# elizabethfong/SparkSmithWaterman

Measured on AMD Instinct MI355X. Metric: GCUPS, higher is better.
Workload: dtype int32

## Files before the change

include/swmi.h:

```cpp
#ifndef SWMI_H
#define SWMI_H

#include <stddef.h>
#include <stdint.h>

#ifdef __cplusplus
extern "C" {
#endif

#define SWMI_ABI_VERSION 3

typedef enum swmi_status {
    SWMI_OK               =  0,
    SWMI_ERR_INVALID      = -1,
    SWMI_ERR_NO_DEVICE    = -2,
    SWMI_ERR_HIP          = -3,
    SWMI_ERR_NOMEM        = -4,
    SWMI_ERR_UNSUPPORTED  = -5,
    SWMI_ERR_RANGE        = -6
} swmi_status;

#define SWMI_TIE_SERIAL 0
#define SWMI_TIE_STRICT 1

typedef struct swmi_params {
    int32_t match;
    int32_t mismatch;
    int32_t gap;
    int32_t tie_mode;
    char    types[4];
} swmi_params;

typedef struct swmi_ctx    swmi_ctx;
typedef struct swmi_batch  swmi_batch;

int         swmi_abi_version(void);
const char *swmi_last_error(void);
int         swmi_device_count(int *count);
int         swmi_create(int device, swmi_ctx **out);
void        swmi_destroy(swmi_ctx *ctx);
void        swmi_default_params(swmi_params *p);

int         swmi_set_option(swmi_ctx *ctx, const char *name, int64_t value);

int  swmi_batch_upload(swmi_ctx *ctx,
                       const uint8_t *ref_bytes, const uint64_t *ref_off, uint32_t n_refs,
                       const uint8_t *read_bytes, const uint64_t *read_off, uint32_t n_reads,
                       swmi_batch **out);
int  swmi_batch_run(swmi_ctx *ctx, swmi_batch *b, const swmi_params *p);
void swmi_batch_free(swmi_ctx *ctx, swmi_batch *b);
int  swmi_batch_run_async(swmi_ctx *ctx, swmi_batch *b, const swmi_params *p);
int  swmi_batch_wait(swmi_ctx *ctx);

typedef struct swmi_timing {
    float    fill_ms, traceback_ms, d2h_ms, total_ms;
    uint32_t fill_launches, rerun_pairs;
    uint64_t cells;
    uint64_t dir_bytes;
    uint32_t strip_fallbacks;
    uint32_t col_chunks;
    uint32_t resident_pairs;
    uint32_t tfused_pairs;
} swmi_timing;
int  swmi_batch_timing(const swmi_batch *b, swmi_timing *t);
int  swmi_batch_mode(const swmi_batch *b, int *mode);

#define SWMI_PAIR_DEGENERATE 0x1u
uint64_t swmi_batch_n_pairs(const swmi_batch *b);
int      swmi_pair_score(const swmi_batch *b, uint64_t pair, int32_t *score);
int      swmi_pair_n_alignments(const swmi_batch *b, uint64_t pair, uint64_t *n, uint32_t *flags);
int      swmi_batch_pair_results(const swmi_batch *b, int32_t *scores, uint64_t *n_alignments, uint64_t n);
int      swmi_pair_alignment(swmi_batch *b, uint64_t pair, uint64_t k,
                             int32_t *begin, int32_t *end_i, int32_t *end_j,
                             const char **ref_aln, const char **read_aln, uint32_t *len);

int      swmi_batch_materialise_all(swmi_batch *b, uint64_t *n_alignments, uint64_t *n_chars);

int      swmi_ref_total(const swmi_batch *b, uint32_t ref, int32_t *total);
int      swmi_ref_totals(const swmi_batch *b, int32_t *totals, uint32_t n);
int      swmi_ref_n_match_sites(swmi_batch *b, uint32_t ref, uint64_t *n);
int      swmi_ref_match_site(swmi_batch *b, uint32_t ref, uint64_t k, int32_t *begin,
                             const char **ref_aln, const char **read_aln, uint32_t *len);

int      swmi_ref_sites_packed(swmi_batch *b, uint32_t ref_lo, uint32_t ref_hi,
                               int32_t *totals, uint64_t *degenerate, uint64_t *site_first,
                               int32_t *begins, uint32_t *lens, uint64_t *str_off, uint64_t sites_cap,
                               uint8_t *blob, uint64_t blob_cap, uint64_t *n_sites, uint64_t *blob_bytes);

int  swmi_align_batch(swmi_ctx *ctx, const swmi_params *p,
                      const uint8_t *ref_bytes, const uint64_t *ref_off, uint32_t n_refs,
                      const uint8_t *read_bytes, const uint64_t *read_off, uint32_t n_reads,
                      swmi_batch **out);

typedef struct swmi_stream swmi_stream;
typedef struct swmi_stream_stats {
    double   push_ms;
    double   parse_ms;
    double   upload_ms, run_ms;
    double   gpu_sweep_ms, gpu_traceback_ms;
    uint64_t bytes, cells;
    uint32_t chunks, pad;
} swmi_stream_stats;
int      swmi_stream_open(swmi_ctx *ctx, const swmi_params *p, const uint8_t *read_bytes, const uint64_t *read_off,
                          uint32_t n_reads, uint32_t slots, uint64_t chunk_bytes, swmi_stream **out);
int      swmi_stream_push(swmi_stream *s, const uint8_t *ref_bytes, const uint64_t *ref_off, uint32_t n_refs);
int      swmi_stream_push_file(swmi_stream *s, const char *path, const char *delimiter, uint32_t parse_threads);
int      swmi_stream_push_file_shard(swmi_stream *s, const char *path, const char *delimiter, uint32_t parse_threads,
                                     uint32_t shard, uint32_t n_shards);
int      swmi_stream_finish(swmi_stream *s);
uint64_t swmi_stream_n_refs(const swmi_stream *s);
uint32_t swmi_stream_n_chunks(const swmi_stream *s);
int      swmi_stream_chunk(swmi_stream *s, uint32_t k, swmi_batch **batch, uint64_t *first_ref);
int      swmi_stream_totals(const swmi_stream *s, int32_t *totals, uint64_t n);
int      swmi_stream_metadata(const swmi_stream *s, uint64_t ref, char *buf, size_t cap);
int      swmi_stream_ref_pos(const swmi_stream *s, uint64_t ref, uint64_t *pos);
int      swmi_stream_ref_sequence(const swmi_stream *s, uint64_t ref, uint8_t *buf, uint64_t cap, uint64_t *len);
int      swmi_stream_get_stats(const swmi_stream *s, swmi_stream_stats *st);
void     swmi_stream_close(swmi_stream *s);

#ifdef __cplusplus
}
#endif
#endif
```

sparksmithwaterman_amd/_capi.py:

```python
import ctypes as C
import os

_HERE = os.path.dirname(os.path.abspath(__file__))
LIB_PATH = os.environ.get("SWMI_LIB") or os.path.join(_HERE, "lib", "libswmi.so")

TIE_SERIAL = 0
TIE_STRICT = 1
PAIR_DEGENERATE = 0x1


class SwmiError(RuntimeError):
    def __init__(self, code, msg):
        super().__init__("swmi error %d: %s" % (code, msg))
        self.code = code


class Params(C.Structure):
    _fields_ = [("match", C.c_int32), ("mismatch", C.c_int32), ("gap", C.c_int32),
                ("tie_mode", C.c_int32), ("types", C.c_char * 4)]


class Timing(C.Structure):
    _fields_ = [("fill_ms", C.c_float), ("traceback_ms", C.c_float), ("d2h_ms", C.c_float),
                ("total_ms", C.c_float), ("fill_launches", C.c_uint32), ("rerun_pairs", C.c_uint32),
                ("cells", C.c_uint64), ("dir_bytes", C.c_uint64),
                ("strip_fallbacks", C.c_uint32), ("col_chunks", C.c_uint32),
                ("resident_pairs", C.c_uint32), ("tfused_pairs", C.c_uint32)]


class StreamStats(C.Structure):
    _fields_ = [("push_ms", C.c_double), ("parse_ms", C.c_double), ("upload_ms", C.c_double), ("run_ms", C.c_double),
                ("gpu_sweep_ms", C.c_double), ("gpu_traceback_ms", C.c_double), ("bytes", C.c_uint64), ("cells", C.c_uint64),
                ("chunks", C.c_uint32), ("pad", C.c_uint32)]


_P = C.c_void_p
_u8p = C.POINTER(C.c_uint8)
_u64p = C.POINTER(C.c_uint64)
SYMBOLS = [
    ("swmi_abi_version", C.c_int, []),
    ("swmi_last_error", C.c_char_p, []),
    ("swmi_device_count", C.c_int, [C.POINTER(C.c_int)]),
    ("swmi_create", C.c_int, [C.c_int, C.POINTER(_P)]),
    ("swmi_destroy", None, [_P]),
    ("swmi_default_params", None, [C.POINTER(Params)]),
    ("swmi_set_option", C.c_int, [_P, C.c_char_p, C.c_int64]),
    ("swmi_batch_upload", C.c_int, [_P, C.c_char_p, _u64p, C.c_uint32, C.c_char_p, _u64p, C.c_uint32, C.POINTER(_P)]),
    ("swmi_batch_run", C.c_int, [_P, _P, C.POINTER(Params)]),
    ("swmi_batch_run_async", C.c_int, [_P, _P, C.POINTER(Params)]),
    ("swmi_batch_wait", C.c_int, [_P]),
    ("swmi_batch_free", None, [_P, _P]),
    ("swmi_batch_timing", C.c_int, [_P, C.POINTER(Timing)]),
    ("swmi_batch_mode", C.c_int, [_P, C.POINTER(C.c_int)]),
    ("swmi_batch_n_pairs", C.c_uint64, [_P]),
    ("swmi_pair_score", C.c_int, [_P, C.c_uint64, C.POINTER(C.c_int32)]),
    ("swmi_pair_n_alignments", C.c_int, [_P, C.c_uint64, _u64p, C.POINTER(C.c_uint32)]),
    ("swmi_pair_alignment", C.c_int, [_P, C.c_uint64, C.c_uint64, C.POINTER(C.c_int32), C.POINTER(C.c_int32),
                                      C.POINTER(C.c_int32), C.POINTER(C.c_char_p), C.POINTER(C.c_char_p),
                                      C.POINTER(C.c_uint32)]),
    ("swmi_batch_pair_results", C.c_int, [_P, C.POINTER(C.c_int32), _u64p, C.c_uint64]),
    ("swmi_batch_materialise_all", C.c_int, [_P, _u64p, _u64p]),
    ("swmi_ref_total", C.c_int, [_P, C.c_uint32, C.POINTER(C.c_int32)]),
    ("swmi_ref_totals", C.c_int, [_P, C.POINTER(C.c_int32), C.c_uint32]),
    ("swmi_ref_n_match_sites", C.c_int, [_P, C.c_uint32, _u64p]),
    ("swmi_ref_match_site", C.c_int, [_P, C.c_uint32, C.c_uint64, C.POINTER(C.c_int32), C.POINTER(C.c_char_p),
                                      C.POINTER(C.c_char_p), C.POINTER(C.c_uint32)]),
    ("swmi_ref_sites_packed", C.c_int, [_P, C.c_uint32, C.c_uint32, C.POINTER(C.c_int32), _u64p, _u64p, C.POINTER(C.c_int32),
                                        C.POINTER(C.c_uint32), _u64p, C.c_uint64, C.c_void_p, C.c_uint64, _u64p, _u64p]),
    ("swmi_stream_open", C.c_int, [_P, C.POINTER(Params), C.c_char_p, _u64p, C.c_uint32, C.c_uint32, C.c_uint64, C.POINTER(_P)]),
    ("swmi_stream_push", C.c_int, [_P, C.c_char_p, _u64p, C.c_uint32]),
    ("swmi_stream_push_file", C.c_int, [_P, C.c_char_p, C.c_char_p, C.c_uint32]),
    ("swmi_stream_push_file_shard", C.c_int, [_P, C.c_char_p, C.c_char_p, C.c_uint32, C.c_uint32, C.c_uint32]),
    ("swmi_stream_finish", C.c_int, [_P]),
    ("swmi_stream_n_refs", C.c_uint64, [_P]),
    ("swmi_stream_n_chunks", C.c_uint32, [_P]),
    ("swmi_stream_chunk", C.c_int, [_P, C.c_uint32, C.POINTER(_P), _u64p]),
    ("swmi_stream_totals", C.c_int, [_P, C.POINTER(C.c_int32), C.c_uint64]),
    ("swmi_stream_metadata", C.c_int, [_P, C.c_uint64, C.c_char_p, C.c_size_t]),
    ("swmi_stream_ref_pos", C.c_int, [_P, C.c_uint64, _u64p]),
    ("swmi_stream_ref_sequence", C.c_int, [_P, C.c_uint64, C.c_void_p, C.c_uint64, _u64p]),
    ("swmi_stream_get_stats", C.c_int, [_P, C.POINTER(StreamStats)]),
    ("swmi_stream_close", None, [_P]),
    ("swmi_align_batch", C.c_int, [_P, C.POINTER(Params), C.c_char_p, _u64p, C.c_uint32, C.c_char_p, _u64p,
                                   C.c_uint32, C.POINTER(_P)]),
]

_lib = None


def load():
    global _lib
    if _lib is None:
        if not os.path.exists(LIB_PATH):
            raise ImportError(
                "%s is missing: build it with `python -c 'import __graft_entry__ as g; g.build()'` "
                "(hipcc, gfx950).  There is no CPU fallback." % LIB_PATH)
        lib = C.CDLL(LIB_PATH)
        for name, res, args in SYMBOLS:
            f = getattr(lib, name)
            f.restype = res
            f.argtypes = args
        _lib = lib
    return _lib


def check(rc):
    if rc != 0:
        raise SwmiError(rc, load().swmi_last_error().decode("utf-8", "replace"))


def as_bytes(s):
    return bytes(s) if isinstance(s, (bytes, bytearray, memoryview)) else s.encode("latin-1")


def pack(seqs):
    bs = [as_bytes(s) for s in seqs]
    off = (C.c_uint64 * (len(bs) + 1))()
    t = 0
    for k, b in enumerate(bs):
        off[k] = t
        t += len(b)
    off[len(bs)] = t
    return b"".join(bs), off
```

sparksmithwaterman_amd/aligner.py:

```python
import ctypes as C
import weakref

from . import _capi
from ._capi import Params, Timing, StreamStats, check

DEFAULT_SCORES = (5, -3, -4)
DEFAULT_TYPES = ("a", "i", "d", "-")


def make_params(align_scores=None, align_types=None, tie_mode=_capi.TIE_SERIAL):
    sc = DEFAULT_SCORES if align_scores is None else tuple(int(x) for x in align_scores)
    ty = DEFAULT_TYPES if align_types is None else tuple(align_types)
    if len(sc) != 3 or len(ty) != 4:
        raise ValueError("alignScores needs 3 entries and alignTypes 4")
    p = Params()
    p.match, p.mismatch, p.gap = sc
    p.tie_mode = tie_mode
    p.types = b"".join(_capi.as_bytes(t)[:1] for t in ty)
    return p


class Context:

    def __init__(self, device=0):
        self._lib = _capi.load()
        h = C.c_void_p()
        check(self._lib.swmi_create(int(device), C.byref(h)))
        self._h = h
        self.device = int(device)

    def set_option(self, name, value):
        check(self._lib.swmi_set_option(self._h, name.encode(), int(value)))

    def upload(self, refs, reads):
        return Batch(self, refs, reads)

    def stream(self, reads, params=None, slots=0, chunk_bytes=0):
        return Stream(self, reads, params, slots, chunk_bytes)

    def close(self):
        if getattr(self, "_h", None):
            self._lib.swmi_destroy(self._h)
            self._h = None

    def __del__(self):
        try:
            self.close()
        except Exception:
            pass


class Batch:

    _owned = True

    @classmethod
    def _view(cls, lib, handle, n_refs, n_reads, owner):
        b = cls.__new__(cls)
        b._ctx, b._lib, b._h, b.n_refs, b.n_reads, b._owned = None, lib, handle, n_refs, n_reads, False
        b._owner = owner
        return b

    def __init__(self, ctx, refs, reads):
        self._ctx = ctx
        self._lib = ctx._lib
        self.n_refs, self.n_reads = len(refs), len(reads)
        rb, ro = _capi.pack(refs)
        qb, qo = _capi.pack(reads)
        h = C.c_void_p()
        check(self._lib.swmi_batch_upload(ctx._h, rb, ro, self.n_refs, qb, qo, self.n_reads, C.byref(h)))
        self._h = h

    def run(self, params=None):
        p = params if params is not None else make_params()
        check(self._lib.swmi_batch_run(self._ctx._h, self._h, C.byref(p)))
        return self

    def run_async(self, params=None):
        p = params if params is not None else make_params()
        self._async_params = p
        check(self._lib.swmi_batch_run_async(self._ctx._h, self._h, C.byref(p)))
        return self

    def wait(self):
        check(self._lib.swmi_batch_wait(self._ctx._h))
        return self

    def timing(self):
        t = Timing()
        check(self._lib.swmi_batch_timing(self._h, C.byref(t)))
        return t

    def pipeline_mode(self):
        v = C.c_int()
        check(self._lib.swmi_batch_mode(self._h, C.byref(v)))
        return v.value

    def score(self, pair):
        v = C.c_int32()
        check(self._lib.swmi_pair_score(self._h, pair, C.byref(v)))
        return v.value

    def n_alignments(self, pair):
        n, f = C.c_uint64(), C.c_uint32()
        check(self._lib.swmi_pair_n_alignments(self._h, pair, C.byref(n), C.byref(f)))
        return n.value, f.value

    def alignment(self, pair, k, with_cell=False):
        b, ei, ej = C.c_int32(), C.c_int32(), C.c_int32()
        r, q, ln = C.c_char_p(), C.c_char_p(), C.c_uint32()
        check(self._lib.swmi_pair_alignment(self._h, pair, k, C.byref(b), C.byref(ei), C.byref(ej),
                                            C.byref(r), C.byref(q), C.byref(ln)))
        rec = (b.value, (r.value.decode("latin-1"), q.value.decode("latin-1")))
        return rec + ((ei.value, ej.value),) if with_cell else rec

    def alignments(self, pair, with_cell=False):
        n, _ = self.n_alignments(pair)
        return [self.alignment(pair, k, with_cell) for k in range(n)]

    def pair_results(self):
        import numpy as np
        n = self.n_refs * self.n_reads
        sc = np.empty(n, dtype=np.int32)
        na = np.empty(n, dtype=np.uint64)
        check(self._lib.swmi_batch_pair_results(self._h, sc.ctypes.data_as(C.POINTER(C.c_int32)),
                                                na.ctypes.data_as(C.POINTER(C.c_uint64)), n))
        return sc, na

    def scores(self):
        import numpy as np
        n = self.n_refs * self.n_reads
        sc = np.empty(n, dtype=np.int32)
        check(self._lib.swmi_batch_pair_results(self._h, sc.ctypes.data_as(C.POINTER(C.c_int32)), None, n))
        return sc

    def materialise_all(self):
        na, nc = C.c_uint64(), C.c_uint64()
        check(self._lib.swmi_batch_materialise_all(self._h, C.byref(na), C.byref(nc)))
        return na.value, nc.value

    def ref_total(self, ref):
        v = C.c_int32()
        check(self._lib.swmi_ref_total(self._h, ref, C.byref(v)))
        return v.value

    def ref_totals(self):
        import numpy as np
        out = np.empty(self.n_refs, dtype=np.int32)
        check(self._lib.swmi_ref_totals(self._h, out.ctypes.data_as(C.POINTER(C.c_int32)), self.n_refs))
        return out

    def ref_match_sites(self, ref):
        n = C.c_uint64()
        check(self._lib.swmi_ref_n_match_sites(self._h, ref, C.byref(n)))
        out = []
        b, r, q, ln = C.c_int32(), C.c_char_p(), C.c_char_p(), C.c_uint32()
        for k in range(n.value):
            check(self._lib.swmi_ref_match_site(self._h, ref, k, C.byref(b), C.byref(r), C.byref(q), C.byref(ln)))
            out.append((b.value, (r.value.decode("latin-1"), q.value.decode("latin-1"))))
        return out

    def ref_sites_packed(self, ref_lo=0, ref_hi=None):
        import numpy as np
        ref_hi = self.n_refs if ref_hi is None else ref_hi
        n = ref_hi - ref_lo
        ns, nb = C.c_uint64(), C.c_uint64()
        check(self._lib.swmi_ref_sites_packed(self._h, ref_lo, ref_hi, None, None, None, None, None, None, 0, None, 0,
                                              C.byref(ns), C.byref(nb)))
        totals = np.empty(max(n, 1), dtype=np.int32)
        deg = np.empty(max(n, 1), dtype=np.uint64)
        first = np.empty(n + 1, dtype=np.uint64)
        begins = np.empty(max(ns.value, 1), dtype=np.int32)
        lens = np.empty(max(ns.value, 1), dtype=np.uint32)
        off = np.empty(max(ns.value, 1), dtype=np.uint64)
        blob = np.empty(max(nb.value, 1), dtype=np.uint8)
        P = C.POINTER
        check(self._lib.swmi_ref_sites_packed(
            self._h, ref_lo, ref_hi, totals.ctypes.data_as(P(C.c_int32)), deg.ctypes.data_as(P(C.c_uint64)),
            first.ctypes.data_as(P(C.c_uint64)), begins.ctypes.data_as(P(C.c_int32)), lens.ctypes.data_as(P(C.c_uint32)),
            off.ctypes.data_as(P(C.c_uint64)), ns.value, blob.ctypes.data_as(C.c_void_p), nb.value, C.byref(ns), C.byref(nb)))
        raw = blob.tobytes()
        out = []
        for r in range(n):
            sites = []
            for s in range(int(first[r]), int(first[r + 1])):
                o, ln = int(off[s]), int(lens[s])
                sites.append((int(begins[s]), (raw[o:o + ln].decode("latin-1"), raw[o + ln:o + 2 * ln].decode("latin-1"))))
            out.append((int(totals[r]), int(deg[r]), sites))
        return out

    def free(self):
        if getattr(self, "_h", None) and self._owned:
            self._lib.swmi_batch_free(self._ctx._h, self._h)
        self._h = None

    def __del__(self):
        try:
            self.free()
        except Exception:
            pass


class Stream:

    def __init__(self, ctx, reads, params=None, slots=0, chunk_bytes=0):
        self._ctx, self._lib = ctx, ctx._lib
        self.n_reads = len(reads)
        qb, qo = _capi.pack(reads)
        p = params if params is not None else make_params()
        h = C.c_void_p()
        check(self._lib.swmi_stream_open(ctx._h, C.byref(p), qb, qo, self.n_reads, int(slots), int(chunk_bytes), C.byref(h)))
        self._h = h
        self._views = []

    def push(self, refs):
        rb, ro = _capi.pack(refs)
        check(self._lib.swmi_stream_push(self._h, rb, ro, len(refs)))
        return self

    def push_file(self, path, delimiter=">gi", parse_threads=0):
        import os
        check(self._lib.swmi_stream_push_file(self._h, os.fspath(path).encode(), delimiter.encode("latin-1"), int(parse_threads)))
        return self

    def push_file_shard(self, path, shard, n_shards, delimiter=">gi", parse_threads=0):
        import os
        check(self._lib.swmi_stream_push_file_shard(self._h, os.fspath(path).encode(), delimiter.encode("latin-1"),
                                                    int(parse_threads), int(shard), int(n_shards)))
        return self

    def finish(self):
        check(self._lib.swmi_stream_finish(self._h))
        return self

    def n_refs(self):
        return self._lib.swmi_stream_n_refs(self._h)

    def chunks(self):
        out = []
        for k in range(self._lib.swmi_stream_n_chunks(self._h)):
            b, first = C.c_void_p(), C.c_uint64()
            check(self._lib.swmi_stream_chunk(self._h, k, C.byref(b), C.byref(first)))
            n_pairs = self._lib.swmi_batch_n_pairs(b)
            v = Batch._view(self._lib, b, n_pairs // max(self.n_reads, 1), self.n_reads, self)
            self._views.append(weakref.ref(v))
            out.append((first.value, v))
        return out

    def totals(self):
# ... 49 lines not shown
```

sparksmithwaterman_amd/csrc/swmi_api.cpp:

```cpp
#include <hip/hip_runtime.h>

#include <algorithm>
#include <atomic>
#include <chrono>
#include <condition_variable>
#include <unistd.h>
#include <cstdarg>
#include <cstdio>
#include <cstdlib>
#include <cstring>
#include <memory>
#include <mutex>
#include <numeric>
#include <string>
#include <thread>
#include <unordered_map>
#include <deque>
#include <vector>

#include "../../include/swmi.h"
#include "swmi_device.h"
#include "swmi_io_internal.h"

extern "C" hipError_t swmi_launch_fill(const FillArgs *a, hipStream_t st, hipEvent_t ev_start, hipEvent_t ev_stop);
extern "C" hipError_t swmi_launch_traceback(const TraceArgs *a, hipStream_t st, hipEvent_t ev_start, hipEvent_t ev_stop);
extern "C" hipError_t swmi_launch_traceback_split(const TraceArgs *a, uint32_t n_windows, hipStream_t st);
extern "C" hipError_t swmi_launch_resident(const TraceArgs *a, const ResidentArgs *x, hipStream_t st);
extern "C" hipError_t swmi_launch_tfused(const TraceArgs *a, const TFusedArgs *x, hipStream_t st);
extern "C" hipError_t swmi_launch_encode(const uint8_t *raw, const uint64_t *raw_off, SeqDesc *desc, uint32_t *seqw,
                                         const uint8_t *lut, uint32_t n_seq, hipStream_t st);

static thread_local std::string g_err;

static int fail(int code, const char *fmt, ...) {
    char buf[512];
    va_list ap;
    va_start(ap, fmt);
    vsnprintf(buf, sizeof buf, fmt, ap);
    va_end(ap);
    g_err = buf;
    return code;
}

int swmi_io_fail(int code, const std::string &msg) { return fail(code, "%s", msg.c_str()); }

#define HIP_TRY(expr)                                                                         \
    do {                                                                                      \
        hipError_t e_ = (expr);                                                               \
        if (e_ != hipSuccess)                                                                 \
            return fail(e_ == hipErrorOutOfMemory ? SWMI_ERR_NOMEM : SWMI_ERR_HIP,            \
                        "%s failed: %s", #expr, hipGetErrorString(e_));                       \
    } while (0)

struct DevBuf {
    void *p = nullptr;
    size_t cap = 0;
    int reserve(size_t bytes) {
        if (bytes <= cap) return SWMI_OK;
        size_t want = bytes >= (256u << 20) ? bytes + bytes / 2 : bytes;
        if (p) { want = std::max(want, cap + cap / 4); (void)hipFree(p); p = nullptr; cap = 0; }
        hipError_t e = hipMalloc(&p, want);
        if (e != hipSuccess && want > bytes) { want = bytes; e = hipMalloc(&p, want); }
        if (e != hipSuccess) { p = nullptr; return fail(SWMI_ERR_NOMEM, "hipMalloc(%zu) failed: %s", bytes, hipGetErrorString(e)); }
        cap = want;
        return SWMI_OK;
    }
    void release() { if (p) (void)hipFree(p); p = nullptr; cap = 0; }
    template <class T> T *as() const { return (T *)p; }
    DevBuf() = default;
    DevBuf(const DevBuf &) = delete;
    DevBuf &operator=(const DevBuf &) = delete;
    ~DevBuf() { release(); }
};

struct PinnedBuf {
    void *p = nullptr;
    void *dp = nullptr;
    size_t cap = 0;
    int reserve(size_t bytes) {
        if (bytes <= cap) return SWMI_OK;
        if (p) { bytes = std::max(bytes, cap + cap / 4); (void)hipHostFree(p); p = nullptr; dp = nullptr; cap = 0; }
        hipError_t e = hipHostMalloc(&p, bytes, hipHostMallocMapped);
        if (e != hipSuccess) { p = nullptr; return fail(SWMI_ERR_NOMEM, "hipHostMalloc(%zu) failed: %s", bytes, hipGetErrorString(e)); }
        e = hipHostGetDevicePointer(&dp, p, 0);
        if (e != hipSuccess) { (void)hipHostFree(p); p = nullptr; return fail(SWMI_ERR_HIP, "hipHostGetDevicePointer: %s", hipGetErrorString(e)); }
        cap = bytes;
        return SWMI_OK;
    }
    void release() { if (p) (void)hipHostFree(p); p = nullptr; dp = nullptr; cap = 0; }
    PinnedBuf() = default;
    PinnedBuf(const PinnedBuf &) = delete;
    PinnedBuf &operator=(const PinnedBuf &) = delete;
    ~PinnedBuf() { release(); }
};

struct swmi_ctx {
    int device = 0;
    hipStream_t stream = nullptr;
    std::mutex mu;
    uint32_t cell_cap = 64;
    uint64_t max_workspace_bytes = 32ull << 30;
    int profiling = 0;
    uint32_t mode = 1;
    int zero_copy = 1;
    uint64_t arena_words_per_pair = 160;
    uint64_t arena_copy_wpp = 160;
    uint64_t recs_per_pair_x16 = 32;
    hipEvent_t ev[6] = {nullptr, nullptr, nullptr, nullptr, nullptr, nullptr};
    PinnedBuf h_err;
    DevBuf d_hdr_ring;
    uint32_t hdr_next = 0;
    DevBuf d_lut;
    int64_t spin_us = 2000;
    uint32_t dbg_strip_spins = 0;
    uint32_t dbg_reverse_strips = 0;
    uint32_t auto_ties_x100 = 300;
    uint32_t col_chunks = 0;
    int tb_split = -1;
    bool ext_events = false;
    int tfused = -1;
    int resident = -1;
    int scores_only = 0;
    int stream_keep_records = 1;
    int device_strings = 1;
    bool cell_cap_set = false;
    std::thread worker;
    std::mutex job_mu;
    std::condition_variable job_cv;
    std::atomic<int> job_state{0};
    swmi_batch *job_batch = nullptr;
    swmi_params job_params{};
    int job_rc = 0;
    std::string job_err;
};

struct HostAln {
    uint32_t rank;
    int32_t begin, end_i, end_j;
    uint32_t n_ops;
    const uint32_t *rec = nullptr;
    int64_t str_id = -1;
};

struct PairRes {
    int32_t score = 0;
    uint32_t flags = 0;
    uint64_t n_cells = 0;
    uint64_t first = 0;
    uint64_t count = 0;
};

struct SiteRef { uint64_t pair; uint64_t k; int32_t begin; };

struct Work {
    uint32_t pair;
    uint64_t cells;
    uint64_t dir_words;
    uint64_t seam_words;
};

struct swmi_batch {
    uint32_t n_refs = 0, n_reads = 0;
    std::vector<uint8_t> ref_bytes, read_bytes;
    const uint8_t *src_map = nullptr;
    std::vector<swmi_io_recpos> src_recs;
    std::unordered_map<uint32_t, std::vector<uint8_t>> src_cache;
    std::vector<uint64_t> ref_off, read_off;
    std::vector<SeqDesc> ref_desc, read_desc;
    DevBuf d_raw, d_raw_off;
    DevBuf d_seqw, d_refs, d_reads, d_pairs, d_dir, d_seam, d_result, d_cells, d_cells_off, d_cells_cap, d_dbg, d_dbg2;
    DevBuf d_strip_items, d_progress;
    DevBuf d_col_items;
    DevBuf d_win_off, d_queue;
    DevBuf d_tf_items;
    DevBuf d_res_items;
    bool views_built = false;
    bool tb_split_used = false;
    bool acgt_known = false;
    PinnedBuf h_result;
    swmi_params params{};
    bool has_run = false;
    int auto_choice = -1;
    swmi_params auto_params{};
    std::vector<Work> work;
    int work_mode = -1;
    bool work_tfused = false;
    uint32_t eff_mode = 1;
    uint64_t work_cells = 0;
    std::vector<uint8_t> pairs_on_device;
    const void *pairs_dev_ptr = nullptr;
    struct Prep {
        bool valid = false;
        size_t lo = 0, hi = 0;
        const void *work = nullptr;
        swmi_params params{};
        int mode = -1;
        uint64_t dir_words = 0, seam_words = 0;
        uint32_t max_path = 0, max_read = 0;
        size_t n_strip_items = 0, n_col_items = 0, n_strip_chunks = 0;
        uint64_t n_windows = 0, seam_priv_words = 0;
        size_t n_res = 0;
        uint32_t res_lds_words = 0, res_ops_words = 0;
        int resident_opt = -1;
        int tfused_opt = -1;
        size_t n_tf = 0;
        uint32_t tf_max_m = 0, tf_max_n = 0, tf_max_path = 0;
        bool exact = false, scores_only = false;
        uint32_t col_chunks_opt = 0;
        bool reverse_strips = false;
    } prep;
    std::vector<PairRes> pairs;
    struct RawChunk { size_t at, words; size_t tab_at, n_rec; size_t lo; std::vector<uint32_t> wpos; };
    std::vector<uint32_t> raw;
    std::vector<AlnRec> rtab;
    const uint32_t *raw_ext = nullptr;
    const AlnRec *rtab_ext = nullptr;
    uint64_t raw_ext_records = 0, raw_ext_cap = 0;
    std::vector<RawChunk> raw_chunks;
    bool indexed = false;
    bool rec_strings = false;
    bool scores_only = false;
    bool records_dropped = false;
    std::vector<HostAln> alns;
    std::vector<char> str_buf;
    std::vector<uint64_t> str_at;
    std::vector<int8_t> ref_view_ready;
    std::vector<std::vector<SiteRef>> ref_sites;
    std::vector<uint64_t> ref_degenerate;
    swmi_timing timing{};
};

static const uint8_t *code_table();

extern "C" int swmi_abi_version(void) { return SWMI_ABI_VERSION; }

extern "C" const char *swmi_last_error(void) { return g_err.c_str(); }

extern "C" int swmi_device_count(int *count) {
    if (!count) return fail(SWMI_ERR_INVALID, "count is null");
    int n = 0;
    hipError_t e = hipGetDeviceCount(&n);
    if (e != hipSuccess) { *count = 0; return fail(SWMI_ERR_NO_DEVICE, "hipGetDeviceCount: %s", hipGetErrorString(e)); }
    *count = n;
    return SWMI_OK;
}

extern "C" void swmi_default_params(swmi_params *p) {
    if (!p) return;
    p->match = 5; p->mismatch = -3; p->gap = -4;
    p->tie_mode = SWMI_TIE_SERIAL;
    p->types[0] = 'a'; p->types[1] = 'i'; p->types[2] = 'd'; p->types[3] = '-';
}

static void ctx_release(swmi_ctx *c) {
    for (auto &ev : c->ev) if (ev) (void)hipEventDestroy(ev);
    if (c->stream) (void)hipStreamDestroy(c->stream);
    c->h_err.release();
    c->d_lut.release();
    c->d_hdr_ring.release();
    delete c;
}

extern "C" int swmi_create(int device, swmi_ctx **out) {
    if (!out) return fail(SWMI_ERR_INVALID, "out is null");
    *out = nullptr;
    int n = 0;
    hipError_t e = hipGetDeviceCount(&n);
    if (e != hipSuccess || n <= 0)
        return fail(SWMI_ERR_NO_DEVICE, "no HIP device available (%s); this library has no CPU fallback",
                    e != hipSuccess ? hipGetErrorString(e) : "device count 0");
    if (device < 0 || device >= n) return fail(SWMI_ERR_INVALID, "device %d out of range [0,%d)", device, n);
    hipDeviceProp_t prop;
    e = hipGetDeviceProperties(&prop, device);
    if (e != hipSuccess) return fail(SWMI_ERR_NO_DEVICE, "hipGetDeviceProperties: %s", hipGetErrorString(e));
    if (strncmp(prop.gcnArchName, "gfx950", 6) != 0)
        return fail(SWMI_ERR_NO_DEVICE, "device %d is %s; the kernels are built for gfx950 (MI355X) only",
                    device, prop.gcnArchName);
    e = hipSetDevice(device);
    if (e != hipSuccess) return fail(SWMI_ERR_NO_DEVICE, "hipSetDevice: %s", hipGetErrorString(e));
    swmi_ctx *c = new swmi_ctx;
    c->device = device;
    e = hipStreamCreateWithFlags(&c->stream, hipStreamNonBlocking);
    if (e != hipSuccess) { c->stream = nullptr; ctx_release(c); return fail(SWMI_ERR_HIP, "hipStreamCreate: %s", hipGetErrorString(e)); }
    for (auto &ev : c->ev) {
        e = hipEventCreate(&ev);
        if (e != hipSuccess) { ev = nullptr; ctx_release(c); return fail(SWMI_ERR_HIP, "hipEventCreate: %s", hipGetErrorString(e)); }
    }
    { int r = c->h_err.reserve(64); if (r) { ctx_release(c); return r; } }
    { static const char *ee = getenv("SWMI_EXT_EVENTS"); if (ee) c->ext_events = atoi(ee) != 0; }
    *(volatile uint32_t *)c->h_err.p = 0u;
    { int r = c->d_lut.reserve(256); if (r) { ctx_release(c); return r; } }
    e = hipMemcpy(c->d_lut.p, code_table(), 256, hipMemcpyHostToDevice);
    if (e != hipSuccess) { ctx_release(c); return fail(SWMI_ERR_HIP, "code table upload: %s", hipGetErrorString(e)); }
    *out = c;
    return SWMI_OK;
}

extern "C" void swmi_destroy(swmi_ctx *ctx) {
    if (!ctx) return;
    (void)hipSetDevice(ctx->device);
    if (ctx->worker.joinable()) {
        {
            std::unique_lock<std::mutex> lk(ctx->job_mu);
            ctx->job_cv.wait(lk, [&] { return ctx->job_state.load() != 1; });
            ctx->job_state.store(3);
        }
        ctx->job_cv.notify_all();
        ctx->worker.join();
    }
    ctx_release(ctx);
}

extern "C" int swmi_set_option(swmi_ctx *ctx, const char *name, int64_t value) {
    if (!ctx || !name) return fail(SWMI_ERR_INVALID, "null argument");
    std::lock_guard<std::mutex> g(ctx->mu);
    if (!strcmp(name, "cell_cap")) {
        if (value < 1 || value > (1 << 20)) return fail(SWMI_ERR_INVALID, "cell_cap out of range");
        ctx->cell_cap = (uint32_t)value;
        ctx->cell_cap_set = true;
    } else if (!strcmp(name, "max_workspace_bytes")) {
        if (value < (1 << 20)) return fail(SWMI_ERR_INVALID, "max_workspace_bytes too small");
        ctx->max_workspace_bytes = (uint64_t)value;
    } else if (!strcmp(name, "mode")) {
        if (value < -1 || value > 2) return fail(SWMI_ERR_INVALID, "mode must be -1 (automatic), 0, 1 or 2");
        ctx->mode = value < 0 ? 1u : (uint32_t)value;
    } else if (!strcmp(name, "auto_ties_x100")) {
        if (value < 100) return fail(SWMI_ERR_INVALID, "auto_ties_x100 out of range");
        ctx->auto_ties_x100 = (uint32_t)value;
    } else if (!strcmp(name, "spin_us")) {
        if (value < 0) return fail(SWMI_ERR_INVALID, "spin_us out of range");
        ctx->spin_us = value;
    } else if (!strcmp(name, "debug_strip_spins")) {
        ctx->dbg_strip_spins = (uint32_t)value;
    } else if (!strcmp(name, "debug_reverse_strips")) {
        ctx->dbg_reverse_strips = value != 0;
    } else if (!strcmp(name, "tfused")) {
        if (value < -1 || value > 1) return fail(SWMI_ERR_INVALID, "tfused must be -1 (automatic), 0 or 1");
        ctx->tfused = (int)value;
    } else if (!strcmp(name, "resident")) {
        if (value < -1 || value > 1) return fail(SWMI_ERR_INVALID, "resident must be -1 (automatic), 0 or 1");
        ctx->resident = (int)value;
    } else if (!strcmp(name, "scores_only")) {
        ctx->scores_only = value != 0;
    } else if (!strcmp(name, "stream_keep_records")) {
        ctx->stream_keep_records = value != 0;
    } else if (!strcmp(name, "device_strings")) {
        ctx->device_strings = value != 0;
    } else if (!strcmp(name, "tb_split")) {
        if (value < -1 || value > 1) return fail(SWMI_ERR_INVALID, "tb_split must be -1 (automatic), 0 or 1");
        ctx->tb_split = (int)value;
    } else if (!strcmp(name, "col_chunks")) {
        if (value < 0 || value > 4096) return fail(SWMI_ERR_INVALID, "col_chunks out of range");
        ctx->col_chunks = (uint32_t)value;
    } else if (!strcmp(name, "zero_copy")) {
        ctx->zero_copy = value != 0;
    } else if (!strcmp(name, "profiling")) {
        if (value < 0 || value > 2) return fail(SWMI_ERR_INVALID, "profiling must be 0, 1 (every stage) or 2 (the sweep only)");
        ctx->profiling = (int)value;
    } else if (!strcmp(name, "arena_words_per_pair")) {
        if (value < 1) return fail(SWMI_ERR_INVALID, "arena_words_per_pair out of range");
        ctx->arena_words_per_pair = (uint64_t)value;
    } else {
        return fail(SWMI_ERR_INVALID, "unknown option '%s'", name);
    }
    return SWMI_OK;
}

static const uint8_t *code_table() {
    static uint8_t T[256];
    static std::once_flag once;
    std::call_once(once, [] {
        uint8_t perm[256];
        for (int i = 0; i < 256; i++) perm[i] = (uint8_t)i;
        const uint8_t fast[8] = {'A', 'C', 'G', 'T', 'N', 'U', 'R', 'Y'};
        for (int k = 0; k < 8; k++) std::swap(perm[fast[k]], perm[4 * k]);
        for (int i = 0; i < 256; i++) {
            int u = i;
            if ((i >= 'a' && i <= 'z') || (i >= 0xE0 && i <= 0xFE && i != 0xF7)) u = i - 32;
            T[i] = perm[u];
        }
    });
    return T;
}

static uint64_t layout_sequences(const uint64_t *off, uint32_t n, uint64_t word0, std::vector<SeqDesc> &desc) {
    desc.resize(n);
    uint64_t at = word0;
    for (uint32_t s = 0; s < n; s++) {
        const uint64_t len = off[s + 1] - off[s];
        at = (at + 3) & ~(uint64_t)3;
        SeqDesc d{};
        d.len = (uint32_t)len;
        d.boff = (uint32_t)at;
        d.acgt = 0;
        desc[s] = d;
        at += (len + 3) / 4 + SWMI_SEQ_PAD_WORDS;
    }
    return at;
}

static int check_offsets(const uint64_t *off, uint32_t n, const char *what) {
    if (!off) return fail(SWMI_ERR_INVALID, "%s offsets are null", what);
    if (off[0] != 0) return fail(SWMI_ERR_INVALID, "%s offsets must start at 0", what);
    for (uint32_t k = 0; k < n; k++) {
        if (off[k + 1] < off[k]) return fail(SWMI_ERR_INVALID, "%s offsets decrease at %u", what, k);
        if (off[k + 1] - off[k] >= (1ull << 30))
            return fail(SWMI_ERR_UNSUPPORTED, "%s %u is longer than 2^30-1 bases", what, k);
    }
    return SWMI_OK;
}

extern "C" void swmi_batch_free(swmi_ctx *ctx, swmi_batch *b) {
    if (!b) return;
    if (ctx) (void)hipSetDevice(ctx->device);
    b->d_raw.release(); b->d_raw_off.release();
    b->d_seqw.release(); b->d_refs.release(); b->d_reads.release(); b->d_pairs.release();
    b->d_dir.release(); b->d_seam.release(); b->d_result.release(); b->d_cells.release();
    b->d_cells_off.release(); b->d_cells_cap.release(); b->d_dbg.release(); b->d_dbg2.release();
    b->d_strip_items.release(); b->d_progress.release(); b->d_col_items.release(); b->d_win_off.release(); b->d_queue.release(); b->d_res_items.release();
    b->d_tf_items.release();
    b->h_result.release();
    delete b;
}

static int upload_device(swmi_ctx *ctx, swmi_batch *b, hipStream_t st, const uint8_t *ref_src, const uint8_t *read_src) {
    const uint32_t n_refs = b->n_refs, n_reads = b->n_reads;
    const uint64_t ref_total = b->ref_off[n_refs], read_total = b->read_off[n_reads];
    uint64_t words = layout_sequences(b->ref_off.data(), n_refs, 0, b->ref_desc);
    words = layout_sequences(b->read_off.data(), n_reads, words, b->read_desc);
    words = ((words + 3) & ~(uint64_t)3) + SWMI_SEQ_PAD_WORDS;
    if (words >= (1ull << 32)) return fail(SWMI_ERR_UNSUPPORTED, "sequence image exceeds 16 GiB");
    int rc;
    const uint64_t read_base = (ref_total + 15) & ~(uint64_t)15;
    if ((rc = b->d_seqw.reserve(words * 4))) return rc;
    if ((rc = b->d_raw.reserve(read_base + read_total + 16))) return rc;
    if ((rc = b->d_raw_off.reserve(((uint64_t)n_refs + n_reads + 2) * 8))) return rc;
    if ((rc = b->d_refs.reserve(std::max<size_t>(n_refs, 1) * sizeof(SeqDesc)))) return rc;
    if ((rc = b->d_reads.reserve(std::max<size_t>(n_reads, 1) * sizeof(SeqDesc)))) return rc;
    HIP_TRY(hipMemsetAsync(b->d_seqw.p, 0, words * 4, st));
    uint8_t *raw = b->d_raw.as<uint8_t>();
    uint64_t *roff = b->d_raw_off.as<uint64_t>();
    if (ref_total) HIP_TRY(hipMemcpyAsync(raw, ref_src, ref_total, hipMemcpyHostToDevice, st));
    if (read_total) HIP_TRY(hipMemcpyAsync(raw + read_base, read_src, read_total, hipMemcpyHostToDevice, st));
    HIP_TRY(hipMemcpyAsync(roff, b->ref_off.data(), ((size_t)n_refs + 1) * 8, hipMemcpyHostToDevice, st));
    std::vector<uint64_t> read_abs(b->read_off);
    for (auto &o : read_abs) o += read_base;
    HIP_TRY(hipMemcpyAsync(roff + n_refs + 1, read_abs.data(), ((size_t)n_reads + 1) * 8, hipMemcpyHostToDevice, st));
    if (n_refs) HIP_TRY(hipMemcpyAsync(b->d_refs.p, b->ref_desc.data(), n_refs * sizeof(SeqDesc), hipMemcpyHostToDevice, st));
    if (n_reads) HIP_TRY(hipMemcpyAsync(b->d_reads.p, b->read_desc.data(), n_reads * sizeof(SeqDesc), hipMemcpyHostToDevice, st));
    HIP_TRY(swmi_launch_encode(raw, roff, b->d_refs.as<SeqDesc>(), b->d_seqw.as<uint32_t>(), ctx->d_lut.as<uint8_t>(), n_refs, st));
    HIP_TRY(swmi_launch_encode(raw, roff + n_refs + 1, b->d_reads.as<SeqDesc>(), b->d_seqw.as<uint32_t>(),
                               ctx->d_lut.as<uint8_t>(), n_reads, st));
    HIP_TRY(hipStreamSynchronize(st));
    b->work_mode = -1; b->prep.valid = false; b->pairs_dev_ptr = nullptr; b->pairs_on_device.clear();
    b->has_run = false; b->acgt_known = false; b->auto_choice = -1;
    return SWMI_OK;
}

extern "C" int swmi_batch_upload(swmi_ctx *ctx,
                                 const uint8_t *ref_bytes, const uint64_t *ref_off, uint32_t n_refs,
                                 const uint8_t *read_bytes, const uint64_t *read_off, uint32_t n_reads,
                                 swmi_batch **out) {
    if (!ctx || !out) return fail(SWMI_ERR_INVALID, "null argument");
    *out = nullptr;
    int rc;
    if ((rc = check_offsets(ref_off, n_refs, "reference"))) return rc;
    if ((rc = check_offsets(read_off, n_reads, "read"))) return rc;
    if ((n_refs && ref_off[n_refs] && !ref_bytes) || (n_reads && read_off[n_reads] && !read_bytes))
        return fail(SWMI_ERR_INVALID, "sequence bytes are null");
    if ((uint64_t)n_refs * n_reads >= (1ull << 32))
        return fail(SWMI_ERR_UNSUPPORTED, "more than 2^32-1 pairs in one batch");
    std::lock_guard<std::mutex> g(ctx->mu);
    HIP_TRY(hipSetDevice(ctx->device));

    std::unique_ptr<swmi_batch> b(new swmi_batch);
    b->n_refs = n_refs; b->n_reads = n_reads;
    b->ref_off.assign(ref_off, ref_off + n_refs + 1);
    b->read_off.assign(read_off, read_off + n_reads + 1);
    b->ref_bytes.assign(ref_bytes, ref_bytes + ref_off[n_refs]);
    b->read_bytes.assign(read_bytes, read_bytes + read_off[n_reads]);
    if ((rc = upload_device(ctx, b.get(), ctx->stream, ref_bytes, read_bytes))) { swmi_batch_free(ctx, b.release()); return rc; }
    *out = b.release();
    return SWMI_OK;
}

namespace {

struct RunState {
    swmi_ctx *ctx;
    swmi_batch *b;
    FillArgs fa{};
    TraceArgs ta{};
    float fill_ms = 0, tb_ms = 0, d2h_ms = 0;
    uint32_t launches = 0;
    double enqueue_us = 0, wait_us = 0, copyout_us = 0, prep_us = 0, prep_upload_us = 0;
    bool one_wave_sweep = false;
    bool tb_split = false;
    bool defer_copy = false;
    bool keep = true;
};

inline size_t result_out_off() { return 64; }
inline size_t result_tab_off(size_t np) { return (64 + np * sizeof(PairOut) + 255) & ~(size_t)255; }
inline size_t result_arena_off(size_t np, uint64_t tab_cap) { return (result_tab_off(np) + tab_cap * sizeof(AlnRec) + 255) & ~(size_t)255; }
inline uint64_t rec_words(uint32_t n_ops, bool strings) {
    return strings ? 2 * ((uint64_t)n_ops / 4 + 1) : ((uint64_t)n_ops + 15) / 16;
}

}

#define SWMI_RES_CELL_CAP 128u

static uint64_t path_bound(uint64_t n_, uint64_t m_, const swmi_params &p) {
    uint64_t path = n_ + m_;
    if (p.match > 0 && p.gap < 0 && p.mismatch <= p.match) {
        const uint64_t g = (uint64_t)(-(int64_t)p.gap), mt = (uint64_t)p.match;
        path = std::min(path, std::min(m_ + std::min(n_, mt * m_ / g), n_ + std::min(m_, mt * n_ / g)));
    }
    return path;
}

static uint64_t traceback_lds_bytes(uint32_t mode, uint64_t max_path, uint64_t max_read) {
    const uint64_t lds_words = (max_path + 3) / 4 + 1, lds_read_words = (max_read + 3) / 4 + 1;
    const uint64_t win = (uint64_t)SWMI_RMAX * 64;
    const uint64_t tile_words = mode == 0 ? 4ull * 16 * win : (mode == 1 ? 32 + 8ull * SWMI_CK_BLOCKS * win : 4ull * SWMI_CK_BLOCKS * win);
    return 4ull * (tile_words + 4ull * (lds_words + lds_read_words + 96));
}

static int prepare_chunk(RunState &rs, const std::vector<Work> &work, size_t lo, size_t hi, const std::vector<uint64_t> *cells_exact) {
    swmi_ctx *ctx = rs.ctx;
    swmi_batch *b = rs.b;
    const size_t np = hi - lo;
    const uint32_t n_reads = b->n_reads;
    int rc;

    std::vector<PairDesc> pd;
    std::vector<StripItem> strip_items;
    uint64_t seam_priv_words = 0;
    size_t n_strip_chunks = 0;
    std::vector<ColItem> col_items;
    uint64_t dir_words = 0, seam_words = 0;
    uint32_t max_path = 0, max_read = 0;
    size_t n_strip_items = 0, n_col_items = 0;
    uint64_t n_windows = 0;
    std::vector<uint32_t> win_off;
    std::vector<uint32_t> res_items;
    size_t n_res = 0;
    uint32_t res_lds_words = 0, res_ops_words = 0;
    std::vector<uint32_t> tf_items;
    size_t n_tf = 0;
    uint32_t tf_max_m = 0, tf_max_n = 0, tf_max_path = 0;
    const uint32_t res_cell_cap = SWMI_RES_CELL_CAP;
    swmi_batch::Prep &pr = b->prep;
    const auto p0 = std::chrono::steady_clock::now();
    const bool prepared = pr.valid && pr.lo == lo && pr.hi == hi && pr.work == (const void *)work.data() && pr.mode == b->eff_mode &&
                          memcmp(&pr.params, &b->params, sizeof(swmi_params)) == 0 && b->pairs_dev_ptr == b->d_pairs.p &&
                          b->pairs_on_device.size() == np * sizeof(PairDesc) && pr.col_chunks_opt == ctx->col_chunks &&
                          pr.reverse_strips == (ctx->dbg_reverse_strips != 0) && pr.resident_opt == ctx->resident &&
                          pr.tfused_opt == ctx->tfused && pr.exact == (cells_exact != nullptr) && pr.scores_only == (ctx->scores_only != 0);
    if (prepared) {
        dir_words = pr.dir_words; seam_words = pr.seam_words; max_path = pr.max_path; max_read = pr.max_read;
        n_strip_items = pr.n_strip_items; n_col_items = pr.n_col_items; n_windows = pr.n_windows;
        seam_priv_words = pr.seam_priv_words; n_strip_chunks = pr.n_strip_chunks;
        n_res = pr.n_res; res_lds_words = pr.res_lds_words; res_ops_words = pr.res_ops_words;
        n_tf = pr.n_tf; tf_max_m = pr.tf_max_m; tf_max_n = pr.tf_max_n; tf_max_path = pr.tf_max_path;
    } else {
    const swmi_params &P = b->params;
    const bool cols_possible = b->eff_mode == 1 && P.match > 0 && P.gap < 0 && P.mismatch <= 0 &&
                               P.match <= 7 && P.mismatch >= -8 && (np <= 512 || ctx->col_chunks > 1) && ctx->col_chunks != 1;
    const bool res_possible = b->eff_mode == 1 && !cells_exact && !ctx->scores_only && ctx->resident != 0 && (ctx->resident == 1 || np >= 256) &&
                              P.match <= 7 && P.match >= -8 && P.mismatch >= -8 && P.mismatch <= 0 && P.gap <= 0;
    auto res_need_words = [&](uint32_t m_, uint32_t n_, uint32_t &opw) -> uint64_t {
        const uint32_t R_ = swmi_rows_per_lane(m_), lact = (m_ + R_ - 1) / R_;
        const uint64_t nblk = ((uint64_t)n_ + lact - 1 + 15) / 16, n_ck = (nblk + SWMI_CK_BLOCKS - 1) / SWMI_CK_BLOCKS;
        opw = (uint32_t)((path_bound(n_, m_, P) + 15) / 16 + 1);
        return nblk * R_ * 64 + ((n_ck + 1) & ~1ull) + 2ull * res_cell_cap + 64ull * opw + (n_ + 3) / 4 + 1 + (m_ + 3) / 4 + 1 + 8 +
               128;
    };
    bool res_maybe = false;
    if (res_possible)
        for (size_t k = 0; k < np && !res_maybe; k++) {
            const uint32_t m_ = b->read_desc[work[lo + k].pair % n_reads].len, n_ = b->ref_desc[work[lo + k].pair / n_reads].len;
            uint32_t opw;
            res_maybe = m_ <= 64u * SWMI_RMAX && (ctx->resident == 1 || (uint64_t)n_ <= 8ull * m_) &&
                        res_need_words(m_, n_, opw) * 4 <= (ctx->resident == 1 ? 40u : 20u) * 1024u;
        }
    const bool tf_possible = b->eff_mode == 1 && !cells_exact && !ctx->scores_only && ctx->tfused == 1 &&
                             P.match > 0 && P.match <= 7 && P.mismatch >= -8 && P.mismatch <= P.match && P.gap < 0 && P.gap >= -64;
    if ((cols_possible || res_maybe || tf_possible) && !b->acgt_known) {
        if (b->n_refs) HIP_TRY(hipMemcpy(b->ref_desc.data(), b->d_refs.p, b->n_refs * sizeof(SeqDesc), hipMemcpyDeviceToHost));
        if (b->n_reads) HIP_TRY(hipMemcpy(b->read_desc.data(), b->d_reads.p, b->n_reads * sizeof(SeqDesc), hipMemcpyDeviceToHost));
        b->acgt_known = true;
    }
    const uint64_t chunk_budget = ctx->col_chunks > 1 ? ctx->col_chunks : std::max<uint64_t>(1, 1024 / std::max<size_t>(np, 1));
    pd.resize(np);
    if (b->eff_mode == 1) win_off.resize(np + 1);
    uint32_t pb_m = 0xFFFFFFFFu, pb_n = 0xFFFFFFFFu, pb_val = 0;
    for (size_t k = 0; k < np; k++) {
        const Work &w = work[lo + k];
        PairDesc d{};
        d.ref_id = w.pair / n_reads;
        d.read_id = w.pair % n_reads;
        d.out_id = (uint32_t)k;
        const uint32_t m_ = b->read_desc[d.read_id].len, n_ = b->ref_desc[d.ref_id].len;
        if (b->eff_mode == 1) {
            const uint64_t rps = 64ull * swmi_rows_per_lane(m_);
            const uint64_t wb = ((uint64_t)n_ + 63u + 15u) / 16u;
            win_off[k] = (uint32_t)std::min<uint64_t>(n_windows, 0xFFFFFFFFu);
            n_windows += ((m_ + rps - 1) / rps) * ((wb + SWMI_CK_BLOCKS - 1u) / SWMI_CK_BLOCKS);
        }
        uint32_t res_opw = 0;
        const bool res_fit = res_maybe && m_ <= 64u * SWMI_RMAX && b->read_desc[d.read_id].acgt && b->ref_desc[d.ref_id].acgt &&
                             (ctx->resident == 1 || (uint64_t)n_ <= 8ull * m_) &&
                             res_need_words(m_, n_, res_opw) * 4 <= (ctx->resident == 1 ? 40u : 20u) * 1024u;
        const bool tf_fit = !res_fit && tf_possible && m_ <= SWMI_TF_MAX_M && n_ <= 64u * SWMI_TF_BMAX &&
                            b->read_desc[d.read_id].acgt && b->ref_desc[d.ref_id].acgt && w.dir_words >= swmi_tf_ck_words(m_);
        if (tf_fit) {
            d.pad = SWMI_PAD_RESIDENT;
            tf_items.push_back((uint32_t)k);
            tf_max_m = std::max(tf_max_m, m_); tf_max_n = std::max(tf_max_n, n_);
            tf_max_path = std::max<uint32_t>(tf_max_path, (uint32_t)path_bound(n_, m_, P));
        } else if (res_fit) {
            d.pad = SWMI_PAD_RESIDENT;
            res_items.push_back((uint32_t)k);
            uint32_t opw;
            res_lds_words = std::max<uint32_t>(res_lds_words, (uint32_t)res_need_words(m_, n_, opw));
            res_ops_words = std::max(res_ops_words, opw);
        } else if (b->eff_mode == 1 && m_ > 64u * SWMI_RMAX && strip_items.size() < (1u << 30)) {
            const uint32_t strips = (m_ + 64u * SWMI_RMAX - 1u) / (64u * SWMI_RMAX);
            d.pad = (uint32_t)strip_items.size();
            auto push_strips = [&](StripItem it) {
                it.pair = (uint32_t)k;
                it.prog = (uint32_t)strip_items.size();
                it.pad = 0;
                if (ctx->dbg_reverse_strips) for (uint32_t st = strips; st-- > 0;) { it.strip = st; strip_items.push_back(it); }
                else                         for (uint32_t st = 0; st < strips; st++) { it.strip = st; strip_items.push_back(it); }
            };
            uint64_t chunks = 1;
            const uint64_t wblocks = ((uint64_t)n_ + 63u + 15u) / 16u;
            const uint32_t n_ck = (uint32_t)((wblocks + SWMI_CK_BLOCKS - 1u) / SWMI_CK_BLOCKS);
            const uint32_t step_w = 16u * SWMI_CK_BLOCKS;
            const uint64_t span = (uint64_t)m_ + (uint64_t)(P.match > 0 ? P.match : 0) * m_ / (uint64_t)(P.gap < 0 ? -(int64_t)P.gap : 1) + 1;
            if (cols_possible) {
                const uint64_t budget = ctx->col_chunks > 1 ? ctx->col_chunks : chunk_budget / strips;
                chunks = std::min<uint64_t>(budget, n_ / std::max<uint64_t>((span + 64) / 4, 256));
                chunks = std::min<uint64_t>(chunks, n_ck);
                if (chunks < 2) chunks = 1;
            }
            if (chunks == 1) {
                StripItem it{};
                it.col0 = 0; it.g_lo = 0; it.g_hi = 0xFFFFFFFFu; it.priv_stride = 0; it.priv_off = 0;
                push_strips(it);
            } else {
                const uint32_t wpc = (uint32_t)((n_ck + chunks - 1) / chunks);
                for (uint32_t g_lo = 0; g_lo < n_ck; g_lo += wpc) {
                    StripItem it{};
                    it.g_lo = g_lo;
                    it.g_hi = std::min(g_lo + wpc, n_ck);
                    if (it.g_hi < n_ck && (uint64_t)it.g_hi * step_w > n_) it.g_hi = n_ck;
                    const int64_t c0 = (int64_t)g_lo * step_w - 64 - (int64_t)span - 1;
                    it.col0 = g_lo == 0 || c0 <= 0 ? 0u : (uint32_t)(c0 / step_w * step_w);
                    const uint64_t ext0 = (uint64_t)it.g_hi * step_w - it.col0 + 64ull * (strips - 1u);
                    const uint64_t n0 = it.g_hi < n_ck ? std::min<uint64_t>(n_ - it.col0, ext0) : n_ - it.col0;
                    it.priv_stride = (uint32_t)((n0 + 1 + 15) & ~15ull);
                    it.priv_off = seam_priv_words;
                    seam_priv_words += (uint64_t)(strips - 1u) * it.priv_stride;
                    if (it.g_hi == n_ck) it.g_hi = 0xFFFFFFFFu;
                    push_strips(it);
                    n_strip_chunks++;
                    if (it.g_hi == 0xFFFFFFFFu) break;
                }
            }
        } else if (cols_possible && chunk_budget > 1 && m_ <= 64u * SWMI_RMAX && b->read_desc[d.read_id].acgt && b->ref_desc[d.ref_id].acgt) {
            const uint64_t span = (uint64_t)m_ + (uint64_t)P.match * m_ / (uint64_t)(-(int64_t)P.gap) + 1;
            const uint64_t wblocks = ((uint64_t)n_ + 63u + 15u) / 16u;
            const uint32_t n_ck = (uint32_t)((wblocks + SWMI_CK_BLOCKS - 1u) / SWMI_CK_BLOCKS);
            const uint32_t step_w = 16u * SWMI_CK_BLOCKS;
            uint64_t chunks = std::min<uint64_t>(chunk_budget, n_ / std::max<uint64_t>(span + 64, 256));
            chunks = std::min<uint64_t>(chunks, n_ck);
            static const bool dbg_one = getenv("SWMI_DEBUG_ONE_CHUNK") != nullptr;
            if (dbg_one) chunks = 1;
            if (chunks >= 2 || dbg_one) {
                const uint32_t wpc = (uint32_t)((n_ck + chunks - 1) / chunks);
                const size_t first = col_items.size();
                for (uint32_t g_lo = 0; g_lo < n_ck; g_lo += wpc) {
                    ColItem ci;
                    ci.pair = (uint32_t)k;
                    ci.g_lo = g_lo;
                    ci.g_hi = std::min(g_lo + wpc, n_ck);
                    if (ci.g_hi < n_ck && (uint64_t)ci.g_hi * step_w > n_) ci.g_hi = n_ck;
                    const int64_t c0 = (int64_t)g_lo * step_w - 64 - (int64_t)span - 1;
                    ci.col0 = g_lo == 0 || c0 <= 0 ? 0u : (uint32_t)(c0 / step_w * step_w);
                    col_items.push_back(ci);
                    if (ci.g_hi == n_ck) break;
                }
                d.pad = SWMI_PAD_COLS | (uint32_t)(col_items.size() - first);
            }
        }
        pd[k] = d;
        if (m_ != pb_m || n_ != pb_n) { pb_m = m_; pb_n = n_; pb_val = (uint32_t)path_bound(n_, m_, b->params); }
        max_path = std::max<uint32_t>(max_path, pb_val);
        max_read = std::max(max_read, m_);
    }
    n_strip_items = strip_items.size();
    n_col_items = col_items.size();
    n_res = res_items.size();
    n_tf = tf_items.size();
    res_lds_words = 0;
    for (uint32_t k : res_items) {
        uint32_t opw;
        const uint32_t m_ = b->read_desc[pd[k].read_id].len, n_ = b->ref_desc[pd[k].ref_id].len;
        const uint64_t own = res_need_words(m_, n_, opw);
        res_lds_words = std::max<uint32_t>(res_lds_words, (uint32_t)(own + 64ull * (res_ops_words - opw)));
    }
    if (16ull * res_lds_words > 160ull * 1024) {
        for (uint32_t k : res_items) pd[k].pad = 0;
        res_items.clear();
        n_res = 0; res_lds_words = 0; res_ops_words = 0;
    }
    {
        std::vector<uint8_t> is_res(np, 0);
        for (uint32_t k : res_items) is_res[k] = 1;
        for (size_t k = 0; k < np; k++) {
            pd[k].dir_off = dir_words;
            pd[k].seam_off = seam_words;
            if (!is_res[k]) { dir_words += work[lo + k].dir_words; seam_words += work[lo + k].seam_words; }
        }
    }
    if (b->eff_mode == 1) win_off[np] = (uint32_t)std::min<uint64_t>(n_windows, 0xFFFFFFFFu);
    for (StripItem &it : strip_items)
        if (it.priv_stride) it.priv_off += seam_words;
    }
    const auto p1 = std::chrono::steady_clock::now();
    if (!prepared && b->eff_mode == 1) {
        if ((rc = b->d_win_off.reserve((np + 1) * sizeof(uint32_t)))) return rc;
        HIP_TRY(hipMemcpyAsync(b->d_win_off.p, win_off.data(), (np + 1) * sizeof(uint32_t), hipMemcpyHostToDevice, ctx->stream));
        HIP_TRY(hipStreamSynchronize(ctx->stream));
    }
    if ((rc = b->d_pairs.reserve(np * sizeof(PairDesc)))) return rc;
    if (!prepared && !strip_items.empty()) {
        if ((rc = b->d_strip_items.reserve(strip_items.size() * sizeof(StripItem)))) return rc;
        if ((rc = b->d_progress.reserve(strip_items.size() * sizeof(uint32_t)))) return rc;
        HIP_TRY(hipMemcpyAsync(b->d_strip_items.p, strip_items.data(), strip_items.size() * sizeof(StripItem), hipMemcpyHostToDevice, ctx->stream));
        HIP_TRY(hipStreamSynchronize(ctx->stream));
    }
    if (!prepared && !res_items.empty()) {
        if ((rc = b->d_res_items.reserve(res_items.size() * sizeof(uint32_t)))) return rc;
        HIP_TRY(hipMemcpyAsync(b->d_res_items.p, res_items.data(), res_items.size() * sizeof(uint32_t), hipMemcpyHostToDevice, ctx->stream));
        HIP_TRY(hipStreamSynchronize(ctx->stream));
    }
    if (!prepared && !tf_items.empty()) {
        if ((rc = b->d_tf_items.reserve(tf_items.size() * sizeof(uint32_t)))) return rc;
        HIP_TRY(hipMemcpyAsync(b->d_tf_items.p, tf_items.data(), tf_items.size() * sizeof(uint32_t), hipMemcpyHostToDevice, ctx->stream));
        HIP_TRY(hipStreamSynchronize(ctx->stream));
    }
    if (!prepared && !col_items.empty()) {
        if ((rc = b->d_col_items.reserve(col_items.size() * sizeof(ColItem)))) return rc;
        HIP_TRY(hipMemcpyAsync(b->d_col_items.p, col_items.data(), col_items.size() * sizeof(ColItem), hipMemcpyHostToDevice, ctx->stream));
        HIP_TRY(hipStreamSynchronize(ctx->stream));
    }
    if ((rc = b->d_dir.reserve(std::max<uint64_t>(dir_words, 1) * 4))) return rc;
    if ((rc = b->d_seam.reserve(std::max<uint64_t>(seam_words + seam_priv_words, 1) * 4))) return rc;
    if (!prepared && (b->pairs_dev_ptr != b->d_pairs.p || b->pairs_on_device.size() != np * sizeof(PairDesc) ||
        memcmp(b->pairs_on_device.data(), pd.data(), np * sizeof(PairDesc)) != 0)) {
        HIP_TRY(hipMemcpyAsync(b->d_pairs.p, pd.data(), np * sizeof(PairDesc), hipMemcpyHostToDevice, ctx->stream));
        HIP_TRY(hipStreamSynchronize(ctx->stream));
        b->pairs_on_device.assign((const uint8_t *)pd.data(), (const uint8_t *)pd.data() + np * sizeof(PairDesc));
        b->pairs_dev_ptr = b->d_pairs.p;
    }
    if (!prepared) {
        pr.valid = b->pairs_dev_ptr == b->d_pairs.p;
        pr.lo = lo; pr.hi = hi; pr.work = (const void *)work.data(); pr.params = b->params; pr.mode = b->eff_mode;
        pr.dir_words = dir_words; pr.seam_words = seam_words; pr.max_path = max_path; pr.max_read = max_read;
        pr.n_strip_items = n_strip_items; pr.n_col_items = n_col_items; pr.n_windows = n_windows;
        pr.seam_priv_words = seam_priv_words; pr.n_strip_chunks = n_strip_chunks;
        pr.n_res = n_res; pr.res_lds_words = res_lds_words; pr.res_ops_words = res_ops_words;
        pr.resident_opt = ctx->resident; pr.exact = cells_exact != nullptr;
        pr.tfused_opt = ctx->tfused; pr.n_tf = n_tf; pr.tf_max_m = tf_max_m; pr.tf_max_n = tf_max_n; pr.tf_max_path = tf_max_path;
        pr.col_chunks_opt = ctx->col_chunks; pr.reverse_strips = ctx->dbg_reverse_strips != 0;
        pr.scores_only = ctx->scores_only != 0;
    }
    rs.prep_us += std::chrono::duration<double, std::micro>(p1 - p0).count();
    rs.prep_upload_us += std::chrono::duration<double, std::micro>(std::chrono::steady_clock::now() - p1).count();
    return SWMI_OK;
}

static int dump_traceback_diagnostics(swmi_batch *b, const TraceArgs &ta, size_t np, size_t n_tf) {
    if (!ta.dbg) return SWMI_OK;
    std::vector<unsigned long long> d(np * 4);
    HIP_TRY(hipMemcpy(d.data(), ta.dbg, np * 32, hipMemcpyDeviceToHost));
    if (n_tf) {
        double t0 = 0, t1 = 0, t2 = 0, t3 = 0, t4 = 0, t5 = 0; unsigned long long mx = 0;
        for (size_t k = 0; k < np; k++) {
            t0 += d[4*k]; t1 += d[4*k+1] & 0xFFFFFFFFull; t2 += d[4*k+1] >> 32; t3 += d[4*k+2] >> 16; t4 += d[4*k+3] >> 32; t5 += d[4*k+3] & 0xFFFFFFFFull;
            mx = std::max(mx, d[4*k]);
        }
        fprintf(stderr, "[swmi tfused dbg] ticks per sweeper wavefront: lifetime mean=%.0f max=%llu = prologue %.0f + sweep %.0f + first block task %.0f (%.2f block tasks per wavefront) + waiting for tasks %.0f + rest (more tasks, walk items) %.0f\n",
                t0 / np, mx, t2 / np, t1 / np, t3 / np, t5 / np, t4 / np, (t0 - t1 - t2 - t3 - t4) / np);
        {
            std::vector<size_t> idx(np);
            for (size_t k = 0; k < np; k++) idx[k] = k;
            std::sort(idx.begin(), idx.end(), [&](size_t x, size_t y) { return d[4 * x] < d[4 * y]; });
            auto at = [&](double q) { return d[4 * idx[std::min<size_t>(np - 1, (size_t)(q * np))]]; };
            fprintf(stderr, "[swmi tfused dbg]   lifetime p10=%llu p50=%llu p90=%llu p99=%llu max=%llu\n", at(0.10), at(0.50), at(0.90), at(0.99), d[4 * idx[np - 1]]);
            for (size_t t = 0; t < std::min<size_t>(np, 6); t++) {
                const size_t k = idx[np - 1 - t];
                fprintf(stderr, "[swmi tfused dbg]   slow wavefront (pair %zu): lifetime %llu, sweep %llu, first block task %llu, block tasks taken %llu, waiting %llu, alignments of its pair %llu\n",
                        k, d[4 * k], d[4 * k + 1] & 0xFFFFFFFFull, d[4 * k + 2] >> 16, d[4 * k + 3] & 0xFFFFFFFFull, d[4 * k + 3] >> 32,
                        (unsigned long long)((const PairOut *)((const uint8_t *)b->h_result.p + result_out_off()))[k].n_cells);
            }
        }
    }
    double a0 = 0, a1 = 0, a2 = 0, a3 = 0; unsigned long long mx = 0;
    double a4 = 0;
    for (size_t k = 0; k < np; k++) { a0 += d[4*k]; a1 += d[4*k+1] & 0xFFFFFFFFull; a2 += d[4*k+2] & 0xFFFF; a4 += d[4*k+2] >> 16; a3 += d[4*k+3] & 0xFFFFFFFFull; mx = std::max(mx, d[4*k]); }
    fprintf(stderr, "[swmi tb dbg] wave ticks mean=%.0f max=%llu; walk ticks mean=%.0f; staging ticks mean=%.0f; steps mean=%.1f; iterations mean=%.2f\n",
            a0 / np, mx, a1 / np, a4 / np, a2 / np, a3 / np);
    const PairOut *po_dbg = (const PairOut *)((const uint8_t *)b->h_result.p + result_out_off());
    double cs[4] = {0, 0, 0, 0}, cw[4] = {0, 0, 0, 0}; unsigned long long cm[4] = {0, 0, 0, 0}; size_t cn[4] = {0, 0, 0, 0};
    for (size_t k = 0; k < np; k++) {
        const size_t c = std::min<uint64_t>(po_dbg[k].n_cells, 4) - (po_dbg[k].n_cells ? 1 : 0);
        cs[c] += d[4 * k]; cw[c] += d[4 * k + 1] & 0xFFFFFFFFull; cm[c] = std::max(cm[c], d[4 * k]); cn[c]++;
    }
    {
        std::vector<size_t> idx(np);
        for (size_t k = 0; k < np; k++) idx[k] = k;
        const size_t top = std::min<size_t>(np, 6);
        std::partial_sort(idx.begin(), idx.begin() + top, idx.end(), [&](size_t x, size_t y) { return d[4 * x] > d[4 * y]; });
        for (size_t t = 0; t < top; t++)
            fprintf(stderr, "[swmi tb dbg]   slow pair %zu: ticks=%llu walk=%llu staging=%llu in %llu stagings, steps=%llu iterations=%llu alignments=%llu\n", idx[t],
                    d[4 * idx[t]], d[4 * idx[t] + 1] & 0xFFFFFFFFull, d[4 * idx[t] + 2] >> 16, d[4 * idx[t] + 3] >> 32, d[4 * idx[t] + 2] & 0xFFFF,
                    d[4 * idx[t] + 3] & 0xFFFFFFFFull, (unsigned long long)po_dbg[idx[t]].n_cells);
        for (size_t t = 0; t < top; t++)
            fprintf(stderr, "[swmi tb dbg]     ... of the staging time of pair %zu, %llu ticks waiting for helpers\n", idx[t], d[4 * idx[t] + 1] >> 32);
    }
    for (int c = 0; c < 4; c++)
        if (cn[c]) fprintf(stderr, "[swmi tb dbg]   %d%s alignment(s): %zu pairs, wave ticks mean=%.0f max=%llu, walk(slot 0) mean=%.0f\n",
                           c + 1, c == 3 ? "+" : "", cn[c], cs[c] / cn[c], cm[c], cw[c] / cn[c]);
    return SWMI_OK;
}

static int dump_fill_diagnostics(swmi_batch *b, const FillArgs &fa, size_t np) {
    if (!fa.dbg) return SWMI_OK;
    std::vector<unsigned long long> d(np * 2);
    HIP_TRY(hipMemcpy(d.data(), fa.dbg, np * 16, hipMemcpyDeviceToHost));
#ifdef SWMI_STRIP_DIAG
    for (size_t k = 0; k < np && k < 8; k++)
        fprintf(stderr, "[swmi strip dbg] pair %zu: strip 0 lifetime %llu ticks, %llu waiting before publications; strip 1 lifetime %llu, "
                "%llu polls, %llu ticks in polls, %llu waiting for seam groups\n", k, d[2 * k] >> 32, d[2 * k] & 0xFFFFFFFFull,
                d[2 * k + 1] >> 40, (d[2 * k + 1] >> 32) & 0xFF, (d[2 * k + 1] >> 16) & 0xFFFF, d[2 * k + 1] & 0xFFFF);
#endif
    unsigned long long ev = 0, cyc = 0, evmax = 0, cmax = 0, cmin = ~0ull;
    for (size_t k = 0; k < np; k++) {
        ev += d[2 * k]; cyc += d[2 * k + 1];
        evmax = std::max(evmax, d[2 * k]); cmax = std::max(cmax, d[2 * k + 1]); cmin = std::min(cmin, d[2 * k + 1]);
    }
    fprintf(stderr, "[swmi fill dbg] pairs=%zu slow-path entries mean=%.1f max=%llu; wave ticks mean=%.0f min=%llu max=%llu\n",
            np, (double)ev / np, evmax, (double)cyc / np, cmin, cmax);
    if (b->eff_mode == 1) {
        std::unordered_map<unsigned long long, int> per_simd, per_cu;
        for (size_t k = 0; k < np; k++) {
            const unsigned long long hw = d[2 * k] & 0xFFFFFFFFull, xcc = (d[2 * k] >> 32) & 0xF;
            const unsigned long long simd = (hw >> 4) & 3, cu = (hw >> 8) & 15, sh = (hw >> 12) & 1, se = (hw >> 13) & 7;
            const unsigned long long cukey = (xcc << 16) | (se << 8) | (sh << 4) | cu;
            per_cu[cukey]++; per_simd[(cukey << 4) | simd]++;
        }
        int h_simd[9] = {0}, h_cu[17] = {0};
        for (auto &kv : per_simd) h_simd[std::min(kv.second, 8)]++;
        for (auto &kv : per_cu) h_cu[std::min(kv.second, 16)]++;
        fprintf(stderr, "[swmi fill dbg] placement: %zu CUs, %zu SIMDs used; SIMDs by waves held: 1:%d 2:%d 3:%d 4+:%d; CUs by waves held: 1-4:%d 5-8:%d 9+:%d\n",
                per_cu.size(), per_simd.size(), h_simd[1], h_simd[2], h_simd[3], h_simd[4] + h_simd[5] + h_simd[6] + h_simd[7] + h_simd[8],
                h_cu[1] + h_cu[2] + h_cu[3] + h_cu[4], h_cu[5] + h_cu[6] + h_cu[7] + h_cu[8], h_cu[9] + h_cu[10] + h_cu[11] + h_cu[12] + h_cu[13] + h_cu[14] + h_cu[15] + h_cu[16]);
    }
    return SWMI_OK;
}

static int keep_chunk_records(RunState &rs, const AlnRec *tab, uint64_t n_rec, const uint32_t *arena, uint64_t arena_cap, size_t lo) {
    swmi_batch *b = rs.b;
    if (rs.defer_copy && b->raw_chunks.empty()) {
        b->raw_ext = arena; b->rtab_ext = tab; b->raw_ext_records = n_rec; b->raw_ext_cap = arena_cap;
        b->raw_chunks.push_back(swmi_batch::RawChunk{0, 0, 0, (size_t)n_rec, lo, {}});
        return SWMI_OK;
    }
    uint64_t used = 0;
    for (uint64_t k = 0; k < n_rec; k++) {
        const uint64_t end = (((uint64_t)tab[k].off_hi << 32) | tab[k].off_lo) + rec_words(tab[k].n_ops, b->rec_strings);
        used = std::max(used, end);
    }
    if (used > arena_cap) return fail(SWMI_ERR_HIP, "record payloads overrun the arena");
    b->raw_chunks.push_back(swmi_batch::RawChunk{b->raw.size(), (size_t)used, b->rtab.size(), (size_t)n_rec, lo, {}});
    b->raw.insert(b->raw.end(), arena, arena + used);
    b->rtab.insert(b->rtab.end(), tab, tab + n_rec);
    return SWMI_OK;
}

static int run_chunk(RunState &rs, const std::vector<Work> &work, size_t lo, size_t hi,
                     const std::vector<uint64_t> *cells_exact, std::vector<PairOut> &outs) {
    swmi_ctx *ctx = rs.ctx;
    swmi_batch *b = rs.b;
    const size_t np = hi - lo;
    int rc;
    if ((rc = prepare_chunk(rs, work, lo, hi, cells_exact))) return rc;
    const swmi_batch::Prep &pr = b->prep;
    const uint64_t seam_words = pr.seam_words, n_windows = pr.n_windows;
    const uint32_t max_path = pr.max_path, max_read = pr.max_read;
    const size_t n_strip_items = pr.n_strip_items, n_col_items = pr.n_col_items, n_res = pr.n_res, n_tf = pr.n_tf;
    const uint32_t res_lds_words = pr.res_lds_words, res_ops_words = pr.res_ops_words, res_cell_cap = SWMI_RES_CELL_CAP;
    const uint32_t tf_max_m = pr.tf_max_m, tf_max_n = pr.tf_max_n, tf_max_path = pr.tf_max_path;
    if (seam_words) HIP_TRY(hipMemsetAsync(b->d_seam.p, 0, seam_words * 4, ctx->stream));

    uint32_t cell_cap = ctx->cell_cap;
    std::vector<uint64_t> coff;
    std::vector<uint32_t> ccap;
    uint64_t cells_total = 0;
    if (cells_exact) {
        coff.resize(np); ccap.resize(np);
        for (size_t k = 0; k < np; k++) {
            coff[k] = cells_total;
            ccap[k] = (uint32_t)std::min<uint64_t>((*cells_exact)[lo + k], 0xFFFFFFFFu);
            cells_total += ccap[k];
        }
        if ((rc = b->d_cells_off.reserve(np * 8))) return rc;
        if ((rc = b->d_cells_cap.reserve(np * 4))) return rc;
        HIP_TRY(hipMemcpyAsync(b->d_cells_off.p, coff.data(), np * 8, hipMemcpyHostToDevice, ctx->stream));
        HIP_TRY(hipMemcpyAsync(b->d_cells_cap.p, ccap.data(), np * 4, hipMemcpyHostToDevice, ctx->stream));
    } else {
        if (!ctx->cell_cap_set) cell_cap = (uint32_t)std::min<uint64_t>(65536, std::max<uint64_t>(cell_cap, (4ull << 20) / np));
        cells_total = (uint64_t)np * cell_cap;
    }
    if ((rc = b->d_cells.reserve(std::max<uint64_t>(cells_total, 1) * sizeof(uint2)))) return rc;

    const uint32_t lds_words = (max_path + 3) / 4 + 1;
    const uint32_t lds_read_words = (max_read + 3) / 4 + 1;
    {
        const uint64_t need = traceback_lds_bytes(b->eff_mode, max_path, max_read);
        if (need > 160ull * 1024)
            return fail(SWMI_ERR_UNSUPPORTED, "a pair of %u bases in total needs %llu bytes of LDS for the traceback (limit 163840)",
                        max_path, (unsigned long long)need);
    }

    const auto c0 = std::chrono::steady_clock::now();
    uint64_t arena_cap = std::max<uint64_t>(np * ctx->arena_words_per_pair, 1024);
    uint64_t tab_cap = std::max<uint64_t>(np * ctx->recs_per_pair_x16 / 16 + 64, 256);
    std::vector<uint8_t> saved_outs;
    for (int attempt = 0;; attempt++) {
        if (attempt > 4) return fail(SWMI_ERR_HIP, "the record arena overflowed %d times in a row; results discarded", attempt);
        const size_t t_off = result_tab_off(np), a_off = result_arena_off(np, tab_cap);
        if ((rc = b->d_result.reserve(a_off + arena_cap * 4))) return rc;
        uint8_t *res = b->d_result.as<uint8_t>();
        if (attempt > 0) {
            HIP_TRY(hipMemsetAsync(res, 0, 64, ctx->stream));
            HIP_TRY(hipMemcpyAsync(res + result_out_off(), saved_outs.data(), saved_outs.size(),
                                   hipMemcpyHostToDevice, ctx->stream));
        }

        FillArgs &fa = rs.fa;
        fa.seqw = b->d_seqw.as<uint32_t>();
        fa.refs = b->d_refs.as<SeqDesc>();
        fa.reads = b->d_reads.as<SeqDesc>();
        fa.pairs = b->d_pairs.as<PairDesc>();
        fa.dir = b->d_dir.as<uint32_t>();
        fa.seam = b->d_seam.as<int32_t>();
        fa.out = (PairOut *)(res + result_out_off());
        fa.cells = b->d_cells.as<uint2>();
        fa.cells_off = cells_exact ? b->d_cells_off.as<uint64_t>() : nullptr;
        fa.cells_cap = cells_exact ? b->d_cells_cap.as<uint32_t>() : nullptr;
        fa.hdr = (ArenaHdr *)res;
        fa.dbg = nullptr;
        fa.dbg_pad = 0;
        static const bool dbg_fill = getenv("SWMI_DEBUG_FILL") != nullptr;
        if (dbg_fill) {
            if ((rc = b->d_dbg.reserve(np * 16))) return rc;
            fa.dbg = b->d_dbg.as<unsigned long long>();
            fa.dbg_thr0 = getenv("SWMI_DEBUG_THR0") ? (uint32_t)atoi(getenv("SWMI_DEBUG_THR0")) : 1u;
            fa.dbg_pad = getenv("SWMI_DEBUG_SKIP") ? 1u : 0u;
        }
        fa.n_pairs = (uint32_t)np;
        fa.cell_cap = cell_cap;
        fa.match = b->params.match; fa.mismatch = b->params.mismatch; fa.gap = b->params.gap;
        fa.strict = b->params.tie_mode == SWMI_TIE_STRICT;
        fa.mode = b->eff_mode;
        const bool pipe = n_strip_items && !rs.one_wave_sweep;
        fa.skip_multi = pipe ? 1u : 0u;
        fa.strip_items = pipe ? b->d_strip_items.as<StripItem>() : nullptr;
        fa.progress = pipe ? b->d_progress.as<uint32_t>() : nullptr;
        fa.n_strip_items = pipe ? (uint32_t)n_strip_items : 0u;
        fa.err_host = (uint32_t *)ctx->h_err.dp;
        fa.pad3 = 0;
        if (attempt == 0) b->timing.col_chunks += (uint32_t)n_col_items + (pipe ? (uint32_t)pr.n_strip_chunks : 0u);
        fa.col_items = n_col_items ? b->d_col_items.as<ColItem>() : nullptr;
        fa.n_col_items = (uint32_t)n_col_items;
        fa.strip_spins = ctx->dbg_strip_spins;
        const bool split_q = rs.tb_split && !cells_exact && b->eff_mode == 1 && n_windows < 0xFFFFFFFFull;
        const uint64_t q_cap = std::min<uint64_t>(std::max<uint64_t>(cells_total, 1), 1ull << 24);
        if (split_q && (rc = b->d_queue.reserve(256 + q_cap * sizeof(uint4)))) return rc;
        fa.q_reset = split_q ? b->d_queue.as<uint32_t>() : nullptr;

        TraceArgs &ta = rs.ta;
        ta.seqw = fa.seqw; ta.refs = fa.refs; ta.reads = fa.reads; ta.pairs = fa.pairs;
        ta.dir = fa.dir; ta.out = fa.out; ta.cells = fa.cells;
        ta.cells_off = fa.cells_off; ta.cells_cap = fa.cells_cap;
        ta.hdr = (ArenaHdr *)res;
        ta.arena = (uint32_t *)(res + a_off);
        ta.arena_cap_words = arena_cap;
        ta.rec_tab = (AlnRec *)(res + t_off);
        ta.rec_tab_cap = (uint32_t)std::min<uint64_t>(tab_cap, 0xFFFFFFFFu);
        ta.n_pairs = fa.n_pairs; ta.cell_cap = fa.cell_cap;
        ta.match = fa.match; ta.mismatch = fa.mismatch; ta.gap = fa.gap; ta.strict = fa.strict;
        ta.lds_words = lds_words;
        ta.seam = fa.seam;
        ta.mode = b->eff_mode;
        ta.pad2 = 0;
        ta.lds_read_words = lds_read_words;
        ta.out_host = nullptr;
        ta.ovf_host = (uint32_t *)ctx->h_err.dp + 4;
        ((volatile uint32_t *)ctx->h_err.p)[4] = 0u; ((volatile uint32_t *)ctx->h_err.p)[5] = 0u;
        ta.win_off = nullptr; ta.q_count = nullptr; ta.q_items = nullptr; ta.q_cap = 0; ta.pad4 = 0;
        const bool strings = ctx->device_strings != 0 && b->d_raw.p != nullptr;
        ta.raw = strings ? b->d_raw.as<uint8_t>() : nullptr;
        ta.raw_off = strings ? b->d_raw_off.as<uint64_t>() : nullptr;
        ta.raw_reads_at = b->n_refs + 1u;
        b->rec_strings = strings;
        ResidentArgs xa;
        xa.res_items = n_res ? b->d_res_items.as<uint32_t>() : nullptr;
        xa.n_res = (uint32_t)n_res; xa.res_lds_words = res_lds_words; xa.res_cell_cap = res_cell_cap; xa.res_ops_words = res_ops_words;
        TFusedArgs xt{};
        xt.items = n_tf ? b->d_tf_items.as<uint32_t>() : nullptr;
        xt.n_items = (uint32_t)n_tf;
        xt.cell_cap = 16;
        xt.tile_words = ((tf_max_m + 63u + 15u) / 16u) * 64u * SWMI_TF_BR;
        xt.ref_words = (tf_max_n + 3u) / 4u + 1u;
        xt.read_words = (tf_max_m + 3u) / 4u + 1u;
        xt.stage_words = (tf_max_path + 3u) / 4u + 1u + 128u;
        static const bool tf_marks = getenv("SWMI_DEBUG_MARKS") != nullptr;
        xt.debug_marks = tf_marks ? 1u : 0u;
        xt.lds_words = (xt.tile_words + 2u * xt.cell_cap + xt.stage_words + xt.ref_words + xt.read_words + 3u) & ~3u;
        {
            static const int tf_helpers = getenv("SWMI_TF_HELPERS") ? atoi(getenv("SWMI_TF_HELPERS")) : 2;
            const uint64_t region = 4ull * xt.lds_words, budget = 156ull * 1024;
            const uint64_t left = budget > 4 * region ? budget - 4 * region : 0;
            xt.n_helpers = (uint32_t)std::min<uint64_t>((uint64_t)std::max(0, std::min(tf_helpers, (int)SWMI_TF_HELPERS)), region ? left / region : 0);
        }
        const bool zc = ctx->zero_copy != 0;
        if (zc) {
            if ((rc = b->h_result.reserve(a_off + arena_cap * 4))) return rc;
            uint8_t *hd = (uint8_t *)b->h_result.dp;
            *(volatile uint32_t *)b->h_result.p = 0u;
            ((volatile uint32_t *)b->h_result.p)[1] = 0u;
            ta.ovf_host = (uint32_t *)hd;
            ta.out_host = (PairOut *)(hd + result_out_off());
            ta.arena = (uint32_t *)(hd + a_off);
            ta.rec_tab = (AlnRec *)(hd + t_off);
        }
        ta.dbg = nullptr;
        if (dbg_fill) {
            if ((rc = b->d_dbg2.reserve(np * 32))) return rc;
            HIP_TRY(hipMemsetAsync(b->d_dbg2.p, 0, np * 32, ctx->stream));
            ta.dbg = b->d_dbg2.as<unsigned long long>();
        }

        const bool whole_only = zc && n_tf + n_res == np;
        if (whole_only) {
            const uint32_t slots = 1024;
            if (!ctx->d_hdr_ring.p || ctx->hdr_next >= slots) {
                if ((rc = ctx->d_hdr_ring.reserve((size_t)slots * 64))) return rc;
                HIP_TRY(hipMemsetAsync(ctx->d_hdr_ring.p, 0, (size_t)slots * 64, ctx->stream));
                ctx->hdr_next = 0;
            }
            ta.hdr = (ArenaHdr *)(ctx->d_hdr_ring.as<uint8_t>() + (size_t)ctx->hdr_next++ * 64);
        }
        const bool split_now = rs.tb_split && !cells_exact && b->eff_mode == 1 && n_windows < 0xFFFFFFFFull;
        const bool ext_timing = ctx->profiling == 1 && attempt == 0 && !whole_only && !n_res && !n_tf && !split_now && b->eff_mode == 1 &&
                                !fa.n_strip_items && !fa.n_col_items && ctx->ext_events;
        if (ctx->profiling && !ext_timing) HIP_TRY(hipEventRecord(ctx->ev[0], ctx->stream));
        if (attempt == 0 && !whole_only) {
            if (fa.n_strip_items) HIP_TRY(hipMemsetAsync(fa.progress, 0, (size_t)fa.n_strip_items * sizeof(uint32_t), ctx->stream));
            HIP_TRY(swmi_launch_fill(&fa, ctx->stream, ext_timing ? ctx->ev[0] : nullptr, ext_timing ? ctx->ev[1] : nullptr));
            rs.launches++;
        }
        if (n_tf) HIP_TRY(swmi_launch_tfused(&ta, &xt, ctx->stream));
        if (whole_only && n_tf) rs.launches++;
        if (ctx->profiling && !ext_timing) HIP_TRY(hipEventRecord(ctx->ev[1], ctx->stream));
        if (n_res) HIP_TRY(swmi_launch_resident(&ta, &xa, ctx->stream));
        if (attempt == 0) b->timing.resident_pairs += (uint32_t)n_res;
        if (attempt == 0) b->timing.tfused_pairs += (uint32_t)n_tf;
        const bool split = rs.tb_split && !cells_exact && b->eff_mode == 1 && n_windows < 0xFFFFFFFFull;
        const bool sweep_only = ctx->scores_only != 0 && !cells_exact;
        if (sweep_only) {
            if ((rc = b->h_result.reserve(a_off + arena_cap * 4))) return rc;
            HIP_TRY(hipMemcpyAsync((uint8_t *)b->h_result.p + result_out_off(), res + result_out_off(), np * sizeof(PairOut),
                                   hipMemcpyDeviceToHost, ctx->stream));
        } else if (split) {
            ta.win_off = b->d_win_off.as<uint32_t>();
            ta.q_count = b->d_queue.as<uint32_t>();
            ta.q_items = (uint4 *)(b->d_queue.as<uint8_t>() + 256);
            ta.q_cap = (uint32_t)q_cap;
            if (attempt > 0 || whole_only) HIP_TRY(hipMemsetAsync(ta.q_count, 0, 4, ctx->stream));
            HIP_TRY(swmi_launch_traceback_split(&ta, (uint32_t)n_windows, ctx->stream));
        } else if (n_res + n_tf < np) {
            HIP_TRY(swmi_launch_traceback(&ta, ctx->stream, ext_timing ? ctx->ev[2] : nullptr, ext_timing ? ctx->ev[3] : nullptr));
        }
        const bool time_all = ctx->profiling == 1;
        if (time_all && !ext_timing) HIP_TRY(hipEventRecord(ctx->ev[3], ctx->stream));

        const uint64_t copy_words = std::min<uint64_t>(arena_cap, std::max<uint64_t>(256, np * ctx->arena_copy_wpp));
        const uint64_t copy_recs = std::min<uint64_t>(tab_cap, np * ctx->recs_per_pair_x16 / 16 + 64);
        if (!zc && !sweep_only) {
            if ((rc = b->h_result.reserve(a_off + arena_cap * 4))) return rc;
            HIP_TRY(hipMemcpyAsync(b->h_result.p, res, t_off + copy_recs * sizeof(AlnRec), hipMemcpyDeviceToHost, ctx->stream));
            HIP_TRY(hipMemcpyAsync((uint8_t *)b->h_result.p + a_off, res + a_off, copy_words * 4, hipMemcpyDeviceToHost, ctx->stream));
            if (time_all) HIP_TRY(hipEventRecord(ctx->ev[4], ctx->stream));
        }
        static const char *watchdog = getenv("SWMI_DEBUG_WATCHDOG");
        if (watchdog) {
            const auto w0 = std::chrono::steady_clock::now();
            while (hipStreamQuery(ctx->stream) == hipErrorNotReady)
                if (std::chrono::duration<double>(std::chrono::steady_clock::now() - w0).count() > atof(watchdog)) {
                    const volatile uint32_t *hm = (const volatile uint32_t *)b->h_result.p;
                    fprintf(stderr, "[swmi watchdog] launch still running after %s s; marks:", watchdog);
                    for (int k = 0; k < 12; k++) fprintf(stderr, " %08x", hm ? hm[k] : 0u);
                    fprintf(stderr, "\n");
                    fflush(stderr);
                    _exit(3);
                }
        }
        const auto c1 = std::chrono::steady_clock::now();
        {
            hipError_t q = hipErrorNotReady;
            while (ctx->spin_us > 0 && (q = hipStreamQuery(ctx->stream)) == hipErrorNotReady &&
                   std::chrono::duration<double, std::micro>(std::chrono::steady_clock::now() - c1).count() < (double)ctx->spin_us)
                __builtin_ia32_pause();
            if (q != hipSuccess && q != hipErrorNotReady) return fail(SWMI_ERR_HIP, "hipStreamQuery: %s", hipGetErrorString(q));
            if (q != hipSuccess) HIP_TRY(hipStreamSynchronize(ctx->stream));
        }
        const auto c2 = std::chrono::steady_clock::now();
        volatile uint32_t *giveup = zc ? (volatile uint32_t *)b->h_result.p + 1 : (volatile uint32_t *)ctx->h_err.p + 5;
        if (*giveup != 0u) {
            const uint32_t code = *giveup;
            *giveup = 0u;
            return fail(SWMI_ERR_HIP, "sw_tfused_kernel: internal wait abandoned (code %08x); results discarded", code);
        }
        if (*(volatile uint32_t *)ctx->h_err.p != 0u) {
            *(volatile uint32_t *)ctx->h_err.p = 0u;
            if (rs.one_wave_sweep)
                return fail(SWMI_ERR_HIP, "the sweep raised its error flag without the strip pipeline; results discarded");
            rs.one_wave_sweep = true;
            b->timing.strip_fallbacks++;
            return run_chunk(rs, work, lo, hi, cells_exact, outs);
        }
        rs.enqueue_us += std::chrono::duration<double, std::micro>(c1 - c0).count();
        rs.wait_us += std::chrono::duration<double, std::micro>(c2 - c1).count();
        if (ctx->profiling) {
            float ms = 0;
            if (attempt == 0 || whole_only) { HIP_TRY(hipEventElapsedTime(&ms, ctx->ev[0], ctx->ev[1])); rs.fill_ms += ms; }
            if (time_all) { HIP_TRY(hipEventElapsedTime(&ms, ctx->ev[ext_timing ? 2 : 1], ctx->ev[3])); rs.tb_ms += ms; }
            if (time_all && !zc) { HIP_TRY(hipEventElapsedTime(&ms, ctx->ev[3], ctx->ev[4])); rs.d2h_ms += ms; }
        }
        if ((rc = dump_traceback_diagnostics(b, ta, np, n_tf))) return rc;
        if (attempt == 0 && (rc = dump_fill_diagnostics(b, fa, np))) return rc;
        const uint8_t *h = (const uint8_t *)b->h_result.p;
        if (sweep_only) {
            outs.assign((const PairOut *)(h + result_out_off()), (const PairOut *)(h + result_out_off()) + np);
            for (size_t k = 0; k < np; k++) {
                PairOut &o = outs[k];
                if (o.score <= 0 && !(o.flags & SWMI_F_DEGENERATE)) {
                    const uint32_t pair = work[lo + k].pair;
                    o.score = 0; o.flags = SWMI_F_DEGENERATE;
                    o.n_cells = (uint64_t)b->read_desc[pair % b->n_reads].len * b->ref_desc[pair / b->n_reads].len;
                }
                o.flags &= SWMI_F_DEGENERATE;
            }
            return SWMI_OK;
        }
        ArenaHdr hdr_copy{};
        const ArenaHdr *hdr = (const ArenaHdr *)h;
        bool overflow;
        if (zc) {
            overflow = *(const volatile uint32_t *)h != 0u;
            if (overflow) {
                HIP_TRY(hipMemcpy(&hdr_copy, ta.hdr, sizeof hdr_copy, hipMemcpyDeviceToHost));
                hdr = &hdr_copy;
            }
        }
        const uint64_t hdr_words = zc && !overflow ? 0 : hdr->reserved & SWMI_HDR_WORD_MASK;
        const uint64_t hdr_recs = zc && !overflow ? 0 : hdr->reserved >> SWMI_HDR_WORD_BITS;
        if (!zc) overflow = hdr_words > arena_cap || hdr_recs > tab_cap;
        if (overflow) {
            if (zc) {
                saved_outs.resize(np * sizeof(PairOut));
                HIP_TRY(hipMemcpy(saved_outs.data(), res + result_out_off(), saved_outs.size(), hipMemcpyDeviceToHost));
            } else {
                saved_outs.assign(h + result_out_off(), h + result_out_off() + np * sizeof(PairOut));
            }
            for (size_t k = 0; k < np; k++) {
                PairOut &so = ((PairOut *)saved_outs.data())[k];
                so.flags &= ~SWMI_F_ARENA_OVF;
                if (split && !(so.flags & SWMI_F_DEGENERATE)) { so.n_cells = 0; so.flags &= ~SWMI_F_CELL_OVF; }
            }
            arena_cap = std::max<uint64_t>(arena_cap, hdr_words + 1024);
            tab_cap = std::max<uint64_t>(tab_cap, hdr_recs + 64);
            if (arena_cap >= SWMI_HDR_WORD_MASK || tab_cap >= (1ull << (64u - SWMI_HDR_WORD_BITS)) - 1ull)
                return fail(SWMI_ERR_UNSUPPORTED, "one launch would hold %llu alignment records in %llu arena dwords: lower max_workspace_bytes so that the batch runs in smaller launches",
                            (unsigned long long)tab_cap, (unsigned long long)arena_cap);
            ctx->arena_words_per_pair = std::max<uint64_t>(ctx->arena_words_per_pair, arena_cap / np + 1);
            ctx->recs_per_pair_x16 = std::max<uint64_t>(ctx->recs_per_pair_x16, tab_cap * 16 / np + 1);
            continue;
        }
        outs.assign((const PairOut *)(h + result_out_off()), (const PairOut *)(h + result_out_off()) + np);
        for (auto &o : outs) o.flags &= ~SWMI_F_ARENA_OVF;
        uint64_t n_rec = 0;
        if (zc) {
            for (auto &o : outs)
                if (!(o.flags & (SWMI_F_DEGENERATE | SWMI_F_CELL_OVF))) n_rec += o.n_cells;
        } else {
            n_rec = hdr_recs;
        }
        if (n_rec > tab_cap) return fail(SWMI_ERR_HIP, "more records than the table holds");
        const AlnRec *tab = (const AlnRec *)(h + t_off);
        const uint32_t *aw = (const uint32_t *)(h + a_off);
        if (!zc) {
            if (n_rec > copy_recs)
                HIP_TRY(hipMemcpy((uint8_t *)b->h_result.p + t_off + copy_recs * sizeof(AlnRec), res + t_off + copy_recs * sizeof(AlnRec),
                                  (n_rec - copy_recs) * sizeof(AlnRec), hipMemcpyDeviceToHost));
            if (hdr_words > copy_words)
                HIP_TRY(hipMemcpy((uint8_t *)b->h_result.p + a_off + copy_words * 4, res + a_off + copy_words * 4,
                                  (hdr_words - copy_words) * 4, hipMemcpyDeviceToHost));
            ctx->arena_copy_wpp = hdr_words * 5 / (4 * np) + 2;
            ctx->recs_per_pair_x16 = std::max<uint64_t>(ctx->recs_per_pair_x16, n_rec * 20 / np + 1);
        }
        if (rs.keep) {
            if ((rc = keep_chunk_records(rs, tab, n_rec, aw, arena_cap, lo))) return rc;
            rs.copyout_us += std::chrono::duration<double, std::micro>(std::chrono::steady_clock::now() - c2).count();
        }
        return SWMI_OK;
    }
}

static int settle_raw(swmi_batch *b) {
    if (!b->raw_ext) return SWMI_OK;
    const uint32_t *aw = b->raw_ext;
    const AlnRec *tab = b->rtab_ext;
    b->raw_ext = nullptr; b->rtab_ext = nullptr;
    uint64_t used = 0;
    for (uint64_t k = 0; k < b->raw_ext_records; k++)
        used = std::max(used, (((uint64_t)tab[k].off_hi << 32) | tab[k].off_lo) + rec_words(tab[k].n_ops, b->rec_strings));
    if (used > b->raw_ext_cap) return fail(SWMI_ERR_HIP, "record payloads overrun the arena");
    b->raw.assign(aw, aw + used);
    b->rtab.assign(tab, tab + b->raw_ext_records);
    if (b->raw_chunks.size() == 1) { b->raw_chunks[0].at = 0; b->raw_chunks[0].words = (size_t)used; b->raw_chunks[0].tab_at = 0; }
    return SWMI_OK;
}

static int ensure_indexed(swmi_batch *b) {
    if (b->indexed) return SWMI_OK;
    if (b->scores_only)
        return fail(SWMI_ERR_INVALID, "the batch was run with scores_only = 1: scores and totals only, no alignments");
    if (b->records_dropped)
        return fail(SWMI_ERR_INVALID, "this chunk's alignment records were not kept (option stream_keep_records = 0): scores, counts and totals only");
    const std::vector<Work> &work = b->work;
    struct Src { const AlnRec *tab; uint64_t n_rec; const uint32_t *arena; uint64_t words; const swmi_batch::RawChunk *c; };
    std::vector<Src> srcs;
    for (auto &c : b->raw_chunks) {
        if (b->raw_ext) srcs.push_back(Src{b->rtab_ext, b->raw_ext_records, b->raw_ext, b->raw_ext_cap, &c});
        else            srcs.push_back(Src{b->rtab.data() + c.tab_at, c.n_rec, b->raw.data() + c.at, c.words, &c});
    }
    auto wpos_of = [](const Src &sr, uint32_t out_id) -> uint64_t {
        return sr.c->wpos.empty() ? sr.c->lo + out_id : (out_id < sr.c->wpos.size() ? sr.c->wpos[out_id] : ~0ull);
    };
    for (auto &w : work) b->pairs[w.pair].count = 0;
    uint64_t total = 0;
    for (auto &sr : srcs) {
        for (uint64_t k = 0; k < sr.n_rec; k++) {
            const uint64_t wp = wpos_of(sr, sr.tab[k].out_id);
            if (wp >= work.size()) return fail(SWMI_ERR_HIP, "record of an unknown pair");
            b->pairs[work[wp].pair].count++;
        }
        total += sr.n_rec;
    }
    uint64_t run = 0;
    for (auto &w : work) { PairRes &pr = b->pairs[w.pair]; pr.first = run; run += pr.count; }
    if (run != total) return fail(SWMI_ERR_HIP, "record count mismatch");
    b->alns.assign(run, HostAln{});
    std::vector<uint32_t> cursor;
    const bool strict = b->params.tie_mode == SWMI_TIE_STRICT;
    for (auto &sr : srcs) {
        for (uint64_t k = 0; k < sr.n_rec; k++) {
            const AlnRec &e = sr.tab[k];
            const uint64_t wp = wpos_of(sr, e.out_id);
            PairRes &pr = b->pairs[work[wp].pair];
            const uint64_t off = ((uint64_t)e.off_hi << 32) | e.off_lo;
            if (off + rec_words(e.n_ops, b->rec_strings) > sr.words) return fail(SWMI_ERR_HIP, "record payload overruns the arena");
            HostAln a;
            a.rank = e.rank; a.begin = e.begin; a.end_i = e.end_i; a.end_j = e.end_j; a.n_ops = e.n_ops;
            a.rec = sr.arena + off;
            if (e.rank == SWMI_RANK_BY_CELL) {
                if (cursor.empty()) cursor.assign(work.size(), 0u);
                uint32_t &c = cursor[wp];
                if (c >= pr.count) return fail(SWMI_ERR_HIP, "more records than counted for a pair");
                b->alns[pr.first + c++] = a;
            } else {
                if (e.rank >= pr.count) return fail(SWMI_ERR_HIP, "record rank %u out of range", e.rank);
                b->alns[pr.first + e.rank] = a;
            }
        }
    }
    for (size_t wi = 0; wi < work.size(); wi++) {
        PairRes &pr = b->pairs[work[wi].pair];
        if (!(pr.flags & SWMI_PAIR_DEGENERATE) && pr.count != pr.n_cells)
            return fail(SWMI_ERR_HIP, "pair %u: %llu records for %llu max cells", work[wi].pair,
                        (unsigned long long)pr.count, (unsigned long long)pr.n_cells);
        if (!cursor.empty() && cursor[wi] > 1) {
            auto key = [strict](const HostAln &x) {
                return strict ? (((uint64_t)((uint32_t)x.end_i + (uint32_t)x.end_j)) << 32) | (uint32_t)x.end_j
                              : ((uint64_t)(uint32_t)x.end_i << 32) | (uint32_t)x.end_j;
            };
            std::sort(b->alns.begin() + pr.first, b->alns.begin() + pr.first + pr.count,
                      [&](const HostAln &x, const HostAln &y) { return key(x) < key(y); });
        }
        if (!cursor.empty() && cursor[wi] != 0)
            for (uint64_t k = 0; k < pr.count; k++) b->alns[pr.first + k].rank = (uint32_t)k;
        if (strict && pr.count > 1)
            std::stable_sort(b->alns.begin() + pr.first, b->alns.begin() + pr.first + pr.count,
                             [](const HostAln &x, const HostAln &y) { return x.begin < y.begin; });
    }
    if (!b->rec_strings) {
        b->str_at.resize(run);
        uint64_t chars = 0;
        for (uint64_t k = 0; k < run; k++) { b->alns[k].str_id = -1; b->str_at[k] = chars; chars += 2ull * (b->alns[k].n_ops + 1); }
        b->str_buf.resize(chars);
    }
    b->indexed = true;
    return SWMI_OK;
}

extern "C" int swmi_batch_run(swmi_ctx *ctx, swmi_batch *b, const swmi_params *p) {
    if (!ctx || !b || !p) return fail(SWMI_ERR_INVALID, "null argument");
    if (p->tie_mode != SWMI_TIE_SERIAL && p->tie_mode != SWMI_TIE_STRICT)
        return fail(SWMI_ERR_INVALID, "unknown tie_mode %d", p->tie_mode);
    if (p->types[0] == p->types[1] || p->types[0] == p->types[2] || p->types[1] == p->types[2])
        return fail(SWMI_ERR_UNSUPPORTED, "alignTypes a/i/d must be pairwise distinct");
    std::lock_guard<std::mutex> g(ctx->mu);
    static const bool host_dbg = getenv("SWMI_DEBUG_HOST") != nullptr;
    auto now = [] { return std::chrono::steady_clock::now(); };
    auto us = [](std::chrono::steady_clock::time_point a, std::chrono::steady_clock::time_point c) {
        return std::chrono::duration<double, std::micro>(c - a).count();
    };
    const auto h0 = now();
    {
        int cur = -1;
        if (hipGetDevice(&cur) != hipSuccess || cur != ctx->device) HIP_TRY(hipSetDevice(ctx->device));
    }
    b->params = *p;
    b->has_run = false;
    b->scores_only = ctx->scores_only != 0;

    const uint32_t n_refs = b->n_refs, n_reads = b->n_reads;
    const uint64_t n_pairs = (uint64_t)n_refs * n_reads;
    b->pairs.assign(n_pairs, PairRes{});
    b->alns.clear(); b->str_at.clear();
    b->raw.clear(); b->rtab.clear(); b->raw_chunks.clear(); b->indexed = false;
    b->raw_ext = nullptr; b->rtab_ext = nullptr;
    if (b->views_built || b->ref_view_ready.size() != n_refs) {
        b->ref_view_ready.assign(n_refs, 0);
        b->ref_sites.assign(n_refs, {});
        b->ref_degenerate.assign(n_refs, 0);
        b->views_built = false;
    }
    b->timing = swmi_timing{};

    b->eff_mode = (ctx->mode == 1 && (p->mismatch > 0 || p->gap > 0)) ? 2u : ctx->mode;
    if (ctx->tb_split < 0 && !ctx->scores_only && b->eff_mode == 1 && n_pairs >= 64 && n_pairs <= 256 &&
        (b->auto_choice < 0 || memcmp(&b->auto_params, p, sizeof(swmi_params)) != 0)) {
        std::vector<Work> sample;
        const uint64_t want = 48, stride = std::max<uint64_t>(1, n_pairs / want);
        for (uint64_t pi = stride / 2; pi < n_pairs && sample.size() < want; pi += stride) {
            const uint32_t m = b->read_desc[pi % n_reads].len, n = b->ref_desc[pi / n_reads].len;
            if (m == 0 || n == 0) continue;
            Work w;
            w.pair = (uint32_t)pi; w.cells = (uint64_t)m * n;
            w.dir_words = swmi_dir_words(m, n, 1); w.seam_words = swmi_seam_words(m, n);
            sample.push_back(w);
        }
        int choice = 1;
        if (!sample.empty()) {
            RunState rs0;
            rs0.ctx = ctx; rs0.b = b;
            rs0.tb_split = true;
            rs0.keep = false;
            std::vector<PairOut> o0;
            int rc = run_chunk(rs0, sample, 0, sample.size(), nullptr, o0);
            if (rc) return rc;
            uint64_t cells = 0, live = 0;
            for (auto &o : o0)
                if (!(o.flags & SWMI_F_DEGENERATE)) { cells += o.n_cells; live++; }
            if (live && cells * 100 >= (uint64_t)ctx->auto_ties_x100 * live) choice = 0;
            b->prep.valid = false;
            b->timing = swmi_timing{};
        }
        b->auto_choice = choice;
        b->auto_params = *p;
    }
    if (b->eff_mode == 0) {
        uint32_t max_n = 0, max_m = 0;
        for (const auto &d : b->ref_desc) max_n = std::max(max_n, d.len);
        for (const auto &d : b->read_desc) max_m = std::max(max_m, d.len);
        if (traceback_lds_bytes(0, path_bound(max_n, max_m, *p), max_m) > 160ull * 1024)
            b->eff_mode = (p->mismatch > 0 || p->gap > 0) ? 2u : 1u;
    }
    if (b->work_mode != (int)b->eff_mode || b->work_tfused != (ctx->tfused == 1)) {
        b->work_tfused = ctx->tfused == 1;
        b->work.clear();
        b->work.reserve(n_pairs);
        b->work_cells = 0;
        std::vector<uint32_t> ro(n_refs), qo(n_reads);
        std::iota(ro.begin(), ro.end(), 0u);
        std::iota(qo.begin(), qo.end(), 0u);
        std::stable_sort(ro.begin(), ro.end(), [&](uint32_t a, uint32_t c) { return b->ref_desc[a].len > b->ref_desc[c].len; });
        std::stable_sort(qo.begin(), qo.end(), [&](uint32_t a, uint32_t c) { return b->read_desc[a].len > b->read_desc[c].len; });
        const bool refs_uniform = n_refs && b->ref_desc[ro.front()].len == b->ref_desc[ro.back()].len;
        auto add = [&](uint32_t r, uint32_t q, uint32_t n, uint32_t m, uint64_t dw, uint64_t sw) {
            Work w;
            w.pair = r * n_reads + q;
            w.cells = (uint64_t)m * n;
            w.dir_words = dw; w.seam_words = sw;
            b->work_cells += w.cells;
            b->work.push_back(w);
        };
        const bool tf = ctx->tfused == 1;
        if (refs_uniform) {
            for (uint32_t q : qo) {
                const uint32_t m = b->read_desc[q].len;
                if (m == 0) continue;
                const uint32_t n = n_refs ? b->ref_desc[ro[0]].len : 0;
                if (n == 0) break;
                const uint64_t dw = swmi_dir_words(m, n, b->eff_mode, tf), sw = swmi_seam_words(m, n);
                for (uint32_t r : ro) add(r, q, n, m, dw, sw);
            }
        } else {
            uint32_t last_m = 0xFFFFFFFFu;
            uint64_t dw = 0, sw = 0;
            for (uint32_t r : ro) {
                const uint32_t n = b->ref_desc[r].len;
                if (n == 0) continue;
                last_m = 0xFFFFFFFFu;
                for (uint32_t q : qo) {
                    const uint32_t m = b->read_desc[q].len;
                    if (m == 0) continue;
                    if (m != last_m) { dw = swmi_dir_words(m, n, b->eff_mode, tf); sw = swmi_seam_words(m, n); last_m = m; }
                    add(r, q, n, m, dw, sw);
                }
            }
        }
        b->work_mode = (int)b->eff_mode;
    }
    const std::vector<Work> &work = b->work;
    const uint64_t total_cells = b->work_cells;
    const auto h1 = now();
    RunState rs;
    rs.ctx = ctx; rs.b = b;
    rs.tb_split = b->eff_mode == 1 &&
                  (ctx->tb_split == 1 || (ctx->tb_split < 0 && (work.size() < 64 || (work.size() <= 256 && b->auto_choice == 0 &&
                                                                                      memcmp(&b->auto_params, p, sizeof(swmi_params)) == 0))));
    b->tb_split_used = rs.tb_split;

    std::vector<PairOut> outs;
    std::vector<uint32_t> arena;
    std::vector<size_t> ovf;
    uint64_t dir_bytes = 0;

    size_t lo = 0;
    while (lo < work.size()) {
        uint64_t words = 0;
        size_t hi = lo;
        while (hi < work.size() && (hi == lo || (words + work[hi].dir_words) * 4 <= ctx->max_workspace_bytes)) {
            words += work[hi].dir_words;
            hi++;
        }
        dir_bytes += words * 4;
        rs.defer_copy = lo == 0 && hi == work.size();
        int rc = run_chunk(rs, work, lo, hi, nullptr, outs);
        rs.defer_copy = false;
        if (rc) return rc;
        for (size_t k = 0; k < hi - lo; k++) {
            PairRes &pr = b->pairs[work[lo + k].pair];
            pr.score = outs[k].score;
            pr.flags = (outs[k].flags & SWMI_F_DEGENERATE) ? SWMI_PAIR_DEGENERATE : 0u;
            pr.n_cells = outs[k].n_cells;
            if (outs[k].flags & SWMI_F_CELL_OVF) ovf.push_back(lo + k);
        }
        lo = hi;
    }

    const auto h2 = now();
    if (!ovf.empty()) {
        { int rc0 = settle_raw(b); if (rc0) return rc0; }
        std::vector<Work> w2;
        std::vector<uint64_t> exact;
        for (size_t pos : ovf) { w2.push_back(work[pos]); exact.push_back(b->pairs[work[pos].pair].n_cells); }
        size_t lo2 = 0;
        while (lo2 < w2.size()) {
            uint64_t words = 0;
            size_t hi2 = lo2;
            while (hi2 < w2.size() && (hi2 == lo2 || (words + w2[hi2].dir_words) * 4 <= ctx->max_workspace_bytes)) {
                words += w2[hi2].dir_words;
                hi2++;
            }
            int rc = run_chunk(rs, w2, lo2, hi2, &exact, outs);
            if (rc) return rc;
            swmi_batch::RawChunk &rc2 = b->raw_chunks.back();
            rc2.wpos.resize(hi2 - lo2);
            for (size_t k = 0; k < hi2 - lo2; k++) rc2.wpos[k] = (uint32_t)ovf[lo2 + k];
            for (size_t k = 0; k < hi2 - lo2; k++) b->pairs[w2[lo2 + k].pair].n_cells = outs[k].n_cells;
            for (size_t k = 0; k < hi2 - lo2; k++)
                if (outs[k].flags & SWMI_F_CELL_OVF)
                    return fail(SWMI_ERR_HIP, "cell list overflowed again on the exact-size re-run");
            lo2 = hi2;
        }
        b->timing.rerun_pairs = (uint32_t)ovf.size();
    }

    b->timing.fill_ms = rs.fill_ms; b->timing.traceback_ms = rs.tb_ms; b->timing.d2h_ms = rs.d2h_ms;
    b->timing.total_ms = rs.fill_ms + rs.tb_ms + rs.d2h_ms;
    b->timing.fill_launches = rs.launches;
    b->timing.cells = total_cells;
    b->timing.dir_bytes = dir_bytes;
    b->has_run = true;
    if (host_dbg)
        fprintf(stderr, "[swmi host] setup %.1f us, chunks (launch+wait+parse) %.1f us [prepare %.1f, its uploads %.1f, enqueue %.1f, wait %.1f, copy-out %.1f], grouping %.1f us\n",
                us(h0, h1), us(h1, h2), rs.prep_us, rs.prep_upload_us, rs.enqueue_us, rs.wait_us, rs.copyout_us, us(h2, now()));
    return SWMI_OK;
}

static void swmi_worker_loop(swmi_ctx *ctx) {
    for (;;) {
        int st = 0;
        for (int spin = 0; spin < 4000 && (st = ctx->job_state.load(std::memory_order_acquire)) != 1 && st != 3; ++spin)
            __builtin_ia32_pause();
        if (st != 1 && st != 3) {
            std::unique_lock<std::mutex> lk(ctx->job_mu);
            ctx->job_cv.wait(lk, [&] { const int v = ctx->job_state.load(); return v == 1 || v == 3; });
            st = ctx->job_state.load();
        }
        if (st == 3) return;
        const int rc = swmi_batch_run(ctx, ctx->job_batch, &ctx->job_params);
        ctx->job_rc = rc;
        ctx->job_err = rc ? swmi_last_error() : "";
        { std::lock_guard<std::mutex> lk(ctx->job_mu); ctx->job_state.store(2, std::memory_order_release); }
        ctx->job_cv.notify_all();
    }
}

extern "C" int swmi_batch_run_async(swmi_ctx *ctx, swmi_batch *b, const swmi_params *p) {
    if (!ctx || !b || !p) return fail(SWMI_ERR_INVALID, "null argument");
    if (ctx->job_state.load(std::memory_order_acquire) != 0)
        return fail(SWMI_ERR_INVALID, "a run is already in flight on this context: call swmi_batch_wait first");
    if (!ctx->worker.joinable()) ctx->worker = std::thread(swmi_worker_loop, ctx);
    ctx->job_batch = b;
    ctx->job_params = *p;
    { std::lock_guard<std::mutex> lk(ctx->job_mu); ctx->job_state.store(1, std::memory_order_release); }
    ctx->job_cv.notify_all();
    return SWMI_OK;
}

extern "C" int swmi_batch_wait(swmi_ctx *ctx) {
    if (!ctx) return fail(SWMI_ERR_INVALID, "null argument");
    int st = ctx->job_state.load(std::memory_order_acquire);
    if (st == 0) return fail(SWMI_ERR_INVALID, "no run in flight on this context");
    for (int spin = 0; spin < 20000 && st != 2; ++spin) {
        __builtin_ia32_pause();
        st = ctx->job_state.load(std::memory_order_acquire);
    }
    if (st != 2) {
        std::unique_lock<std::mutex> lk(ctx->job_mu);
        ctx->job_cv.wait(lk, [&] { return ctx->job_state.load() == 2; });
    }
    const int rc = ctx->job_rc;
    const std::string err = ctx->job_err;
    ctx->job_state.store(0, std::memory_order_release);
    if (rc) return fail(rc, "%s", err.c_str());
    return SWMI_OK;
}

extern "C" int swmi_batch_mode(const swmi_batch *b, int *mode) {
    if (!b || !mode) return fail(SWMI_ERR_INVALID, "null argument");
    if (!b->has_run) return fail(SWMI_ERR_INVALID, "batch has no results (run it first)");
    *mode = (int)b->eff_mode;
    return SWMI_OK;
}

extern "C" int swmi_batch_timing(const swmi_batch *b, swmi_timing *t) {
    if (!b || !t) return fail(SWMI_ERR_INVALID, "null argument");
    *t = b->timing;
    return SWMI_OK;
}

extern "C" int swmi_align_batch(swmi_ctx *ctx, const swmi_params *p,
                                const uint8_t *ref_bytes, const uint64_t *ref_off, uint32_t n_refs,
                                const uint8_t *read_bytes, const uint64_t *read_off, uint32_t n_reads,
                                swmi_batch **out) {
    int rc = swmi_batch_upload(ctx, ref_bytes, ref_off, n_refs, read_bytes, read_off, n_reads, out);
    if (rc) return rc;
    rc = swmi_batch_run(ctx, *out, p);
    if (rc) { swmi_batch_free(ctx, *out); *out = nullptr; }
    return rc;
}

extern "C" uint64_t swmi_batch_n_pairs(const swmi_batch *b) { return b ? (uint64_t)b->n_refs * b->n_reads : 0; }

static int check_pair(const swmi_batch *b, uint64_t pair) {
    if (!b) return fail(SWMI_ERR_INVALID, "batch is null");
    if (!b->has_run) return fail(SWMI_ERR_INVALID, "batch has no results (run it first)");
    if (pair >= (uint64_t)b->n_refs * b->n_reads) return fail(SWMI_ERR_RANGE, "pair %llu out of range", (unsigned long long)pair);
    return SWMI_OK;
}

extern "C" int swmi_pair_score(const swmi_batch *b, uint64_t pair, int32_t *score) {
    int rc = check_pair(b, pair);
    if (rc) return rc;
    if (score) *score = b->pairs[pair].score;
    return SWMI_OK;
}

extern "C" int swmi_pair_n_alignments(const swmi_batch *b, uint64_t pair, uint64_t *n, uint32_t *flags) {
    int rc = check_pair(b, pair);
    if (rc) return rc;
    if (b->scores_only && !(b->pairs[pair].flags & SWMI_PAIR_DEGENERATE))
        return fail(SWMI_ERR_INVALID, "the batch was run with scores_only = 1: the number of alignments was not computed");
    if (n) *n = b->pairs[pair].n_cells;
    if (flags) *flags = b->pairs[pair].flags;
    return SWMI_OK;
}

extern "C" int swmi_batch_pair_results(const swmi_batch *b, int32_t *scores, uint64_t *n_alignments, uint64_t n) {
    if (!b) return fail(SWMI_ERR_INVALID, "batch is null");
    if (!b->has_run) return fail(SWMI_ERR_INVALID, "batch has no results (run it first)");
    if (n != (uint64_t)b->n_refs * b->n_reads) return fail(SWMI_ERR_RANGE, "the batch has %llu pairs, not %llu",
                                                           (unsigned long long)b->n_refs * b->n_reads, (unsigned long long)n);
    if (b->scores_only && n_alignments)
        return fail(SWMI_ERR_INVALID, "the batch was run with scores_only = 1: pass n_alignments = NULL");
    for (uint64_t k = 0; k < n; k++) {
        if (scores) scores[k] = b->pairs[k].score;
        if (n_alignments) n_alignments[k] = b->pairs[k].n_cells;
    }
    return SWMI_OK;
}

static void materialise(swmi_batch *b, uint64_t pair, HostAln &a, uint64_t slot) {
    const uint32_t r = (uint32_t)(pair / b->n_reads), q = (uint32_t)(pair % b->n_reads);
    const uint8_t *ref;
    if (b->src_map) {
        auto it = b->src_cache.find(r);
        if (it == b->src_cache.end()) {
            it = b->src_cache.emplace(r, std::vector<uint8_t>()).first;
            swmi_io_read_record(b->src_map, b->src_recs[r], it->second);
        }
        ref = it->second.data();
    } else {
        ref = b->ref_bytes.data() + b->ref_off[r];
    }
    const uint8_t *read = b->read_bytes.data() + b->read_off[q];
    char *sr = b->str_buf.data() + b->str_at[slot], *sq = sr + a.n_ops + 1;
    sr[a.n_ops] = 0; sq[a.n_ops] = 0;
    int64_t i = a.end_i, j = a.end_j;
    const uint32_t *ops = a.rec;
    struct Lut { uint8_t nref, nread, roff[4], qoff[4], rgap[4], qgap[4]; };
    static const Lut *lut = [] {
        static Lut t[256];
        for (int v = 0; v < 256; v++) {
            Lut &L = t[v];
            L.nref = L.nread = 0;
            for (int k = 0; k < 4; k++) {
                const uint32_t op = (v >> (2 * k)) & 3u;
                const bool use_ref = op != SWMI_DIR_I, use_read = op != SWMI_DIR_D;
                L.roff[k] = L.nref; L.qoff[k] = L.nread;
                L.rgap[k] = use_ref ? 0 : 0xFF; L.qgap[k] = use_read ? 0 : 0xFF;
                L.nref += use_ref; L.nread += use_read;
            }
        }
        return t;
    }();
    uint32_t t = 0;
    while (t + 4 <= a.n_ops && i >= 4 && j >= 4) {
        const Lut &L = lut[(ops[t >> 4] >> (2 * (t & 15))) & 0xFFu];
        const uint32_t pos = a.n_ops - 1 - t;
        for (int k = 0; k < 4; k++) {
            const uint8_t rc = ref[j - 1 - L.roff[k]], qc = read[i - 1 - L.qoff[k]];
            sr[pos - k] = (char)((rc & ~L.rgap[k]) | ('_' & L.rgap[k]));
            sq[pos - k] = (char)((qc & ~L.qgap[k]) | ('_' & L.qgap[k]));
        }
        j -= L.nref; i -= L.nread;
        t += 4;
    }
    for (; t < a.n_ops; t++) {
        const uint32_t op = (ops[t >> 4] >> (2 * (t & 15))) & 3u;
        const uint32_t pos = a.n_ops - 1 - t;
        const bool use_ref = op != SWMI_DIR_I, use_read = op != SWMI_DIR_D;
        sr[pos] = use_ref ? (char)ref[j - 1] : '_';
        sq[pos] = use_read ? (char)read[i - 1] : '_';
        j -= use_ref; i -= use_read;
    }
    a.str_id = (int64_t)b->str_at[slot];
}

static const char EMPTY_STR[1] = {0};

extern "C" int swmi_pair_alignment(swmi_batch *b, uint64_t pair, uint64_t k,
                                   int32_t *begin, int32_t *end_i, int32_t *end_j,
                                   const char **ref_aln, const char **read_aln, uint32_t *len) {
    int rc = check_pair(b, pair);
    if (rc) return rc;
    if ((rc = ensure_indexed(b))) return rc;
    PairRes &pr = b->pairs[pair];
    if (k >= pr.n_cells) return fail(SWMI_ERR_RANGE, "alignment %llu out of range", (unsigned long long)k);
    if (pr.flags & SWMI_PAIR_DEGENERATE) {
        const uint32_t n = b->ref_desc[pair / b->n_reads].len;
        if (begin) *begin = 0;
        if (end_i) *end_i = (int32_t)(k / n) + 1;
        if (end_j) *end_j = (int32_t)(k % n) + 1;
        if (ref_aln) *ref_aln = EMPTY_STR;
        if (read_aln) *read_aln = EMPTY_STR;
        if (len) *len = 0;
        return SWMI_OK;
    }
    HostAln &a = b->alns[pr.first + k];
    if (begin) *begin = a.begin;
    if (end_i) *end_i = a.end_i;
    if (end_j) *end_j = a.end_j;
    if (len) *len = a.n_ops;
    if (b->rec_strings) {
        const uint32_t *sr = a.rec;
        if (ref_aln) *ref_aln = (const char *)sr;
        if (read_aln) *read_aln = (const char *)(sr + a.n_ops / 4u + 1u);
        return SWMI_OK;
    }
    if (a.str_id < 0) materialise(b, pair, a, pr.first + k);
    if (ref_aln) *ref_aln = b->str_buf.data() + a.str_id;
    if (read_aln) *read_aln = b->str_buf.data() + a.str_id + a.n_ops + 1;
    return SWMI_OK;
}

extern "C" int swmi_batch_materialise_all(swmi_batch *b, uint64_t *n_alignments, uint64_t *n_chars) {
    if (!b) return fail(SWMI_ERR_INVALID, "batch is null");
// ... 575 lines not shown
```

sparksmithwaterman_amd/csrc/swmi_kernels.hip:

```cpp
#include <hip/hip_runtime.h>
#include <hip/hip_ext.h>
#include <stdint.h>
#include <stdlib.h>
#include "swmi_device.h"
#include "swmi_emit.h"

#define WAVE 64
#ifndef SWMI_HELPER_SLEEP
#define SWMI_HELPER_SLEEP 8
#endif
#define BALLOT(pred) __builtin_amdgcn_ballot_w64(pred)
#define WAVE_SYNC() do { __builtin_amdgcn_fence(__ATOMIC_ACQ_REL, "wavefront"); __builtin_amdgcn_wave_barrier(); } while (0)

__device__ __forceinline__ int wave_shr1(int old, int src) {
    return __builtin_amdgcn_update_dpp(old, src, 0x138 , 0xf, 0xf, false);
}
__device__ __forceinline__ int wave_shr1_zero(int src) {
    return __builtin_amdgcn_update_dpp(0, src, 0x138 , 0xf, 0xf, true);
}

__device__ __forceinline__ int wave_max_i32(int v) {
#ifndef SWMI_NO_ASM
    asm volatile("s_nop 1\n\t"
                 "v_max_i32_dpp %0, %0, %0 row_shr:1 row_mask:0xf bank_mask:0xf\n\ts_nop 1\n\t"
// ... 623 lines not shown
    const SeqDesc qd = A.reads[pd.read_id];
    const uint32_t n_full = rd.len, m = qd.len;
    const StripGeom G = strip_geom<R>(m, n_full, 1u);
    const uint32_t col0 = COLS ? ci.col0 : 0u;
    const uint32_t g_lo = COLS ? ci.g_lo : 0u, g_hi = COLS ? ci.g_hi : G.n_ck;
    const bool last = g_hi >= G.n_ck;
    const uint32_t n = (last ? n_full : 16u * SWMI_CK_BLOCKS * g_hi) - col0;
    const uint32_t *__restrict__ refw = A.seqw + rd.boff + (col0 >> 2);
    const uint32_t *__restrict__ readw = A.seqw + qd.boff;
    const uint32_t lact = m >= G.rps ? WAVE : (m + R - 1) / R;
    const uint32_t lane_eff = lane < lact ? lane : 0x40000000u;
    const uint32_t T = n + lact - 1;
    const uint32_t nblk = last ? (T + 15u) / 16u : n / 16u;
    const uint32_t gm = (uint32_t)(-(int64_t)A.gap);
    const int one = 1;
    int pair_max = 0;

    const unsigned long long dbg_t0 = A.dbg ? __builtin_amdgcn_s_memtime() : 0ull;
    SweepState<R> S;
    build_profiles<R>(S.q, readw, lane * R, m, A.match, A.mismatch);
#pragma unroll
    for (int k = 0; k < R; ++k) {
        S.h[k] = 0; S.g[k] = 0; S.hp[k] = 0;
    }
    S.lmax = -1;
    const uint4 *__restrict__ refq = reinterpret_cast<const uint4 *>(refw);
    uint4 wnext = refq[0];
    S.rby = 0;
    S.rbx = wave_shr1((int)(1u << (wnext.x & 31u)), 0);

    uint32_t *__restrict__ wsp = A.dir + pd.dir_off + lane;
    auto close_window = [&](uint32_t g) {
        const int wm = wave_max_i32(lane < lact ? S.lmax : -1);
        if (lane == 0) A.dir[pd.dir_off + G.wmax_off + g] = (uint32_t)wm;
        pair_max = pair_max > wm ? pair_max : wm;
        S.lmax = -1;
    };
    for (uint32_t tb = 0; tb < nblk; ++tb) {
        const uint4 w = wnext;
        wnext = refq[tb + 1];
        const uint32_t tbg = tb + (col0 >> 4);
        if ((tbg % SWMI_CK_BLOCKS) == 0u) {
            const uint32_t g = tbg / SWMI_CK_BLOCKS;
            if (tb > 0u) {
                if (g > g_lo) close_window(g - 1u); else S.lmax = -1;
            }
            if (g >= g_lo) {
                uint32_t *__restrict__ ck = wsp + (uint64_t)g * (R + 2) * WAVE;
#pragma unroll
                for (int k = 0; k < R; ++k) ck[k * WAVE] = (uint32_t)S.h[k];
                ck[R * WAVE] = (uint32_t)wave_shr1_zero(S.g[R - 1]);
                ck[(R + 1) * WAVE] = (uint32_t)S.rby;
            }
        }
        const uint32_t t0 = 16u * tb;
#ifndef SWMI_NO_ASM
        if (t0 + 15u < n) {
            SweepStep4Asm<R>::run(S.h, S.g, S.hp, S.q, S.rbx, S.rby, w.x, w.y, one, gm, S.lmax);
            SweepStep4Asm<R>::run(S.h, S.g, S.hp, S.q, S.rbx, S.rby, w.y, w.z, one, gm, S.lmax);
            SweepStep4Asm<R>::run(S.h, S.g, S.hp, S.q, S.rbx, S.rby, w.z, w.w, one, gm, S.lmax);
            SweepStep4Asm<R>::run(S.h, S.g, S.hp, S.q, S.rbx, S.rby, w.w, wnext.x, one, gm, S.lmax);
        } else
#endif
        {
            sweep_tail_block<R>(S, w, wnext.x, t0, lane_eff, n, one, gm);
        }
    }
    {
        const uint32_t gl = (nblk - 1u + (col0 >> 4)) / SWMI_CK_BLOCKS;
        if (gl >= g_lo) close_window(gl);
    }
    if (lane != 0) return;
    if (A.dbg) {
        A.dbg[2 * pd.out_id] = (unsigned long long)__builtin_amdgcn_s_getreg((4 ) | (0 << 6) | (31 << 11)) |
                               ((unsigned long long)__builtin_amdgcn_s_getreg((20 ) | (0 << 6) | (31 << 11)) << 32);
        A.dbg[2 * pd.out_id + 1] = __builtin_amdgcn_s_memtime() - dbg_t0;
    }
    PairOut *o = &A.out[pd.out_id];
    if (COLS) {
        if (pair_max > 0) atomicMax(&o->score, pair_max);
        return;
    }
    PairOut v;
    if (pair_max <= 0) { v.score = 0; v.flags = SWMI_F_DEGENERATE; v.n_cells = (uint64_t)m * n_full; }
    else               { v.score = pair_max; v.flags = 0u; v.n_cells = 0; }
    *o = v;
}

template <bool COLS>
__device__ __forceinline__ void sweep_fast_dispatch(const FillArgs &A, const PairDesc pd, uint32_t lane, uint32_t m, const ColItem ci) {
    const uint32_t R = swmi_rows_per_lane(m);
    if (R == 1)      sweep_fast<1, COLS>(A, pd, lane, ci);
    else if (R == 2) sweep_fast<2, COLS>(A, pd, lane, ci);
    else if (R == 3) sweep_fast<3, COLS>(A, pd, lane, ci);
    else             sweep_fast<4, COLS>(A, pd, lane, ci);
}

template <bool ACGT, bool STRICT, int MODE>
__device__ __forceinline__ void fill_dispatch(const FillArgs &A, const PairDesc pd, uint32_t lane, uint32_t m) {
    const uint32_t R = swmi_rows_per_lane(m);
    if (R == 1)      fill_pair<1, ACGT, STRICT, false, MODE>(A, pd, lane);
    else if (R == 2) fill_pair<2, ACGT, STRICT, false, MODE>(A, pd, lane);
    else if (R == 3) fill_pair<3, ACGT, STRICT, false, MODE>(A, pd, lane);
    else if (m <= WAVE * SWMI_RMAX) fill_pair<SWMI_RMAX, ACGT, STRICT, false, MODE>(A, pd, lane);
    else             fill_pair<SWMI_RMAX, ACGT, STRICT, true, MODE>(A, pd, lane);
}

#define FILL_WAVES 4
template <int MODE>
__device__ __forceinline__ void fill_entry(const FillArgs &A) {
    const uint32_t pair = blockIdx.x * FILL_WAVES + (threadIdx.x >> 6);
    if (pair >= A.n_pairs) return;
    const uint32_t lane = threadIdx.x & 63u;
    if (pair == 0 && lane == 0 && A.hdr) { A.hdr->reserved = 0; A.hdr->pad = 0; }
    if (pair == 0 && lane == 0 && A.q_reset) *A.q_reset = 0u;
    const PairDesc pd = A.pairs[pair];
    if (MODE == SWMI_MODE_WINMAX && (pd.pad & SWMI_PAD_RESIDENT)) return;
    const SeqDesc rd = A.refs[pd.ref_id];
    const SeqDesc qd = A.reads[pd.read_id];
    if (MODE == SWMI_MODE_WINMAX && A.skip_multi && qd.len > WAVE * SWMI_RMAX) {
        if (lane == 0) { PairOut z; z.score = 0; z.flags = 0u; z.n_cells = 0; A.out[pd.out_id] = z; }
        return;
    }
    const bool acgt = rd.acgt && qd.acgt &&
                      SWMI_SCORES_FIT(A);
    if (MODE == SWMI_MODE_WINMAX && qd.len <= WAVE * SWMI_RMAX && (pd.pad & SWMI_PAD_COLS)) {
        if (lane == 0) { PairOut z; z.score = 0; z.flags = 0u; z.n_cells = 0; A.out[pd.out_id] = z; }
        return;
    }
    if (MODE == SWMI_MODE_WINMAX && acgt && qd.len <= WAVE * SWMI_RMAX && A.gap <= 0) {
        sweep_fast_dispatch<false>(A, pd, lane, qd.len, ColItem{0u, 0u, 0u, 0u});
        return;
    }
    if (MODE == SWMI_MODE_SCORE || MODE == SWMI_MODE_WINMAX) {
        if (acgt) fill_dispatch<true, false, MODE>(A, pd, lane, qd.len);
        else      fill_dispatch<false, false, MODE>(A, pd, lane, qd.len);
    } else if (acgt) {
        if (A.strict) fill_dispatch<true, true, MODE>(A, pd, lane, qd.len);
        else          fill_dispatch<true, false, MODE>(A, pd, lane, qd.len);
    } else {
        if (A.strict) fill_dispatch<false, true, MODE>(A, pd, lane, qd.len);
        else          fill_dispatch<false, false, MODE>(A, pd, lane, qd.len);
    }
}

extern "C" __global__ void __launch_bounds__(WAVE * FILL_WAVES)
sw_fill_kernel(const FillArgs A) { fill_entry<SWMI_MODE_FIELD>(A); }

extern "C" __global__ void __launch_bounds__(WAVE * FILL_WAVES)
sw_fill_score_kernel(const FillArgs A) { fill_entry<SWMI_MODE_SCORE>(A); }

extern "C" __global__ void __launch_bounds__(WAVE * FILL_WAVES) __attribute__((amdgpu_waves_per_eu(4, 4)))
sw_sweep_winmax_kernel(const FillArgs A) { fill_entry<SWMI_MODE_WINMAX>(A); }

extern "C" __global__ void __launch_bounds__(WAVE * FILL_WAVES)
sw_sweep_winmax_strips_kernel(const FillArgs A) {
    const uint32_t item = blockIdx.x * FILL_WAVES + (threadIdx.x >> 6);
    if (item >= A.n_strip_items) return;
    const uint32_t lane = threadIdx.x & 63u;
    const StripItem *it = A.strip_items + item;
    const PairDesc pd = A.pairs[it->pair];
    const SeqDesc rd = A.refs[pd.ref_id];
    const SeqDesc qd = A.reads[pd.read_id];
    const bool acgt = rd.acgt && qd.acgt &&
                      SWMI_SCORES_FIT(A);
    const uint32_t strip = __builtin_amdgcn_readfirstlane(it->strip);
    if (acgt) fill_pair<SWMI_RMAX, true, false, true, SWMI_MODE_WINMAX, true>(A, pd, lane, strip, it);
    else      fill_pair<SWMI_RMAX, false, false, true, SWMI_MODE_WINMAX, true>(A, pd, lane, strip, it);
}

extern "C" __global__ void __launch_bounds__(WAVE * FILL_WAVES)
sw_sweep_winmax_cols_kernel(const FillArgs A) {
    const uint32_t item = blockIdx.x * FILL_WAVES + (threadIdx.x >> 6);
    if (item >= A.n_col_items) return;
    const uint32_t lane = threadIdx.x & 63u;
    const ColItem ci = A.col_items[item];
    const PairDesc pd = A.pairs[ci.pair];
    sweep_fast_dispatch<true>(A, pd, lane, A.reads[pd.read_id].len, ci);
}

#define SWMI_TB_BLOCKS 16u
#define SWMI_TB_REFWIN_WORDS 96u
#define SWMI_TB_SLOTS 4u
#if SWMI_CK_BLOCKS > 2
#define SWMI_TB_WAVES 4u
#else
#define SWMI_TB_WAVES 8u
#endif

template <int R, bool STRICT>
__device__ __forceinline__ void replay_window_fast(const TraceArgs &A, const PairDesc pd, const uint32_t n, const uint32_t m,
                                                   const uint32_t *__restrict__ refw, const uint32_t *__restrict__ readw,
                                                   const uint32_t wlo, const uint32_t lane, uint32_t *__restrict__ lds_tile) {
    const uint32_t gm = (uint32_t)(-(int64_t)A.gap);
    const int one = 1;
    int h[R], g[R], hp[R], q[R];
    uint32_t acc[R];
    const uint32_t *__restrict__ ck = A.dir + pd.dir_off + (uint64_t)(wlo / SWMI_CK_BLOCKS) * (R + 2) * WAVE + lane;
    build_profiles<R>(q, readw, lane * R, m, A.match, A.mismatch);
#pragma unroll
    for (int k = 0; k < R; ++k) {
        h[k] = (int)ld_l2(ck + k * WAVE);
        hp[k] = (uint32_t)h[k] > gm ? (int)((uint32_t)h[k] - gm) : 0;
        g[k] = 0;
        acc[k] = 0;
    }
    const int nprev = (int)ld_l2(ck + R * WAVE);
    g[R - 1] = __builtin_amdgcn_update_dpp(0, nprev, 0x130 , 0xf, 0xf, true);
    const int rb_ck = (int)ld_l2(ck + (R + 1) * WAVE);
    const uint32_t lact = m >= WAVE * R ? WAVE : (m + R - 1) / R;
    const uint32_t T = n + lact - 1, nblk = (T + 15u) / 16u;
    const uint4 *__restrict__ refq = reinterpret_cast<const uint4 *>(refw);
    uint4 wv[SWMI_CK_BLOCKS + 1];
#pragma unroll
    for (uint32_t b = 0; b <= SWMI_CK_BLOCKS; ++b) wv[b] = refq[wlo + b];
    int rbx = wave_shr1((int)(1u << (wv[0].x & 31u)), rb_ck), rby = rb_ck;
#pragma unroll
    for (uint32_t b = 0; b < SWMI_CK_BLOCKS; ++b) {
        if (wlo + b >= nblk) break;
        const uint4 w = wv[b];
        DirStep4Asm<R, STRICT>::run(h, g, hp, acc, q, rbx, rby, w.x, w.y, one, gm);
        DirStep4Asm<R, STRICT>::run(h, g, hp, acc, q, rbx, rby, w.y, w.z, one, gm);
        DirStep4Asm<R, STRICT>::run(h, g, hp, acc, q, rbx, rby, w.z, w.w, one, gm);
        DirStep4Asm<R, STRICT>::run(h, g, hp, acc, q, rbx, rby, w.w, wv[b + 1].x, one, gm);
#pragma unroll
        for (int k = 0; k < R; ++k) lds_tile[(b * R + k) * WAVE + lane] = acc[k];
    }
}

template <int R, bool ACGT, bool STRICT, bool MULTI, bool DETECT>
__device__ __forceinline__ uint32_t replay_window(const TraceArgs &A, const PairDesc pd, const uint32_t n, const uint32_t m,
                                                  const uint32_t *__restrict__ refw, const uint32_t *__restrict__ readw,
                                                  const StripGeom G, const uint32_t s, const uint32_t wlo,
                                                  const uint32_t lane, uint32_t *__restrict__ lds_tile,
                                                  const int maxv, const uint32_t cnt_in, uint2 *__restrict__ cells, const uint32_t ccap) {
#ifndef SWMI_NO_ASM
    if constexpr (ACGT && !MULTI && !DETECT) {
        if (A.gap <= 0 && s == 0u) {
            replay_window_fast<R, STRICT>(A, pd, n, m, refw, readw, wlo, lane, lds_tile);
            return cnt_in;
        }
    }
#endif
    constexpr int BM = DETECT ? SWMI_MODE_DETECT : SWMI_MODE_REPLAY;
    FillState<R> S;
    S.thr = DETECT ? maxv : 0x7FFFFFFF; S.cnt = cnt_in; S.ev_prev = 0; S.events = 0; S.dbg_skip = false; S.lmax = -1;
    const uint32_t row0 = s * G.rps + lane * R;
    const uint32_t rows_left = m - s * G.rps;
    const uint32_t lact = rows_left >= G.rps ? WAVE : (rows_left + R - 1) / R;
    const uint32_t T = n + lact - 1;
    const uint32_t lane_eff = lane < lact ? lane : 0x40000000u;
    setup_rows<R, ACGT>(S, readw, row0, m, A.match, A.mismatch);
    const uint32_t *__restrict__ ck = A.dir + pd.dir_off + s * G.strip_words +
                                      (uint64_t)(wlo / SWMI_CK_BLOCKS) * (R + 2) * WAVE + lane;
#pragma unroll
    for (int k = 0; k < R; ++k) S.h[k] = (int)ld_l2(ck + k * WAVE);
    S.nprev = (int)ld_l2(ck + R * WAVE);
    S.rb = (int)ld_l2(ck + (R + 1) * WAVE);
    const int32_t *seam_in = nullptr;
    if (MULTI) seam_in = A.seam + pd.seam_off + (uint64_t)(s > 0 ? s - 1 : 0) * (n + 1);
    const bool reads_seam = MULTI && (s > 0);
    const uint32_t nblk = (T + 15u) / 16u;
    const uint4 *__restrict__ refq = reinterpret_cast<const uint4 *>(refw);
    uint4 wv[SWMI_CK_BLOCKS];
#pragma unroll
    for (uint32_t b = 0; b < SWMI_CK_BLOCKS; ++b) wv[b] = refq[wlo + b];
#pragma unroll
    for (uint32_t b = 0; b < SWMI_CK_BLOCKS; ++b) {
        const uint32_t tb = wlo + b;
        if (tb >= nblk) break;
        const uint4 w = wv[b];
        const uint32_t t0 = 16u * tb;
        int seamv = 0;
        if (reads_seam) {
            const uint32_t col = t0 + 1u + (lane & 15u);
            seamv = col <= n ? (int)ld_l2((const uint32_t *)seam_in + col) : 0;
        }
        const bool steady = (t0 + 1u >= lact) && (t0 + 15u < n);
        if (steady)
            fill_block16<R, ACGT, STRICT, MULTI, false, BM>(S, w, t0, lane, lane_eff, n, m, row0, A.gap, A.match, A.mismatch,
                                                            seamv, reads_seam, false, nullptr, cells, ccap);
        else
            fill_block16<R, ACGT, STRICT, MULTI, true, BM>(S, w, t0, lane, lane_eff, n, m, row0, A.gap, A.match, A.mismatch,
                                                           seamv, reads_seam, false, nullptr, cells, ccap);
        const int miss = (int)(t0 + 15u) - ((int)(lane + n) - 1);
#pragma unroll
        for (int k = 0; k < R; ++k) {
            uint32_t v = S.acc[k];
            if (miss > 0 && miss < 16) v <<= 2 * miss;
            lds_tile[(b * R + k) * WAVE + lane] = v;
        }
    }
    return S.cnt;
}

template <int R, bool MULTI, bool DETECT>
__device__ __forceinline__ uint32_t replay_dispatch(const TraceArgs &A, const PairDesc pd, uint32_t n, uint32_t m, bool acgt,
                                                    const uint32_t *__restrict__ refw, const uint32_t *__restrict__ readw,
                                                    const StripGeom G, uint32_t s, uint32_t wlo, uint32_t lane, uint32_t *lds_tile,
                                                    int maxv, uint32_t cnt_in, uint2 *__restrict__ cells, uint32_t ccap) {
    if (acgt) {
        if (A.strict) return replay_window<R, true, true, MULTI, DETECT>(A, pd, n, m, refw, readw, G, s, wlo, lane, lds_tile, maxv, cnt_in, cells, ccap);
        else          return replay_window<R, true, false, MULTI, DETECT>(A, pd, n, m, refw, readw, G, s, wlo, lane, lds_tile, maxv, cnt_in, cells, ccap);
    } else {
        if (A.strict) return replay_window<R, false, true, MULTI, DETECT>(A, pd, n, m, refw, readw, G, s, wlo, lane, lds_tile, maxv, cnt_in, cells, ccap);
        else          return replay_window<R, false, false, MULTI, DETECT>(A, pd, n, m, refw, readw, G, s, wlo, lane, lds_tile, maxv, cnt_in, cells, ccap);
// ... 445 lines not shown
        last = seq;
        __builtin_amdgcn_fence(__ATOMIC_ACQUIRE, "workgroup");
        const uint32_t flags = shared[4u + 4u * team], wlo = shared[5u + 4u * team], nq = shared[6u + 4u * team];
        const uint32_t s = flags >> 2;
        const uint32_t win = (flags & 2u) ? q - 1u : q;
        if (q < ts && win < nq) {
            uint32_t *__restrict__ base = ((flags & 1u) ? tiles + n_waves_all * (SWMI_CK_BLOCKS * SWMI_RMAX * WAVE) : tiles) +
                                          team * ts * (SWMI_CK_BLOCKS * SWMI_RMAX * WAVE);
            (void)replay_any<R, false, false>(A, pd, n, m, acgt, refw, readw, G, s, wlo + win * SWMI_CK_BLOCKS, lane,
                                       base + win * SWMI_CK_BLOCKS * R * WAVE, 0, 0u, nullptr, 0u);
            __builtin_amdgcn_fence(__ATOMIC_RELEASE, "workgroup");
            if (lane == 0) atomicAdd(const_cast<uint32_t *>(&shared[20u + team]), 1u);
        }
    }
}

template <int TMODE>
__device__ __forceinline__ void traceback_entry(const TraceArgs &A, uint32_t *lds_all) {
    const uint32_t wave = threadIdx.x >> 6;
    const uint32_t pair = blockIdx.x * FILL_WAVES + wave;
    if (pair >= A.n_pairs) return;
    const uint32_t lane = threadIdx.x & 63u;
    const uint32_t slot = blockIdx.y;
    uint32_t *tb_lds = lds_all + wave * (A.lds_words + A.lds_read_words + SWMI_TB_REFWIN_WORDS +
                                         (TMODE == 0 ? SWMI_TB_BLOCKS : SWMI_CK_BLOCKS) * SWMI_RMAX * WAVE);
    uint32_t *tile = tb_lds + A.lds_words + A.lds_read_words + SWMI_TB_REFWIN_WORDS;
    const PairDesc pd = A.pairs[pair];
    const PairOut po = A.out[pd.out_id];
    if (A.out_host && slot == 0 && lane == 0) A.out_host[pd.out_id] = po;
    if (po.flags & (SWMI_F_DEGENERATE | SWMI_F_CELL_OVF)) return;
    if (po.n_cells <= slot) return;
    const uint32_t R = swmi_rows_per_lane(A.reads[pd.read_id].len);
    if (R == 1)      traceback_pair<1, TMODE, false>(A, pd, po, lane, slot, SWMI_TB_SLOTS, tb_lds, tile, nullptr, 1u);
    else if (R == 2) traceback_pair<2, TMODE, false>(A, pd, po, lane, slot, SWMI_TB_SLOTS, tb_lds, tile, nullptr, 1u);
    else if (R == 3) traceback_pair<3, TMODE, false>(A, pd, po, lane, slot, SWMI_TB_SLOTS, tb_lds, tile, nullptr, 1u);
    else             traceback_pair<4, TMODE, false>(A, pd, po, lane, slot, SWMI_TB_SLOTS, tb_lds, tile, nullptr, 1u);
}

template <int R>
__device__ __forceinline__ uint32_t winmax_detect(const TraceArgs &A, const PairDesc pd, PairOut &po, const uint32_t lane,
                                                  const uint32_t wave, const uint32_t n_waves, const uint32_t ccap,
                                                  uint32_t *__restrict__ tiles, uint32_t *__restrict__ walker_lds,
                                                  const uint32_t per_walker, volatile uint32_t *__restrict__ shared) {
    const SeqDesc rd = A.refs[pd.ref_id];
    const SeqDesc qd = A.reads[pd.read_id];
    const uint32_t n = rd.len, m = qd.len;
    const uint32_t *__restrict__ refw = A.seqw + rd.boff;
    const uint32_t *__restrict__ readw = A.seqw + qd.boff;
    const bool acgt = rd.acgt && qd.acgt && SWMI_SCORES_FIT(A);
    const StripGeom G = strip_geom<R>(m, n, 1u);
    constexpr uint32_t WIN_WORDS = SWMI_CK_BLOCKS * SWMI_RMAX * WAVE;
    uint32_t ncand = 0, gc[SWMI_TB_SLOTS] = {0u, 0u, 0u, 0u};
    if (G.n_strips == 1u) {
        const uint32_t *__restrict__ wm = A.dir + pd.dir_off + G.wmax_off;
        for (uint32_t g0 = 0; g0 < G.n_ck; g0 += WAVE) {
            const uint32_t g = g0 + lane;
            const int wv = g < G.n_ck ? (int)wm[g] : -1;
            uint64_t cand = BALLOT(wv == po.score);
            while (cand) {
                const uint32_t gg = g0 + (uint32_t)__builtin_ctzll(cand);
                cand &= cand - 1ull;
                if (ncand == 0u) gc[0] = gg; else if (ncand == 1u) gc[1] = gg; else if (ncand == 2u) gc[2] = gg; else if (ncand == 3u) gc[3] = gg;
                ++ncand;
            }
        }
    }
    auto stage_ref = [&](uint32_t *__restrict__ dst, uint32_t wlo, uint32_t nwin) {
        const int clo = (int)(16u * wlo) - 63;
        const uint32_t cw0 = clo > 0 ? (uint32_t)clo >> 2 : 0u;
        const uint32_t cw1 = (16u * (wlo + nwin * SWMI_CK_BLOCKS) - 1u) >> 2;
        for (uint32_t x = cw0 + lane; x <= cw1 && x < (n + 3u) / 4u; x += WAVE) dst[x - cw0] = refw[x];
    };
    auto publish = [&](uint32_t cnt, uint32_t staged) {
        if (lane == 0) {
            po.n_cells = cnt;
            if (cnt > ccap) po.flags |= SWMI_F_CELL_OVF;
            A.out[pd.out_id] = po;
            if (A.out_host) A.out_host[pd.out_id] = po;
            shared[0] = cnt;
            shared[3] = staged;
        }
        if (lane < SWMI_TB_SLOTS) { shared[7u + 4u * lane] = 0u; shared[20u + lane] = 0u; }
        asm volatile("s_waitcnt vmcnt(0)" ::: "memory");
    };
    const uint64_t cbase = A.cells_off ? A.cells_off[pd.out_id] : (uint64_t)pd.out_id * A.cell_cap;
    uint2 *__restrict__ cells = const_cast<uint2 *>(A.cells) + cbase;

    const uint32_t seg = ccap / SWMI_TB_SLOTS;
    if (ncand >= 2u && ncand <= SWMI_TB_SLOTS && ncand <= n_waves && seg >= 1u) {
        const uint32_t nw = ncand, ts = n_waves / nw;
        if (wave < nw) {
            const uint32_t g = wave == 0u ? gc[0] : wave == 1u ? gc[1] : wave == 2u ? gc[2] : gc[3];
            const uint32_t nq0 = g + 1u < ts ? g + 1u : ts;
            const uint32_t wlo0 = (g + 1u - nq0) * SWMI_CK_BLOCKS;
            uint32_t *my = walker_lds + wave * per_walker;
            for (uint32_t w = lane; w < (m + 3u) / 4u; w += WAVE) my[A.lds_words + w] = readw[w];
            stage_ref(my + A.lds_words + A.lds_read_words, wlo0, nq0);
            const uint32_t c = replay_any<R, true, false>(A, pd, n, m, acgt, refw, readw, G, 0u, g * SWMI_CK_BLOCKS, lane,
                                                   tiles + wave * ts * WIN_WORDS + (nq0 - 1u) * SWMI_CK_BLOCKS * R * WAVE,
                                                   po.score, 0u, cells + wave * seg, seg);
            if (lane == 0) { shared[24u + wave] = c; shared[28u + wave] = wlo0; }
            asm volatile("s_waitcnt vmcnt(0)" ::: "memory");
        } else {
            const uint32_t team = (wave - nw) % nw, q = 1u + (wave - nw) / nw;
            const uint32_t g = team == 0u ? gc[0] : team == 1u ? gc[1] : team == 2u ? gc[2] : gc[3];
            const uint32_t nq0 = g + 1u < ts ? g + 1u : ts;
            if (q < nq0)
                (void)replay_any<R, false, false>(A, pd, n, m, acgt, refw, readw, G, 0u, (g - q) * SWMI_CK_BLOCKS, lane,
                                           tiles + team * ts * WIN_WORDS + (nq0 - 1u - q) * SWMI_CK_BLOCKS * R * WAVE,
                                           0, 0u, nullptr, 0u);
        }
        __syncthreads();
        bool one_each = true;
        for (uint32_t w = 0; w < nw; ++w) one_each = one_each && shared[24u + w] == 1u;
        if (one_each) {
            if (wave == 0) {
                uint2 c = make_uint2(0, 0);
                if (lane < nw) { c.x = ld_l2(&cells[lane * seg].x); c.y = ld_l2(&cells[lane * seg].y); }
                if (lane < nw) cells[lane] = c;
                publish(nw, 1u);
            }
            __syncthreads();
            return wave < nw ? shared[28u + wave] : 0xFFFFFFFFu;
        }
        __syncthreads();
    }

    const bool pre = ncand == 1u;
    const uint32_t nq0 = gc[0] + 1u < n_waves ? gc[0] + 1u : n_waves;
    const uint32_t wlo0 = (gc[0] + 1u - nq0) * SWMI_CK_BLOCKS;
    if (wave == 0) {
        if (n_waves == 1u) {
            for (uint32_t w = lane; w < (m + 3u) / 4u; w += WAVE) walker_lds[A.lds_words + w] = readw[w];
            if (pre) stage_ref(walker_lds + A.lds_words + A.lds_read_words, wlo0, nq0);
        }
        const uint32_t cnt = detect_cells<R, false>(A, pd, po, lane, pre ? tiles + (nq0 - 1u) * SWMI_CK_BLOCKS * R * WAVE : tiles);
        publish(cnt, (pre && cnt == 1u) ? 1u : 0u);
    } else {
        if (wave < SWMI_TB_SLOTS)
            for (uint32_t w = lane; w < (m + 3u) / 4u; w += WAVE) walker_lds[wave * per_walker + A.lds_words + w] = readw[w];
        if (wave == n_waves - 1u)
            for (uint32_t w = lane; w < (m + 3u) / 4u; w += WAVE) walker_lds[A.lds_words + w] = readw[w];
        if (pre) {
            if (wave < nq0)
                (void)replay_any<R, false, false>(A, pd, n, m, acgt, refw, readw, G, 0u, wlo0 + (wave - 1u) * SWMI_CK_BLOCKS, lane,
                                           tiles + (wave - 1u) * SWMI_CK_BLOCKS * R * WAVE, 0, 0u, nullptr, 0u);
            if (wave == n_waves - 1u) stage_ref(walker_lds + A.lds_words + A.lds_read_words, wlo0, nq0);
        }
    }
    __syncthreads();
    return (pre && wave == 0) ? wlo0 : 0xFFFFFFFFu;
}

extern "C" __global__ void __launch_bounds__(WAVE * SWMI_TB_WAVES) __attribute__((amdgpu_waves_per_eu(4, 4)))
sw_traceback_winmax_kernel(const TraceArgs A) {
    extern __shared__ uint32_t wm_lds[];
    const uint32_t pair = blockIdx.x;
    if (pair >= A.n_pairs) return;
    const uint32_t wave = threadIdx.x >> 6, lane = threadIdx.x & 63u;
    const PairDesc pd = A.pairs[pair];
    PairOut po = A.out[pd.out_id];
    if (finish_pair(A, pd, po) && wave == 0 && lane == 0) A.out[pd.out_id] = po;
    if (po.flags & (SWMI_F_DEGENERATE | SWMI_F_DONE)) {
        if (A.out_host && wave == 0 && lane == 0) A.out_host[pd.out_id] = po;
        return;
    }
    const uint32_t n_waves = blockDim.x >> 6;
    const uint32_t per_walker = A.lds_words + A.lds_read_words + SWMI_TB_REFWIN_WORDS;
    constexpr uint32_t WIN_WORDS = SWMI_CK_BLOCKS * SWMI_RMAX * WAVE;
    uint32_t *shared = wm_lds;
    uint32_t *tiles = wm_lds + 32;
    const uint32_t R = swmi_rows_per_lane(A.reads[pd.read_id].len);
    const uint32_t ccap = A.cells_cap ? A.cells_cap[pd.out_id] : A.cell_cap;
    const uint32_t tile_sets = A.pad2 ? 2u : 1u;
    uint32_t *tiles2 = A.pad2 ? tiles + n_waves * WIN_WORDS : nullptr;
    uint32_t *walker_lds0 = tiles + tile_sets * n_waves * WIN_WORDS;
    if (!swmi_common_pair(A, A.refs[pd.ref_id], A.reads[pd.read_id])) {
        if (wave == 0) {
            uint32_t c;
            if (R == 1)      c = detect_cells<1>(A, pd, po, lane, tiles);
            else if (R == 2) c = detect_cells<2>(A, pd, po, lane, tiles);
            else if (R == 3) c = detect_cells<3>(A, pd, po, lane, tiles);
            else             c = detect_cells<4>(A, pd, po, lane, tiles);
            if (lane == 0) {
                po.n_cells = c;
                if (c > ccap) po.flags |= SWMI_F_CELL_OVF;
                A.out[pd.out_id] = po;
                if (A.out_host) A.out_host[pd.out_id] = po;
                shared[0] = c;
            }
            asm volatile("s_waitcnt vmcnt(0)" ::: "memory");
        }
        __syncthreads();
        const uint32_t c = shared[0];
        uint32_t nwr = c < SWMI_TB_SLOTS ? c : SWMI_TB_SLOTS;
        if (nwr > n_waves) nwr = n_waves;
        if (c > ccap || wave >= nwr) return;
        po.n_cells = c;
        uint32_t *lds = walker_lds0 + wave * per_walker;
        uint32_t *tile = tiles + wave * WIN_WORDS;
        if (R == 1)      traceback_pair<1, 1, false>(A, pd, po, lane, wave, nwr, lds, tile, nullptr, 1u);
        else if (R == 2) traceback_pair<2, 1, false>(A, pd, po, lane, wave, nwr, lds, tile, nullptr, 1u);
        else if (R == 3) traceback_pair<3, 1, false>(A, pd, po, lane, wave, nwr, lds, tile, nullptr, 1u);
        else             traceback_pair<4, 1, false>(A, pd, po, lane, wave, nwr, lds, tile, nullptr, 1u);
        return;
    }
    uint32_t pre_wlo;
    if (R == 1)      pre_wlo = winmax_detect<1>(A, pd, po, lane, wave, n_waves, ccap, tiles, walker_lds0, per_walker, shared);
    else if (R == 2) pre_wlo = winmax_detect<2>(A, pd, po, lane, wave, n_waves, ccap, tiles, walker_lds0, per_walker, shared);
    else if (R == 3) pre_wlo = winmax_detect<3>(A, pd, po, lane, wave, n_waves, ccap, tiles, walker_lds0, per_walker, shared);
    else             pre_wlo = winmax_detect<4>(A, pd, po, lane, wave, n_waves, ccap, tiles, walker_lds0, per_walker, shared);
    const uint32_t cnt = shared[0];
    if (shared[3] != 1u) pre_wlo = 0xFFFFFFFFu;
    if (cnt > ccap || cnt == 0u) return;
    po.n_cells = cnt;
    uint32_t nw = cnt < SWMI_TB_SLOTS ? cnt : SWMI_TB_SLOTS;
    if (nw > n_waves) nw = n_waves;
    const uint32_t ts = n_waves / nw;
    if (ts == 1u) {
        if (wave >= nw) return;
        uint32_t *lds = walker_lds0 + wave * per_walker;
        uint32_t *tile = tiles + wave * WIN_WORDS;
        if (R == 1)      traceback_pair<1, 1, false, false>(A, pd, po, lane, wave, nw, lds, tile, nullptr, 1u, pre_wlo, true);
        else if (R == 2) traceback_pair<2, 1, false, false>(A, pd, po, lane, wave, nw, lds, tile, nullptr, 1u, pre_wlo, true);
        else if (R == 3) traceback_pair<3, 1, false, false>(A, pd, po, lane, wave, nw, lds, tile, nullptr, 1u, pre_wlo, true);
        else             traceback_pair<4, 1, false, false>(A, pd, po, lane, wave, nw, lds, tile, nullptr, 1u, pre_wlo, true);
        return;
    }
    if (wave < nw) {
        uint32_t *lds = walker_lds0 + wave * per_walker;
        uint32_t *tile = tiles + wave * ts * WIN_WORDS;
        uint32_t *tile2 = tiles2 ? tiles2 + wave * ts * WIN_WORDS : nullptr;
        if (R == 1)      traceback_pair<1, 1, true, false>(A, pd, po, lane, wave, nw, lds, tile, shared, ts, pre_wlo, true, nullptr, tile2);
        else if (R == 2) traceback_pair<2, 1, true, false>(A, pd, po, lane, wave, nw, lds, tile, shared, ts, pre_wlo, true, nullptr, tile2);
        else if (R == 3) traceback_pair<3, 1, true, false>(A, pd, po, lane, wave, nw, lds, tile, shared, ts, pre_wlo, true, nullptr, tile2);
        else             traceback_pair<4, 1, true, false>(A, pd, po, lane, wave, nw, lds, tile, shared, ts, pre_wlo, true, nullptr, tile2);
    } else {
        if (R == 1)      coop_helper<1>(A, pd, lane, wave, nw, ts, n_waves, tiles, shared);
        else if (R == 2) coop_helper<2>(A, pd, lane, wave, nw, ts, n_waves, tiles, shared);
        else if (R == 3) coop_helper<3>(A, pd, lane, wave, nw, ts, n_waves, tiles, shared);
        else             coop_helper<4>(A, pd, lane, wave, nw, ts, n_waves, tiles, shared);
    }
}

extern "C" __global__ void __launch_bounds__(WAVE * FILL_WAVES)
sw_traceback_kernel(const TraceArgs A) {
    extern __shared__ uint32_t tb_lds[];
    traceback_entry<0>(A, tb_lds);
}

extern "C" __global__ void __launch_bounds__(WAVE * FILL_WAVES)
sw_traceback_replay_kernel(const TraceArgs A) {
    extern __shared__ uint32_t tb_lds[];
    traceback_entry<1>(A, tb_lds);
}

#define SWMI_SPLIT_WAVES 4u

extern "C" __global__ void __launch_bounds__(WAVE * SWMI_SPLIT_WAVES)
sw_detect_windows_kernel(const TraceArgs A) {
    extern __shared__ uint32_t dw_lds[];
    const uint32_t wave = threadIdx.x >> 6, lane = threadIdx.x & 63u;
    const uint32_t item = blockIdx.x * SWMI_SPLIT_WAVES + wave;
    const uint32_t n_items = A.win_off[A.n_pairs];
    if (item >= n_items) return;
    uint32_t lo = 0, hi = A.n_pairs;
    while (hi - lo > 1u) {
        const uint32_t mid = (lo + hi) >> 1;
        if (A.win_off[mid] <= item) lo = mid; else hi = mid;
    }
    const uint32_t pair = lo, wloc = item - A.win_off[pair];
    const PairDesc pd = A.pairs[pair];
    PairOut po = A.out[pd.out_id];
    if (finish_pair(A, pd, po) && wloc == 0u && lane == 0) A.out[pd.out_id] = po;
    if (po.flags & (SWMI_F_DEGENERATE | SWMI_F_DONE)) return;
    const SeqDesc rd = A.refs[pd.ref_id];
    const SeqDesc qd = A.reads[pd.read_id];
    const uint32_t n = rd.len, m = qd.len;
    const uint32_t R = swmi_rows_per_lane(m);
    const uint64_t wblocks = ((uint64_t)n + 63u + 15u) / 16u;
    const uint32_t n_ck = (uint32_t)((wblocks + SWMI_CK_BLOCKS - 1u) / SWMI_CK_BLOCKS);
    const uint32_t strip = wloc / n_ck, g = wloc - strip * n_ck;
    const uint64_t wmax_off = (uint64_t)n_ck * (R + 2) * WAVE;
    const uint64_t strip_words = wmax_off + (uint64_t)((n_ck + 63u) & ~63u);
    if ((int)A.dir[pd.dir_off + strip * strip_words + wmax_off + g] != po.score) return;

    constexpr uint32_t WIN_WORDS = SWMI_CK_BLOCKS * SWMI_RMAX * WAVE;
    uint32_t *tile = dw_lds + wave * (WIN_WORDS + 2u * SWMI_DETECT_LCAP);
    uint2 *found = reinterpret_cast<uint2 *>(tile + WIN_WORDS);
    const uint32_t *__restrict__ refw = A.seqw + rd.boff;
    const uint32_t *__restrict__ readw = A.seqw + qd.boff;
    const bool acgt = rd.acgt && qd.acgt && SWMI_SCORES_FIT(A);
    uint32_t cnt;
    if (R == 1)      { const StripGeom G = strip_geom<1>(m, n, 1u); cnt = replay_any<1, true>(A, pd, n, m, acgt, refw, readw, G, strip, g * SWMI_CK_BLOCKS, lane, tile, po.score, 0u, found, SWMI_DETECT_LCAP); }
    else if (R == 2) { const StripGeom G = strip_geom<2>(m, n, 1u); cnt = replay_any<2, true>(A, pd, n, m, acgt, refw, readw, G, strip, g * SWMI_CK_BLOCKS, lane, tile, po.score, 0u, found, SWMI_DETECT_LCAP); }
    else if (R == 3) { const StripGeom G = strip_geom<3>(m, n, 1u); cnt = replay_any<3, true>(A, pd, n, m, acgt, refw, readw, G, strip, g * SWMI_CK_BLOCKS, lane, tile, po.score, 0u, found, SWMI_DETECT_LCAP); }
    else             { const StripGeom G = strip_geom<4>(m, n, 1u); cnt = replay_any<4, true>(A, pd, n, m, acgt, refw, readw, G, strip, g * SWMI_CK_BLOCKS, lane, tile, po.score, 0u, found, SWMI_DETECT_LCAP); }
    if (cnt == 0u) return;
    WAVE_SYNC();
    const uint64_t cbase = A.cells_off ? A.cells_off[pd.out_id] : (uint64_t)pd.out_id * A.cell_cap;
    const uint32_t ccap = A.cells_cap ? A.cells_cap[pd.out_id] : A.cell_cap;
    unsigned long long base = 0;
    uint32_t qbase = 0;
    const uint32_t have = cnt < SWMI_DETECT_LCAP ? cnt : SWMI_DETECT_LCAP;
    if (lane == 0) {
        base = atomicAdd((unsigned long long *)&A.out[pd.out_id].n_cells, (unsigned long long)cnt);
        const bool fits = cnt <= SWMI_DETECT_LCAP && base + cnt <= (unsigned long long)ccap;
        if (fits) {
            qbase = atomicAdd(A.q_count, have);
            if (qbase + have > A.q_cap) qbase = 0xFFFFFFFFu;
        } else {
            qbase = 0xFFFFFFFFu;
        }
        if (qbase == 0xFFFFFFFFu) atomicOr(&A.out[pd.out_id].flags, SWMI_F_CELL_OVF);
    }
    base = ((unsigned long long)(uint32_t)__builtin_amdgcn_readfirstlane((int)(base >> 32)) << 32) |
           (uint32_t)__builtin_amdgcn_readfirstlane((int)(uint32_t)base);
    qbase = (uint32_t)__builtin_amdgcn_readfirstlane((int)qbase);
    if (qbase == 0xFFFFFFFFu) return;
    uint2 *__restrict__ cells = const_cast<uint2 *>(A.cells) + cbase;
    for (uint32_t c = lane; c < have; c += WAVE) {
        const uint2 cell = found[c];
        cells[base + c] = cell;
        A.q_items[qbase + c] = make_uint4(pair, cell.x, cell.y, 0u);
    }
}

extern "C" __global__ void __launch_bounds__(WAVE * SWMI_SPLIT_WAVES)
sw_walk_items_kernel(const TraceArgs A) {
    extern __shared__ uint32_t wi_lds[];
    const uint32_t wave = threadIdx.x >> 6, lane = threadIdx.x & 63u;
    const uint32_t gw = blockIdx.x * SWMI_SPLIT_WAVES + wave, n_waves = gridDim.x * SWMI_SPLIT_WAVES;
    if (A.out_host)
        for (uint32_t p = gw * WAVE + lane; p < A.n_pairs; p += n_waves * WAVE) A.out_host[p] = A.out[p];
    uint32_t n_items = *A.q_count;
    if (n_items > A.q_cap) n_items = A.q_cap;
    constexpr uint32_t WIN_WORDS = SWMI_CK_BLOCKS * SWMI_RMAX * WAVE;
    const uint32_t per_wave = A.lds_words + A.lds_read_words + SWMI_TB_REFWIN_WORDS + WIN_WORDS;
    uint32_t *lds = wi_lds + wave * per_wave;
    uint32_t *tile = lds + A.lds_words + A.lds_read_words + SWMI_TB_REFWIN_WORDS;
    for (uint32_t it = gw; it < n_items; it += n_waves) {
        const uint4 item = A.q_items[it];
        const PairDesc pd = A.pairs[item.x];
        PairOut po = A.out[pd.out_id];
        if (po.flags & (SWMI_F_DEGENERATE | SWMI_F_CELL_OVF)) continue;
        const uint32_t R = swmi_rows_per_lane(A.reads[pd.read_id].len);
        if (R == 1)      traceback_pair<1, 1, false>(A, pd, po, lane, 0u, 1u, lds, tile, nullptr, 1u, 0xFFFFFFFFu, false, &item);
        else if (R == 2) traceback_pair<2, 1, false>(A, pd, po, lane, 0u, 1u, lds, tile, nullptr, 1u, 0xFFFFFFFFu, false, &item);
        else if (R == 3) traceback_pair<3, 1, false>(A, pd, po, lane, 0u, 1u, lds, tile, nullptr, 1u, 0xFFFFFFFFu, false, &item);
        else             traceback_pair<4, 1, false>(A, pd, po, lane, 0u, 1u, lds, tile, nullptr, 1u, 0xFFFFFFFFu, false, &item);
        WAVE_SYNC();
    }
}

__device__ __forceinline__ uint32_t wave_scan_add_u32(uint32_t v) {
#define SWMI_DPP_ADD(ctrl, rmask, bmask)                                                     \
    { const uint32_t o_ = (uint32_t)__builtin_amdgcn_update_dpp(0, (int)v, ctrl, rmask, bmask, true); v += o_; }
    SWMI_DPP_ADD(0x111, 0xf, 0xf)
    SWMI_DPP_ADD(0x112, 0xf, 0xf)
    SWMI_DPP_ADD(0x114, 0xf, 0xf)
    SWMI_DPP_ADD(0x118, 0xf, 0xf)
    SWMI_DPP_ADD(0x142, 0xa, 0xf)
    SWMI_DPP_ADD(0x143, 0xc, 0xf)
#undef SWMI_DPP_ADD
    return v;
}

template <int R, bool STRICT>
__device__ __forceinline__ void resident_pair(const TraceArgs &A, const ResidentArgs &X, const PairDesc pd, const uint32_t lane, uint32_t *__restrict__ lds) {
    const SeqDesc rd = A.refs[pd.ref_id];
    const SeqDesc qd = A.reads[pd.read_id];
    const uint32_t n = rd.len, m = qd.len;
    const uint32_t *__restrict__ refw = A.seqw + rd.boff;
    const uint32_t *__restrict__ readw = A.seqw + qd.boff;
    const uint32_t lact = (m + R - 1) / R;
    const uint32_t lane_eff = lane < lact ? lane : 0x40000000u;
    const uint32_t T = n + lact - 1, nblk = (T + 15u) / 16u, n_ck = (nblk + SWMI_CK_BLOCKS - 1u) / SWMI_CK_BLOCKS;
    uint32_t *field = lds;
    uint32_t *wmaxs = field + nblk * R * WAVE;
    uint2 *cells = reinterpret_cast<uint2 *>(wmaxs + ((n_ck + 1u) & ~1u));
    uint32_t *opsb = reinterpret_cast<uint32_t *>(cells + X.res_cell_cap);
    uint32_t *refc = opsb + WAVE * X.res_ops_words;
    uint32_t *readc = refc + (n + 3u) / 4u + 1u;
    uint32_t *scratch = readc + (m + 3u) / 4u + 1u;
    for (uint32_t w = lane; w < (n + 3u) / 4u; w += WAVE) refc[w] = refw[w];
    for (uint32_t w = lane; w < (m + 3u) / 4u; w += WAVE) readc[w] = readw[w];
    const uint4 *__restrict__ refq = reinterpret_cast<const uint4 *>(refw);

    int pair_max = 0;
    {
        const uint32_t gm = (uint32_t)(-(int64_t)A.gap);
        const int one = 1;
        SweepState<R> S;
        build_profiles<R>(S.q, readw, lane * R, m, A.match, A.mismatch);
#pragma unroll
        for (int k = 0; k < R; ++k) { S.h[k] = 0; S.g[k] = 0; S.hp[k] = 0; }
// ... 33 lines not shown
        if (lane == 0) { A.out[pd.out_id] = po; if (A.out_host) A.out_host[pd.out_id] = po; }
        return;
    }
    WAVE_SYNC();

    uint32_t ncell;
    {
        FillState<R> S;
        S.thr = pair_max; S.cnt = 0; S.ev_prev = 0; S.events = 0; S.dbg_skip = false; S.lmax = -1;
        setup_rows<R, true>(S, readw, lane * R, m, A.match, A.mismatch);
        uint4 wnext = refq[0];
        for (uint32_t tb = 0; tb < nblk; ++tb) {
            const uint4 w = wnext;
            wnext = refq[tb + 1];
            const uint32_t t0 = 16u * tb;
            const bool steady = (t0 + 1u >= lact) && (t0 + 15u < n);
            const bool hot = (int)wmaxs[tb / SWMI_CK_BLOCKS] == pair_max;
            if (hot) {
                if (steady) fill_block16<R, true, STRICT, false, false, SWMI_MODE_DETECT>(S, w, t0, lane, lane_eff, n, m, lane * R, A.gap, A.match, A.mismatch,
                                                                                          0, false, false, nullptr, cells, X.res_cell_cap);
                else        fill_block16<R, true, STRICT, false, true, SWMI_MODE_DETECT>(S, w, t0, lane, lane_eff, n, m, lane * R, A.gap, A.match, A.mismatch,
                                                                                         0, false, false, nullptr, cells, X.res_cell_cap);
            } else {
                if (steady) fill_block16<R, true, STRICT, false, false, SWMI_MODE_REPLAY>(S, w, t0, lane, lane_eff, n, m, lane * R, A.gap, A.match, A.mismatch,
                                                                                          0, false, false, nullptr, nullptr, 0u);
                else        fill_block16<R, true, STRICT, false, true, SWMI_MODE_REPLAY>(S, w, t0, lane, lane_eff, n, m, lane * R, A.gap, A.match, A.mismatch,
                                                                                         0, false, false, nullptr, nullptr, 0u);
            }
            const int miss = (int)(t0 + 15u) - ((int)(lane + n) - 1);
#pragma unroll
            for (int k = 0; k < R; ++k) {
                uint32_t v = S.acc[k];
                if (miss > 0 && miss < 16) v <<= 2 * miss;
                field[(tb * R + k) * WAVE + lane] = v;
            }
        }
        ncell = S.cnt;
    }
    po.score = pair_max; po.flags = SWMI_F_DONE | (ncell > X.res_cell_cap ? SWMI_F_CELL_OVF : 0u); po.n_cells = ncell;
    if (lane == 0) { A.out[pd.out_id] = po; if (A.out_host) A.out_host[pd.out_id] = po; }
    if (ncell > X.res_cell_cap || ncell == 0u) return;
    WAVE_SYNC();

    const uint8_t *ref_b = reinterpret_cast<const uint8_t *>(refc);
    const uint8_t *read_b = reinterpret_cast<const uint8_t *>(readc);
    const uint32_t umat = (uint32_t)A.match, umis = (uint32_t)A.mismatch, ugap = (uint32_t)A.gap;
    const uint32_t max_ops = 16u * X.res_ops_words;
    for (uint32_t base = 0; base < ncell; base += WAVE) {
        const bool mine = base + lane < ncell;
        const uint2 c0 = mine ? cells[base + lane] : make_uint2(0u, 0u);
        uint32_t i = c0.x, j = c0.y, score = (uint32_t)pair_max, nops = 0, cur = 0;
        int begin = 0;
        bool active = mine;
        uint32_t *my_ops = opsb + lane * X.res_ops_words;
        while (BALLOT(active)) {
            if (active) {
                const uint32_t rho = i - 1u, l = rho / R, k = rho - l * R;
                const uint32_t t = j - 1u + l;
                const uint32_t dw = field[((t >> 4) * R + k) * WAVE + l];
                const uint32_t rc = ref_b[j - 1u], qc = read_b[i - 1u];
                const uint32_t d = (dw >> (2u * (15u - (t & 15u)))) & 3u;
                const bool isA = (d & 1u) != 0u, isI = d == 2u;
                begin = (int)j;
                score -= isA ? (rc == qc ? umat : umis) : ugap;
                const uint32_t op = isA ? SWMI_DIR_A : (isI ? SWMI_DIR_I : SWMI_DIR_D);
                cur |= op << (2u * (nops & 15u));
                ++nops;
                if ((nops & 15u) == 0u) { if (nops <= max_ops) my_ops[(nops >> 4) - 1u] = cur; cur = 0; }
                i -= (isA || isI) ? 1u : 0u;
                j -= (isA || !isI) ? 1u : 0u;
                active = (int)score > 0 && i != 0u && j != 0u;
            }
        }
        if ((nops & 15u) != 0u && nops <= max_ops) my_ops[nops >> 4] = cur;
        WAVE_SYNC();
        const uint32_t opw = A.raw ? 0u : (nops + 15u) / 16u;
        const uint32_t words = mine ? swmi_payload_words(nops, A.raw != nullptr) : 0u;
        const uint32_t incl = wave_scan_add_u32(words);
        const uint32_t total = (uint32_t)__builtin_amdgcn_readlane((int)incl, 63);
        const uint32_t nhere = ncell - base < WAVE ? ncell - base : WAVE;
        unsigned long long off;
        uint32_t rslot;
        const bool fits = swmi_reserve(A, lane, total, nhere, off, rslot);
        const bool too_long = BALLOT(mine && nops > max_ops) != 0ull;
        if (fits && !too_long) {
            if (mine) {
                uint32_t *dst = A.arena + off + (incl - words);
                swmi_write_rec(A, rslot + lane, pd.out_id, SWMI_RANK_BY_CELL, begin, c0.x, c0.y, nops, off + (incl - words));
                for (uint32_t w = 0; w < opw; ++w) dst[w] = my_ops[w];
            }
            if (A.raw) {
                const uint8_t *__restrict__ raw_ref = A.raw + A.raw_off[pd.ref_id];
                const uint8_t *__restrict__ raw_read = A.raw + A.raw_off[A.raw_reads_at + pd.read_id];
                for (uint32_t a = 0; a < nhere; ++a) {
                    const uint32_t na = (uint32_t)__builtin_amdgcn_readlane((int)nops, (int)a);
                    const uint32_t at = (uint32_t)__builtin_amdgcn_readlane((int)(incl - words), (int)a);
                    const uint32_t ai = (uint32_t)__builtin_amdgcn_readlane((int)c0.x, (int)a);
                    const uint32_t aj = (uint32_t)__builtin_amdgcn_readlane((int)c0.y, (int)a);
                    swmi_emit_strings(A.arena + off + at, SwmiOpsPacked{opsb + a * X.res_ops_words},
                                      na, ai, aj, raw_ref, raw_read, lane, scratch);
                }
            }
        } else if (lane == 0) {
            atomicOr(&A.out[pd.out_id].flags, SWMI_F_ARENA_OVF);
            if (A.ovf_host) *A.ovf_host = 1u;
        }
        WAVE_SYNC();
    }
}

extern "C" __global__ void __launch_bounds__(WAVE * FILL_WAVES)
sw_resident_pairs_kernel(const TraceArgs A, const ResidentArgs X) {
    extern __shared__ uint32_t rp_lds[];
    const uint32_t wave = threadIdx.x >> 6, lane = threadIdx.x & 63u;
    const uint32_t item = blockIdx.x * FILL_WAVES + wave;
    if (item >= X.n_res) return;
    const PairDesc pd = A.pairs[X.res_items[item]];
    uint32_t *lds = rp_lds + wave * X.res_lds_words;
    const uint32_t R = swmi_rows_per_lane(A.reads[pd.read_id].len);
    if (A.strict) {
        if (R == 1)      resident_pair<1, true>(A, X, pd, lane, lds);
        else if (R == 2) resident_pair<2, true>(A, X, pd, lane, lds);
        else if (R == 3) resident_pair<3, true>(A, X, pd, lane, lds);
        else             resident_pair<4, true>(A, X, pd, lane, lds);
    } else {
        if (R == 1)      resident_pair<1, false>(A, X, pd, lane, lds);
        else if (R == 2) resident_pair<2, false>(A, X, pd, lane, lds);
        else if (R == 3) resident_pair<3, false>(A, X, pd, lane, lds);
        else             resident_pair<4, false>(A, X, pd, lane, lds);
    }
}

extern "C" hipError_t swmi_launch_resident(const TraceArgs *a, const ResidentArgs *x, hipStream_t st) {
    if (x->n_res == 0) return hipSuccess;
    static const bool attr = [] { (void)hipFuncSetAttribute(reinterpret_cast<const void *>(sw_resident_pairs_kernel),
                                                            hipFuncAttributeMaxDynamicSharedMemorySize, 160 * 1024); return true; }();
    (void)attr;
    hipLaunchKernelGGL(sw_resident_pairs_kernel, dim3((x->n_res + FILL_WAVES - 1) / FILL_WAVES), dim3(WAVE * FILL_WAVES),
                       (size_t)FILL_WAVES * x->res_lds_words * sizeof(uint32_t), st, *a, *x);
    return hipGetLastError();
}

static size_t spread_lds(uint32_t n_groups) {
    static const int on = getenv("SWMI_LDS_SPREAD") ? atoi(getenv("SWMI_LDS_SPREAD")) : 1;
    if (!on || n_groups == 0 || n_groups > 4u * 256u) return 0;
    const uint32_t per_cu = (n_groups + 255u) / 256u;
    return ((size_t)(160u * 1024u) / (per_cu + 1u) / 1024u + 1u) * 1024u;
}
template <class K>
static void allow_big_lds(K kernel) {
    (void)hipFuncSetAttribute(reinterpret_cast<const void *>(kernel), hipFuncAttributeMaxDynamicSharedMemorySize, 160 * 1024);
}

extern "C" hipError_t swmi_launch_fill(const FillArgs *a, hipStream_t st, hipEvent_t ev_start, hipEvent_t ev_stop) {
    if (a->n_pairs == 0) return hipSuccess;
    static const bool attrs = [] {
        allow_big_lds(sw_fill_kernel); allow_big_lds(sw_fill_score_kernel); allow_big_lds(sw_sweep_winmax_kernel);
        allow_big_lds(sw_sweep_winmax_strips_kernel); allow_big_lds(sw_sweep_winmax_cols_kernel);
        return true;
    }();
    (void)attrs;
    const dim3 grid((a->n_pairs + FILL_WAVES - 1) / FILL_WAVES), block(WAVE * FILL_WAVES);
    const size_t lds = spread_lds(grid.x);
    if (a->mode == 0)      hipLaunchKernelGGL(sw_fill_kernel, grid, block, lds, st, *a);
    else if (a->mode == 1) {
        if (ev_start && ev_stop && !(a->skip_multi && a->n_strip_items) && !a->n_col_items) {
            hipExtLaunchKernelGGL(sw_sweep_winmax_kernel, grid, block, (uint32_t)lds, st, ev_start, ev_stop, 0u, *a);
            return hipGetLastError();
        }
        hipLaunchKernelGGL(sw_sweep_winmax_kernel, grid, block, a->n_col_items || a->n_strip_items ? 0 : lds, st, *a);
        if (a->skip_multi && a->n_strip_items) {
            const uint32_t g = (a->n_strip_items + FILL_WAVES - 1) / FILL_WAVES;
            hipLaunchKernelGGL(sw_sweep_winmax_strips_kernel, dim3(g), block, spread_lds(g), st, *a);
        }
        if (a->n_col_items) {
            const uint32_t g = (a->n_col_items + FILL_WAVES - 1) / FILL_WAVES;
            hipLaunchKernelGGL(sw_sweep_winmax_cols_kernel, dim3(g), block, spread_lds(g), st, *a);
        }
    }
    else                   hipLaunchKernelGGL(sw_fill_score_kernel, grid, block, lds, st, *a);
    return hipGetLastError();
}

extern "C" hipError_t swmi_launch_traceback_split(const TraceArgs *a, uint32_t n_windows, hipStream_t st) {
    if (a->n_pairs == 0) return hipSuccess;
    const size_t win = (size_t)SWMI_CK_BLOCKS * SWMI_RMAX * WAVE;
    const size_t det_words = SWMI_SPLIT_WAVES * (win + 2u * SWMI_DETECT_LCAP);
    if (n_windows)
        hipLaunchKernelGGL(sw_detect_windows_kernel, dim3((n_windows + SWMI_SPLIT_WAVES - 1) / SWMI_SPLIT_WAVES), dim3(WAVE * SWMI_SPLIT_WAVES),
                           det_words * sizeof(uint32_t), st, *a);
    const size_t per_wave = (size_t)a->lds_words + a->lds_read_words + SWMI_TB_REFWIN_WORDS + win;
    uint32_t groups = (a->q_cap + SWMI_SPLIT_WAVES - 1) / SWMI_SPLIT_WAVES;
    if (groups > 2048u) groups = 2048u;
    if (groups < 1u) groups = 1u;
    hipLaunchKernelGGL(sw_walk_items_kernel, dim3(groups), dim3(WAVE * SWMI_SPLIT_WAVES), SWMI_SPLIT_WAVES * per_wave * sizeof(uint32_t), st, *a);
    return hipGetLastError();
}

extern "C" hipError_t swmi_launch_traceback(const TraceArgs *a, hipStream_t st, hipEvent_t ev_start, hipEvent_t ev_stop) {
    if (a->n_pairs == 0) return hipSuccess;
    const size_t tile = (size_t)(a->mode == 0 ? SWMI_TB_BLOCKS : SWMI_CK_BLOCKS) * SWMI_RMAX * WAVE;
    const size_t per_wave = (size_t)a->lds_words + a->lds_read_words + SWMI_TB_REFWIN_WORDS + tile;
    const dim3 block(WAVE * FILL_WAVES);
    if (a->mode == 1) {
        static int forced = getenv("SWMI_TB_WAVES") ? atoi(getenv("SWMI_TB_WAVES")) : 0;
        static int big = getenv("SWMI_TB_BIG") ? atoi(getenv("SWMI_TB_BIG")) : 10000;
        const uint32_t n_waves = forced ? (uint32_t)forced : (a->n_pairs <= 512u ? SWMI_TB_WAVES : a->n_pairs <= (uint32_t)big ? 4u : 1u);
        const size_t n_walkers = n_waves < SWMI_TB_SLOTS ? n_waves : SWMI_TB_SLOTS;
        const size_t tiles = (size_t)n_waves * SWMI_CK_BLOCKS * SWMI_RMAX * WAVE;
        size_t words = 32 + tiles + n_walkers * ((size_t)a->lds_words + a->lds_read_words + SWMI_TB_REFWIN_WORDS);
        static const int spec_opt = getenv("SWMI_TB_SPEC") ? atoi(getenv("SWMI_TB_SPEC")) : 1;
        TraceArgs t = *a;
        t.pad2 = (spec_opt && (spec_opt == 2 || a->n_pairs <= 384u) && n_waves > 1u && (words + tiles) * sizeof(uint32_t) <= 160u * 1024u) ? 1u : 0u;
        if (t.pad2) words += tiles;
        if (ev_start && ev_stop)
            hipExtLaunchKernelGGL(sw_traceback_winmax_kernel, dim3(a->n_pairs), dim3(WAVE * n_waves), (uint32_t)(words * sizeof(uint32_t)), st, ev_start, ev_stop, 0u, t);
        else
            hipLaunchKernelGGL(sw_traceback_winmax_kernel, dim3(a->n_pairs), dim3(WAVE * n_waves), words * sizeof(uint32_t), st, t);
    } else {
        const dim3 grid((a->n_pairs + FILL_WAVES - 1) / FILL_WAVES, SWMI_TB_SLOTS);
        if (a->mode == 0) hipLaunchKernelGGL(sw_traceback_kernel, grid, block, per_wave * FILL_WAVES * sizeof(uint32_t), st, *a);
        else              hipLaunchKernelGGL(sw_traceback_replay_kernel, grid, block, per_wave * FILL_WAVES * sizeof(uint32_t), st, *a);
    }
    return hipGetLastError();
}
```

Measured before the change: 2421.

## Add specialised fast sweep and fixed-R traceback kernels for uniform ACGT batches

Adds a host-side check that routes plain winmax batches to specialised kernels when every pair is ACGT-only, the scoring is in range, and there are no strip, column, resident or fused items. The fast sweep kernel calls a direct sweep dispatch with higher waves-per-EU. Traceback kernels are templated on a compile-time rows-per-lane, skip the non-common-pair path, and are capped at 56 VGPRs. The aim is to cut dispatch overhead and raise occupancy, at the cost of possible register spills, more code size and extra host-side prep scanning.

```diff
diff --git a/include/swmi.h b/include/swmi.h
--- a/include/swmi.h
+++ b/include/swmi.h
@@ -63,6 +63,7 @@
     uint32_t tfused_pairs;
 } swmi_timing;
 int  swmi_batch_timing(const swmi_batch *b, swmi_timing *t);
+int  swmi_batch_fast_kernels(const swmi_batch *b, uint32_t *sweeps, uint32_t *tracebacks);
 int  swmi_batch_mode(const swmi_batch *b, int *mode);
 
 #define SWMI_PAIR_DEGENERATE 0x1u
diff --git a/sparksmithwaterman_amd/_capi.py b/sparksmithwaterman_amd/_capi.py
--- a/sparksmithwaterman_amd/_capi.py
+++ b/sparksmithwaterman_amd/_capi.py
@@ -52,6 +52,7 @@
     ("swmi_batch_free", None, [_P, _P]),
     ("swmi_batch_timing", C.c_int, [_P, C.POINTER(Timing)]),
     ("swmi_batch_mode", C.c_int, [_P, C.POINTER(C.c_int)]),
+    ("swmi_batch_fast_kernels", C.c_int, [_P, C.POINTER(C.c_uint32), C.POINTER(C.c_uint32)]),
     ("swmi_batch_n_pairs", C.c_uint64, [_P]),
     ("swmi_pair_score", C.c_int, [_P, C.c_uint64, C.POINTER(C.c_int32)]),
     ("swmi_pair_n_alignments", C.c_int, [_P, C.c_uint64, _u64p, C.POINTER(C.c_uint32)]),
diff --git a/sparksmithwaterman_amd/aligner.py b/sparksmithwaterman_amd/aligner.py
--- a/sparksmithwaterman_amd/aligner.py
+++ b/sparksmithwaterman_amd/aligner.py
@@ -95,6 +95,11 @@
         v = C.c_int()
         check(self._lib.swmi_batch_mode(self._h, C.byref(v)))
         return v.value
+
+    def fast_kernels(self):
+        s, t = C.c_uint32(), C.c_uint32()
+        check(self._lib.swmi_batch_fast_kernels(self._h, C.byref(s), C.byref(t)))
+        return s.value, t.value
 
     def score(self, pair):
         v = C.c_int32()
diff --git a/sparksmithwaterman_amd/csrc/swmi_api.cpp b/sparksmithwaterman_amd/csrc/swmi_api.cpp
--- a/sparksmithwaterman_amd/csrc/swmi_api.cpp
+++ b/sparksmithwaterman_amd/csrc/swmi_api.cpp
@@ -22,8 +22,8 @@
 #include "swmi_device.h"
 #include "swmi_io_internal.h"
 
-extern "C" hipError_t swmi_launch_fill(const FillArgs *a, hipStream_t st, hipEvent_t ev_start, hipEvent_t ev_stop);
-extern "C" hipError_t swmi_launch_traceback(const TraceArgs *a, hipStream_t st, hipEvent_t ev_start, hipEvent_t ev_stop);
+extern "C" hipError_t swmi_launch_fill(const FillArgs *a, hipStream_t st, hipEvent_t ev_start, hipEvent_t ev_stop, uint32_t fast);
+extern "C" hipError_t swmi_launch_traceback(const TraceArgs *a, hipStream_t st, hipEvent_t ev_start, hipEvent_t ev_stop, uint32_t fast_r);
 extern "C" hipError_t swmi_launch_traceback_split(const TraceArgs *a, uint32_t n_windows, hipStream_t st);
 extern "C" hipError_t swmi_launch_resident(const TraceArgs *a, const ResidentArgs *x, hipStream_t st);
 extern "C" hipError_t swmi_launch_tfused(const TraceArgs *a, const TFusedArgs *x, hipStream_t st);
@@ -120,6 +120,7 @@
     bool ext_events = false;
     int tfused = -1;
     int resident = -1;
+    int fast_kernels = 1;
     int scores_only = 0;
     int stream_keep_records = 1;
     int device_strings = 1;
@@ -177,6 +178,7 @@
     bool views_built = false;
     bool tb_split_used = false;
     bool acgt_known = false;
+    uint32_t fast_sweeps = 0, fast_tracebacks = 0;
     PinnedBuf h_result;
     swmi_params params{};
     bool has_run = false;
@@ -203,6 +205,9 @@
         uint32_t res_lds_words = 0, res_ops_words = 0;
         int resident_opt = -1;
         int tfused_opt = -1;
+        int fast_opt = -1;
+        bool fast_sweep = false;
+        uint32_t fast_r = 0;
         size_t n_tf = 0;
         uint32_t tf_max_m = 0, tf_max_n = 0, tf_max_path = 0;
         bool exact = false, scores_only = false;
@@ -340,6 +345,9 @@
     } else if (!strcmp(name, "resident")) {
         if (value < -1 || value > 1) return fail(SWMI_ERR_INVALID, "resident must be -1 (automatic), 0 or 1");
         ctx->resident = (int)value;
+    } else if (!strcmp(name, "fast_kernels")) {
+        if (value < 0 || value > 1) return fail(SWMI_ERR_INVALID, "fast_kernels must be 0 (never) or 1 (automatic)");
+        ctx->fast_kernels = (int)value;
     } else if (!strcmp(name, "scores_only")) {
         ctx->scores_only = value != 0;
     } else if (!strcmp(name, "stream_keep_records")) {
@@ -550,6 +558,8 @@
     std::vector<uint32_t> tf_items;
     size_t n_tf = 0;
     uint32_t tf_max_m = 0, tf_max_n = 0, tf_max_path = 0;
+    bool fast_sweep = false;
+    uint32_t fast_r = 0;
     const uint32_t res_cell_cap = SWMI_RES_CELL_CAP;
     swmi_batch::Prep &pr = b->prep;
     const auto p0 = std::chrono::steady_clock::now();
@@ -557,13 +567,14 @@
                           memcmp(&pr.params, &b->params, sizeof(swmi_params)) == 0 && b->pairs_dev_ptr == b->d_pairs.p &&
                           b->pairs_on_device.size() == np * sizeof(PairDesc) && pr.col_chunks_opt == ctx->col_chunks &&
                           pr.reverse_strips == (ctx->dbg_reverse_strips != 0) && pr.resident_opt == ctx->resident &&
-                          pr.tfused_opt == ctx->tfused && pr.exact == (cells_exact != nullptr) && pr.scores_only == (ctx->scores_only != 0);
+                          pr.tfused_opt == ctx->tfused && pr.fast_opt == ctx->fast_kernels && pr.exact == (cells_exact != nullptr) && pr.scores_only == (ctx->scores_only != 0);
     if (prepared) {
         dir_words = pr.dir_words; seam_words = pr.seam_words; max_path = pr.max_path; max_read = pr.max_read;
         n_strip_items = pr.n_strip_items; n_col_items = pr.n_col_items; n_windows = pr.n_windows;
         seam_priv_words = pr.seam_priv_words; n_strip_chunks = pr.n_strip_chunks;
         n_res = pr.n_res; res_lds_words = pr.res_lds_words; res_ops_words = pr.res_ops_words;
         n_tf = pr.n_tf; tf_max_m = pr.tf_max_m; tf_max_n = pr.tf_max_n; tf_max_path = pr.tf_max_path;
+        fast_sweep = pr.fast_sweep; fast_r = pr.fast_r;
     } else {
     const swmi_params &P = b->params;
     const bool cols_possible = b->eff_mode == 1 && P.match > 0 && P.gap < 0 && P.mismatch <= 0 &&
@@ -587,7 +598,9 @@
         }
     const bool tf_possible = b->eff_mode == 1 && !cells_exact && !ctx->scores_only && ctx->tfused == 1 &&
                              P.match > 0 && P.match <= 7 && P.mismatch >= -8 && P.mismatch <= P.match && P.gap < 0 && P.gap >= -64;
-    if ((cols_possible || res_maybe || tf_possible) && !b->acgt_known) {
+    const bool fast_possible = b->eff_mode == 1 && ctx->fast_kernels != 0 && P.gap <= 0 &&
+                               P.match >= -8 && P.match <= 7 && P.mismatch >= -8 && P.mismatch <= 7;
+    if ((cols_possible || res_maybe || tf_possible || fast_possible) && !b->acgt_known) {
         if (b->n_refs) HIP_TRY(hipMemcpy(b->ref_desc.data(), b->d_refs.p, b->n_refs * sizeof(SeqDesc), hipMemcpyDeviceToHost));
         if (b->n_reads) HIP_TRY(hipMemcpy(b->read_desc.data(), b->d_reads.p, b->n_reads * sizeof(SeqDesc), hipMemcpyDeviceToHost));
         b->acgt_known = true;
@@ -718,6 +731,17 @@
         res_items.clear();
         n_res = 0; res_lds_words = 0; res_ops_words = 0;
     }
+    if (fast_possible && strip_items.empty() && col_items.empty() && res_items.empty() && tf_items.empty()) {
+        fast_sweep = true;
+        uint32_t r0 = 0;
+        for (size_t k = 0; k < np && fast_sweep; k++) {
+            const SeqDesc &qd = b->read_desc[pd[k].read_id];
+            fast_sweep = qd.acgt && b->ref_desc[pd[k].ref_id].acgt && qd.len <= 64u * SWMI_RMAX;
+            const uint32_t r = swmi_rows_per_lane(qd.len);
+            r0 = k == 0 ? r : (r0 == r ? r0 : 0u);
+        }
+        fast_r = fast_sweep && b->params.tie_mode != SWMI_TIE_STRICT ? r0 : 0u;
+    }
     {
         std::vector<uint8_t> is_res(np, 0);
         for (uint32_t k : res_items) is_res[k] = 1;
@@ -779,6 +803,7 @@
         pr.tfused_opt = ctx->tfused; pr.n_tf = n_tf; pr.tf_max_m = tf_max_m; pr.tf_max_n = tf_max_n; pr.tf_max_path = tf_max_path;
         pr.col_chunks_opt = ctx->col_chunks; pr.reverse_strips = ctx->dbg_reverse_strips != 0;
         pr.scores_only = ctx->scores_only != 0;
+        pr.fast_opt = ctx->fast_kernels; pr.fast_sweep = fast_sweep; pr.fast_r = fast_r;
     }
     rs.prep_us += std::chrono::duration<double, std::micro>(p1 - p0).count();
     rs.prep_upload_us += std::chrono::duration<double, std::micro>(std::chrono::steady_clock::now() - p1).count();
@@ -1075,8 +1100,10 @@
         if (ctx->profiling && !ext_timing) HIP_TRY(hipEventRecord(ctx->ev[0], ctx->stream));
         if (attempt == 0 && !whole_only) {
             if (fa.n_strip_items) HIP_TRY(hipMemsetAsync(fa.progress, 0, (size_t)fa.n_strip_items * sizeof(uint32_t), ctx->stream));
-            HIP_TRY(swmi_launch_fill(&fa, ctx->stream, ext_timing ? ctx->ev[0] : nullptr, ext_timing ? ctx->ev[1] : nullptr));
+            HIP_TRY(swmi_launch_fill(&fa, ctx->stream, ext_timing ? ctx->ev[0] : nullptr, ext_timing ? ctx->ev[1] : nullptr,
+                                     pr.fast_sweep ? 1u : 0u));
             rs.launches++;
+            if (pr.fast_sweep) b->fast_sweeps++;
         }
         if (n_tf) HIP_TRY(swmi_launch_tfused(&ta, &xt, ctx->stream));
         if (whole_only && n_tf) rs.launches++;
@@ -1098,7 +1125,8 @@
             if (attempt > 0 || whole_only) HIP_TRY(hipMemsetAsync(ta.q_count, 0, 4, ctx->stream));
             HIP_TRY(swmi_launch_traceback_split(&ta, (uint32_t)n_windows, ctx->stream));
         } else if (n_res + n_tf < np) {
-            HIP_TRY(swmi_launch_traceback(&ta, ctx->stream, ext_timing ? ctx->ev[2] : nullptr, ext_timing ? ctx->ev[3] : nullptr));
+            HIP_TRY(swmi_launch_traceback(&ta, ctx->stream, ext_timing ? ctx->ev[2] : nullptr, ext_timing ? ctx->ev[3] : nullptr, pr.fast_r));
+            if (pr.fast_r) b->fast_tracebacks++;
         }
         const bool time_all = ctx->profiling == 1;
         if (time_all && !ext_timing) HIP_TRY(hipEventRecord(ctx->ev[3], ctx->stream));
@@ -1367,6 +1395,7 @@
         b->views_built = false;
     }
     b->timing = swmi_timing{};
+    b->fast_sweeps = 0; b->fast_tracebacks = 0;
 
     b->eff_mode = (ctx->mode == 1 && (p->mismatch > 0 || p->gap > 0)) ? 2u : ctx->mode;
     if (ctx->tb_split < 0 && !ctx->scores_only && b->eff_mode == 1 && n_pairs >= 64 && n_pairs <= 256 &&
@@ -1396,6 +1425,7 @@
             if (live && cells * 100 >= (uint64_t)ctx->auto_ties_x100 * live) choice = 0;
             b->prep.valid = false;
             b->timing = swmi_timing{};
+            b->fast_sweeps = 0; b->fast_tracebacks = 0;
         }
         b->auto_choice = choice;
         b->auto_params = *p;
@@ -1588,6 +1618,14 @@
     return SWMI_OK;
 }
 
+extern "C" int swmi_batch_fast_kernels(const swmi_batch *b, uint32_t *sweeps, uint32_t *tracebacks) {
+    if (!b) return fail(SWMI_ERR_INVALID, "null argument");
+    if (!b->has_run) return fail(SWMI_ERR_INVALID, "batch has no results (run it first)");
+    if (sweeps) *sweeps = b->fast_sweeps;
+    if (tracebacks) *tracebacks = b->fast_tracebacks;
+    return SWMI_OK;
+}
+
 extern "C" int swmi_batch_timing(const swmi_batch *b, swmi_timing *t) {
     if (!b || !t) return fail(SWMI_ERR_INVALID, "null argument");
     *t = b->timing;
diff --git a/sparksmithwaterman_amd/csrc/swmi_kernels.hip b/sparksmithwaterman_amd/csrc/swmi_kernels.hip
--- a/sparksmithwaterman_amd/csrc/swmi_kernels.hip
+++ b/sparksmithwaterman_amd/csrc/swmi_kernels.hip
@@ -799,6 +799,17 @@
 
 extern "C" __global__ void __launch_bounds__(WAVE * FILL_WAVES) __attribute__((amdgpu_waves_per_eu(4, 4)))
 sw_sweep_winmax_kernel(const FillArgs A) { fill_entry<SWMI_MODE_WINMAX>(A); }
+
+extern "C" __global__ void __launch_bounds__(WAVE * FILL_WAVES) __attribute__((amdgpu_waves_per_eu(8, 8)))
+sw_sweep_winmax_fast_kernel(const FillArgs A) {
+    const uint32_t pair = blockIdx.x * FILL_WAVES + (threadIdx.x >> 6);
+    if (pair >= A.n_pairs) return;
+    const uint32_t lane = threadIdx.x & 63u;
+    if (pair == 0 && lane == 0 && A.hdr) { A.hdr->reserved = 0; A.hdr->pad = 0; }
+    if (pair == 0 && lane == 0 && A.q_reset) *A.q_reset = 0u;
+    const PairDesc pd = A.pairs[pair];
+    sweep_fast_dispatch<false>(A, pd, lane, A.reads[pd.read_id].len, ColItem{0u, 0u, 0u, 0u});
+}
 
 extern "C" __global__ void __launch_bounds__(WAVE * FILL_WAVES)
 sw_sweep_winmax_strips_kernel(const FillArgs A) {
@@ -1550,9 +1561,15 @@
     return (pre && wave == 0) ? wlo0 : 0xFFFFFFFFu;
 }
 
-extern "C" __global__ void __launch_bounds__(WAVE * SWMI_TB_WAVES) __attribute__((amdgpu_waves_per_eu(4, 4)))
-sw_traceback_winmax_kernel(const TraceArgs A) {
-    extern __shared__ uint32_t wm_lds[];
+#define SWMI_BY_R(...)                                                     \
+    if constexpr (RF != 0) { constexpr int RR = RF; __VA_ARGS__; }         \
+    else if (R == 1) { constexpr int RR = 1; __VA_ARGS__; }                \
+    else if (R == 2) { constexpr int RR = 2; __VA_ARGS__; }                \
+    else if (R == 3) { constexpr int RR = 3; __VA_ARGS__; }                \
+    else             { constexpr int RR = 4; __VA_ARGS__; }
+
+template <int RF>
+__device__ __forceinline__ void traceback_winmax_entry(const TraceArgs &A, uint32_t *wm_lds) {
     const uint32_t pair = blockIdx.x;
     if (pair >= A.n_pairs) return;
     const uint32_t wave = threadIdx.x >> 6, lane = threadIdx.x & 63u;
@@ -1568,46 +1585,39 @@
     constexpr uint32_t WIN_WORDS = SWMI_CK_BLOCKS * SWMI_RMAX * WAVE;
     uint32_t *shared = wm_lds;
     uint32_t *tiles = wm_lds + 32;
-    const uint32_t R = swmi_rows_per_lane(A.reads[pd.read_id].len);
+    const uint32_t R = RF ? (uint32_t)RF : swmi_rows_per_lane(A.reads[pd.read_id].len);
     const uint32_t ccap = A.cells_cap ? A.cells_cap[pd.out_id] : A.cell_cap;
     const uint32_t tile_sets = A.pad2 ? 2u : 1u;
     uint32_t *tiles2 = A.pad2 ? tiles + n_waves * WIN_WORDS : nullptr;
     uint32_t *walker_lds0 = tiles + tile_sets * n_waves * WIN_WORDS;
-    if (!swmi_common_pair(A, A.refs[pd.ref_id], A.reads[pd.read_id])) {
-        if (wave == 0) {
-            uint32_t c;
-            if (R == 1)      c = detect_cells<1>(A, pd, po, lane, tiles);
-            else if (R == 2) c = detect_cells<2>(A, pd, po, lane, tiles);
-            else if (R == 3) c = detect_cells<3>(A, pd, po, lane, tiles);
-            else             c = detect_cells<4>(A, pd, po, lane, tiles);
-            if (lane == 0) {
-                po.n_cells = c;
-                if (c > ccap) po.flags |= SWMI_F_CELL_OVF;
-                A.out[pd.out_id] = po;
-                if (A.out_host) A.out_host[pd.out_id] = po;
-                shared[0] = c;
-            }
-            asm volatile("s_waitcnt vmcnt(0)" ::: "memory");
-        }
-        __syncthreads();
-        const uint32_t c = shared[0];
-        uint32_t nwr = c < SWMI_TB_SLOTS ? c : SWMI_TB_SLOTS;
-        if (nwr > n_waves) nwr = n_waves;
-        if (c > ccap || wave >= nwr) return;
-        po.n_cells = c;
-        uint32_t *lds = walker_lds0 + wave * per_walker;
-        uint32_t *tile = tiles + wave * WIN_WORDS;
-        if (R == 1)      traceback_pair<1, 1, false>(A, pd, po, lane, wave, nwr, lds, tile, nullptr, 1u);
-        else if (R == 2) traceback_pair<2, 1, false>(A, pd, po, lane, wave, nwr, lds, tile, nullptr, 1u);
-        else if (R == 3) traceback_pair<3, 1, false>(A, pd, po, lane, wave, nwr, lds, tile, nullptr, 1u);
-        else             traceback_pair<4, 1, false>(A, pd, po, lane, wave, nwr, lds, tile, nullptr, 1u);
-        return;
+    if constexpr (RF == 0) {
+        if (!swmi_common_pair(A, A.refs[pd.ref_id], A.reads[pd.read_id])) {
+            if (wave == 0) {
+                uint32_t c;
+                SWMI_BY_R(c = detect_cells<RR>(A, pd, po, lane, tiles));
+                if (lane == 0) {
+                    po.n_cells = c;
+                    if (c > ccap) po.flags |= SWMI_F_CELL_OVF;
+                    A.out[pd.out_id] = po;
+                    if (A.out_host) A.out_host[pd.out_id] = po;
+                    shared[0] = c;
+                }
+                asm volatile("s_waitcnt vmcnt(0)" ::: "memory");
+            }
+            __syncthreads();
+            const uint32_t c = shared[0];
+            uint32_t nwr = c < SWMI_TB_SLOTS ? c : SWMI_TB_SLOTS;
+            if (nwr > n_waves) nwr = n_waves;
+            if (c > ccap || wave >= nwr) return;
+            po.n_cells = c;
+            uint32_t *lds = walker_lds0 + wave * per_walker;
+            uint32_t *tile = tiles + wave * WIN_WORDS;
+            SWMI_BY_R(traceback_pair<RR, 1, false>(A, pd, po, lane, wave, nwr, lds, tile, nullptr, 1u));
+            return;
+        }
     }
     uint32_t pre_wlo;
-    if (R == 1)      pre_wlo = winmax_detect<1>(A, pd, po, lane, wave, n_waves, ccap, tiles, walker_lds0, per_walker, shared);
-    else if (R == 2) pre_wlo = winmax_detect<2>(A, pd, po, lane, wave, n_waves, ccap, tiles, walker_lds0, per_walker, shared);
-    else if (R == 3) pre_wlo = winmax_detect<3>(A, pd, po, lane, wave, n_waves, ccap, tiles, walker_lds0, per_walker, shared);
-    else             pre_wlo = winmax_detect<4>(A, pd, po, lane, wave, n_waves, ccap, tiles, walker_lds0, per_walker, shared);
+    SWMI_BY_R(pre_wlo = winmax_detect<RR>(A, pd, po, lane, wave, n_waves, ccap, tiles, walker_lds0, per_walker, shared));
     const uint32_t cnt = shared[0];
     if (shared[3] != 1u) pre_wlo = 0xFFFFFFFFu;
     if (cnt > ccap || cnt == 0u) return;
@@ -1619,27 +1629,40 @@
         if (wave >= nw) return;
         uint32_t *lds = walker_lds0 + wave * per_walker;
         uint32_t *tile = tiles + wave * WIN_WORDS;
-        if (R == 1)      traceback_pair<1, 1, false, false>(A, pd, po, lane, wave, nw, lds, tile, nullptr, 1u, pre_wlo, true);
-        else if (R == 2) traceback_pair<2, 1, false, false>(A, pd, po, lane, wave, nw, lds, tile, nullptr, 1u, pre_wlo, true);
-        else if (R == 3) traceback_pair<3, 1, false, false>(A, pd, po, lane, wave, nw, lds, tile, nullptr, 1u, pre_wlo, true);
-        else             traceback_pair<4, 1, false, false>(A, pd, po, lane, wave, nw, lds, tile, nullptr, 1u, pre_wlo, true);
+        SWMI_BY_R(traceback_pair<RR, 1, false, false>(A, pd, po, lane, wave, nw, lds, tile, nullptr, 1u, pre_wlo, true));
         return;
     }
     if (wave < nw) {
         uint32_t *lds = walker_lds0 + wave * per_walker;
         uint32_t *tile = tiles + wave * ts * WIN_WORDS;
         uint32_t *tile2 = tiles2 ? tiles2 + wave * ts * WIN_WORDS : nullptr;
-        if (R == 1)      traceback_pair<1, 1, true, false>(A, pd, po, lane, wave, nw, lds, tile, shared, ts, pre_wlo, true, nullptr, tile2);
-        else if (R == 2) traceback_pair<2, 1, true, false>(A, pd, po, lane, wave, nw, lds, tile, shared, ts, pre_wlo, true, nullptr, tile2);
-        else if (R == 3) traceback_pair<3, 1, true, false>(A, pd, po, lane, wave, nw, lds, tile, shared, ts, pre_wlo, true, nullptr, tile2);
-        else             traceback_pair<4, 1, true, false>(A, pd, po, lane, wave, nw, lds, tile, shared, ts, pre_wlo, true, nullptr, tile2);
+        SWMI_BY_R(traceback_pair<RR, 1, true, false>(A, pd, po, lane, wave, nw, lds, tile, shared, ts, pre_wlo, true, nullptr, tile2));
     } else {
-        if (R == 1)      coop_helper<1>(A, pd, lane, wave, nw, ts, n_waves, tiles, shared);
-        else if (R == 2) coop_helper<2>(A, pd, lane, wave, nw, ts, n_waves, tiles, shared);
-        else if (R == 3) coop_helper<3>(A, pd, lane, wave, nw, ts, n_waves, tiles, shared);
-        else             coop_helper<4>(A, pd, lane, wave, nw, ts, n_waves, tiles, shared);
-    }
-}
+        SWMI_BY_R(coop_helper<RR>(A, pd, lane, wave, nw, ts, n_waves, tiles, shared));
+    }
+}
+#undef SWMI_BY_R
+
+extern "C" __global__ void __launch_bounds__(WAVE * SWMI_TB_WAVES) __attribute__((amdgpu_waves_per_eu(4, 4)))
+sw_traceback_winmax_kernel(const TraceArgs A) {
+    extern __shared__ uint32_t wm_lds[];
+    traceback_winmax_entry<0>(A, wm_lds);
+}
+
+#ifndef SWMI_TB_FAST_ATTR
+#define SWMI_TB_FAST_ATTR __attribute__((amdgpu_num_vgpr(56)))
+#endif
+#define SWMI_TB_FAST_KERNEL(RR)                                                                                      \
+    extern "C" __global__ void __launch_bounds__(WAVE * SWMI_TB_WAVES) SWMI_TB_FAST_ATTR                              \
+    sw_traceback_winmax_fast_r##RR##_kernel(const TraceArgs A) {                                                      \
+        extern __shared__ uint32_t wm_lds[];                                                                          \
+        traceback_winmax_entry<RR>(A, wm_lds);                                                                        \
+    }
+SWMI_TB_FAST_KERNEL(1)
+SWMI_TB_FAST_KERNEL(2)
+SWMI_TB_FAST_KERNEL(3)
+SWMI_TB_FAST_KERNEL(4)
+#undef SWMI_TB_FAST_KERNEL
 
 extern "C" __global__ void __launch_bounds__(WAVE * FILL_WAVES)
 sw_traceback_kernel(const TraceArgs A) {
@@ -1979,11 +2002,12 @@
     (void)hipFuncSetAttribute(reinterpret_cast<const void *>(kernel), hipFuncAttributeMaxDynamicSharedMemorySize, 160 * 1024);
 }
 
-extern "C" hipError_t swmi_launch_fill(const FillArgs *a, hipStream_t st, hipEvent_t ev_start, hipEvent_t ev_stop) {
+extern "C" hipError_t swmi_launch_fill(const FillArgs *a, hipStream_t st, hipEvent_t ev_start, hipEvent_t ev_stop, uint32_t fast) {
     if (a->n_pairs == 0) return hipSuccess;
     static const bool attrs = [] {
         allow_big_lds(sw_fill_kernel); allow_big_lds(sw_fill_score_kernel); allow_big_lds(sw_sweep_winmax_kernel);
         allow_big_lds(sw_sweep_winmax_strips_kernel); allow_big_lds(sw_sweep_winmax_cols_kernel);
+        allow_big_lds(sw_sweep_winmax_fast_kernel);
         return true;
     }();
     (void)attrs;
@@ -1991,7 +2015,13 @@
     const size_t lds = spread_lds(grid.x);
     if (a->mode == 0)      hipLaunchKernelGGL(sw_fill_kernel, grid, block, lds, st, *a);
     else if (a->mode == 1) {
-        if (ev_start && ev_stop && !(a->skip_multi && a->n_strip_items) && !a->n_col_items) {
+        const bool plain = !(a->skip_multi && a->n_strip_items) && !a->n_col_items;
+        if (fast && plain) {
+            if (ev_start && ev_stop) hipExtLaunchKernelGGL(sw_sweep_winmax_fast_kernel, grid, block, (uint32_t)lds, st, ev_start, ev_stop, 0u, *a);
+            else                     hipLaunchKernelGGL(sw_sweep_winmax_fast_kernel, grid, block, lds, st, *a);
+            return hipGetLastError();
+        }
+        if (ev_start && ev_stop && plain) {
             hipExtLaunchKernelGGL(sw_sweep_winmax_kernel, grid, block, (uint32_t)lds, st, ev_start, ev_stop, 0u, *a);
             return hipGetLastError();
         }
@@ -2024,7 +2054,7 @@
     return hipGetLastError();
 }
 
-extern "C" hipError_t swmi_launch_traceback(const TraceArgs *a, hipStream_t st, hipEvent_t ev_start, hipEvent_t ev_stop) {
+extern "C" hipError_t swmi_launch_traceback(const TraceArgs *a, hipStream_t st, hipEvent_t ev_start, hipEvent_t ev_stop, uint32_t fast_r) {
     if (a->n_pairs == 0) return hipSuccess;
     const size_t tile = (size_t)(a->mode == 0 ? SWMI_TB_BLOCKS : SWMI_CK_BLOCKS) * SWMI_RMAX * WAVE;
     const size_t per_wave = (size_t)a->lds_words + a->lds_read_words + SWMI_TB_REFWIN_WORDS + tile;
@@ -2040,10 +2070,13 @@
         TraceArgs t = *a;
         t.pad2 = (spec_opt && (spec_opt == 2 || a->n_pairs <= 384u) && n_waves > 1u && (words + tiles) * sizeof(uint32_t) <= 160u * 1024u) ? 1u : 0u;
         if (t.pad2) words += tiles;
+        void (*k)(const TraceArgs) = fast_r == 1u ? sw_traceback_winmax_fast_r1_kernel : fast_r == 2u ? sw_traceback_winmax_fast_r2_kernel :
+                                      fast_r == 3u ? sw_traceback_winmax_fast_r3_kernel : fast_r == 4u ? sw_traceback_winmax_fast_r4_kernel :
+                                                     sw_traceback_winmax_kernel;
         if (ev_start && ev_stop)
-            hipExtLaunchKernelGGL(sw_traceback_winmax_kernel, dim3(a->n_pairs), dim3(WAVE * n_waves), (uint32_t)(words * sizeof(uint32_t)), st, ev_start, ev_stop, 0u, t);
+            hipExtLaunchKernelGGL(k, dim3(a->n_pairs), dim3(WAVE * n_waves), (uint32_t)(words * sizeof(uint32_t)), st, ev_start, ev_stop, 0u, t);
         else
-            hipLaunchKernelGGL(sw_traceback_winmax_kernel, dim3(a->n_pairs), dim3(WAVE * n_waves), words * sizeof(uint32_t), st, t);
+            hipLaunchKernelGGL(k, dim3(a->n_pairs), dim3(WAVE * n_waves), words * sizeof(uint32_t), st, t);
     } else {
         const dim3 grid((a->n_pairs + FILL_WAVES - 1) / FILL_WAVES, SWMI_TB_SLOTS);
         if (a->mode == 0) hipLaunchKernelGGL(sw_traceback_kernel, grid, block, per_wave * FILL_WAVES * sizeof(uint32_t), st, *a);
```

Result: faster. 2470 (median of 6 runs) (+2.1%).
